# CogSP/CoEvoNet

Hardware: NVIDIA B200
Metric: mpe_env_steps_per_sec (higher is better)
Workload: dtype f32

## Files before the change

### coevonet_b200/_lib.py

```python
from __future__ import annotations

import ctypes
import os
from ctypes import (POINTER, Structure, c_char_p, c_double, c_float, c_int, c_int32,
                    c_int64, c_uint8, c_uint32, c_uint64, c_void_p)

_HERE = os.path.dirname(os.path.abspath(__file__))
LIB_PATH = os.environ.get("COEVONET_LIB") or os.path.join(_HERE, "csrc", "libcoevonet_b200.so")

CEV_OK = 0
STATUS_NONFINITE = 1
SEAT = {"adversary_0": 0, "agent_0": 1, "agent_1": 2}
KIND_ES, KIND_GA, KIND_ENV, KIND_FRAMES, KIND_INIT, KIND_XOVER = 0, 1, 2, 3, 4, 5
INIT_STATE_DIM = 11
ROLLOUT_OUT_DIM = 4
ORDER_STABLE_DESC, ORDER_REFERENCE = 0, 1
GS_GEN, GS_SIGMA, GS_BEST, GS_STALE, GS_STOP, GS_STOP_GEN, GS_LAST_EVAL, GS_HIST = 0, 1, 4, 7, 10, 11, 12, 16


class RolloutCfg(Structure):
    _fields_ = [("n_cycles", c_int32), ("integrate_pos_first", c_int32),
                ("variant", c_int32), ("reserved", c_int32)]


class RolloutRole(Structure):
    _fields_ = [("member_seat", c_int32), ("reserved", c_int32),
                ("members", c_void_p), ("member_pitch", c_int64),
                ("opp_a", c_void_p), ("opp_a_pitch", c_int64),
                ("opp_b", c_void_p), ("opp_b_pitch", c_int64),
                ("init", c_void_p), ("out", c_void_p)]


class CevError(RuntimeError):
    pass


_SIGNATURES = {
    "cev_version": (c_int, []),
    "cev_last_error": (c_char_p, []),
    "cev_create": (c_int, [c_int, POINTER(c_void_p)]),
    "cev_destroy": (c_int, [c_void_p]),
    "cev_device_info": (c_int, [c_void_p, POINTER(c_int), POINTER(c_int)]),
    "cev_fc_dim": (c_int, [c_int]),
    "cev_fc_pitch": (c_int, [c_int]),
    "cev_dqn_dim": (c_int, [c_int, c_int]),
    "cev_dqn_pitch": (c_int, [c_int, c_int]),
    "cev_mpe_rollout_f32": (c_int, [c_void_p, c_int, c_void_p, c_int, c_int64,
                                    c_void_p, c_int64, c_void_p, c_int64, c_int,
                                    c_void_p, c_int, c_int, POINTER(RolloutCfg),
                                    c_void_p, c_void_p, c_void_p]),
    "cev_mpe_rollout_roles_f32": (c_int, [c_void_p, c_int, POINTER(RolloutRole), c_int, c_int, c_int, c_int,
                                          POINTER(RolloutCfg), c_void_p, c_void_p]),
    "cev_mpe_rollout_trace_f32": (c_int, [c_void_p, c_int, c_void_p, c_int, c_int64,
                                          c_void_p, c_int64, c_void_p, c_int64, c_int,
                                          c_void_p, c_int, c_int, POINTER(RolloutCfg),
                                          c_void_p, c_void_p, c_void_p, c_void_p, c_void_p, c_void_p]),
    "cev_mpe_rollout_plan": (c_int, [c_void_p, c_int, c_int, c_int, c_int, c_int, POINTER(c_int), POINTER(c_int)]),
    "cev_kernel_timing_enable": (c_int, [c_void_p, c_int]),
    "cev_kernel_timing_read": (c_int, [c_void_p, c_int, POINTER(c_double), POINTER(c_int)]),
    "cev_mpe_rollout_indexed_f32": (c_int, [c_void_p, c_void_p, c_int64, c_void_p, c_int64,
                                            c_void_p, c_int64, c_void_p, c_void_p, c_int,
                                            POINTER(RolloutCfg), c_void_p, c_void_p, c_void_p]),
    "cev_fc_forward_f32": (c_int, [c_void_p, c_void_p, c_int64, c_int, c_void_p, c_void_p, c_int64,
                                   c_void_p, c_void_p, c_void_p, c_void_p]),
    "cev_ga_repopulate_f32": (c_int, [c_void_p, c_void_p, c_int, c_int, c_int64, c_float, c_void_p, c_float,
                                      c_uint64, c_int, c_uint32, c_int64, c_int64,
                                      c_void_p, c_void_p, c_void_p]),
    "cev_gather_rows_f32": (c_int, [c_void_p, c_void_p, c_int64, c_void_p, c_int, c_int64, c_int64, c_void_p,
                                    c_void_p]),
    "cev_select_topk_f64": (c_int, [c_void_p, c_void_p, c_int64, c_int, c_int, c_void_p, c_void_p]),
    "cev_es_perturb_f32": (c_int, [c_void_p, c_void_p, c_int, c_float, c_void_p, c_uint64, c_int, c_uint32,
                                   c_int64, c_int64, c_int64, c_void_p, c_void_p, c_void_p]),
    "cev_es_perturb_prefix_f32": (c_int, [c_void_p, c_void_p, c_int64, c_int64, c_float, c_void_p, c_uint64, c_int,
                                          c_uint32, c_int64, c_int64, c_int64, c_void_p, c_void_p]),
    "cev_es_update_f32": (c_int, [c_void_p, c_void_p, c_int, c_float, c_void_p, c_float, c_int64,
                                  c_uint64, c_int, c_uint32, c_int64, c_int64, c_void_p, c_void_p]),
    "cev_es_update_members_f32": (c_int, [c_void_p, c_void_p, c_void_p, c_int64, c_void_p, c_int, c_float, c_void_p,
                                          c_float, c_int64, c_int64, c_void_p, c_void_p]),
    "cev_weight_stats_f32": (c_int, [c_void_p, c_void_p, c_int64, c_int64, c_int, c_void_p, c_void_p]),
    "cev_generation_state_doubles": (c_int, [c_int]),
    "cev_generation_end_f64": (c_int, [c_void_p, c_void_p, c_int, c_int, c_int, c_void_p, c_int, c_int, c_double,
                                       c_double, c_int, c_double, c_int, c_void_p]),
    "cev_axpy_f32": (c_int, [c_void_p, c_float, c_void_p, c_void_p, c_int64, c_void_p]),
    "cev_diversity_dist_f32": (c_int, [c_void_p, c_void_p, c_int64, c_int64, c_void_p, c_int,
                                       c_void_p, c_void_p]),
    "cev_deepqn_forward": (c_int, [c_void_p, c_void_p, c_int, c_int64, c_void_p, c_int, c_int,
                                   c_int, c_void_p, c_void_p, c_void_p]),
    "cev_atari_synth_step_u8": (c_int, [c_void_p, c_uint64, c_int64, c_int64, c_int, c_void_p, c_void_p, c_void_p,
                                        c_void_p, c_void_p]),
    "cev_atari_observe_u8": (c_int, [c_void_p, c_void_p, c_int64, c_int, c_int, c_void_p, c_void_p]),
    "cev_fc_init_f32": (c_int, [c_void_p, c_int, c_uint64, c_int, c_int64, c_int64, c_int64, c_void_p, c_void_p]),
    "cev_init_states_f64": (c_int, [c_void_p, c_uint64, c_uint32, c_int64, c_int64, c_void_p, c_void_p]),
    "cev_random_frames_u8": (c_int, [c_void_p, c_uint64, c_int64, c_void_p, c_void_p]),
    "cev_philox_words": (c_int, [c_void_p, c_uint64, c_int, c_int, c_uint32, c_int64, c_int64,
                                 c_int64, c_void_p, c_void_p]),
    "cev_fp32_peak": (c_int, [c_void_p, c_int, POINTER(c_double), c_void_p]),
}

EXPORTED_SYMBOLS = tuple(_SIGNATURES)

_lib = None


def load():
    global _lib
    if _lib is not None:
        return _lib
    if not os.path.isfile(LIB_PATH):
        raise CevError(
            f"{LIB_PATH} is missing: build it with `python -c 'import __graft_entry__ as g; g.build()'` "
            "(or `make -C coevonet_b200/csrc`).  coevonet_b200 has no CPU fallback.")
    lib = ctypes.CDLL(LIB_PATH)
    for name, (res, args) in _SIGNATURES.items():
        fn = getattr(lib, name)
        fn.restype = res
        fn.argtypes = args
    _lib = lib
    return lib


def check(rc, what=""):
    if rc != CEV_OK:
        msg = load().cev_last_error()
        raise CevError(f"{what} failed (rc={rc}): {msg.decode() if msg else ''}")


_handles = {}


def handle(device_index, stream=0):
    key = (int(device_index), int(stream or 0))
    h = _handles.get(key)
    if h is None:
        lib = load()
        hp = c_void_p()
        check(lib.cev_create(int(device_index), ctypes.byref(hp)), "cev_create")
        h = _handles[key] = hp
    return h


def device_info(device_index):
    n_sm, n_cl = c_int(), c_int()
    check(load().cev_device_info(handle(device_index), ctypes.byref(n_sm), ctypes.byref(n_cl)),
          "cev_device_info")
    return n_sm.value, n_cl.value
```

### coevonet_b200/csrc/api.cu

```cuda
#include <stdarg.h>
#include <string.h>

#include "common.cuh"

namespace cev {

static thread_local char g_err[512] = "";

void set_error(const char* fmt, ...) {
    va_list ap;
    va_start(ap, fmt);
    vsnprintf(g_err, sizeof(g_err), fmt, ap);
    va_end(ap);
}

int check_cuda(cudaError_t e, const char* what) {
    if (e == cudaSuccess) return CEV_OK;
    set_error("CUDA error %d (%s) in %s", (int)e, cudaGetErrorString(e), what);
    return CEV_ERR_CUDA;
}

}

using namespace cev;
// ... 83 lines not shown

int cev_dqn_dim(int c_in, int n_actions) {
    return 32 * c_in * 64 + 32 + 64 * 32 * 16 + 64 + 64 * 64 * 9 + 64 + 512 * 3136 + 512 + n_actions * 512 +
           n_actions + 2 * (32 + 64 + 64);
}
int cev_dqn_pitch(int c_in, int n_actions) { return round_up(cev_dqn_dim(c_in, n_actions), 32); }

static int rollout_plan(const cev_handle* h, int P, int K, int E, int variant) {
    if (variant != 0) return variant;
    if ((int64_t)P * K * E >= 2048) return 3;
    return h->n_clusters > 0 ? 2 : 1;
}

static int check_cfg(const cev_rollout_cfg* cfg) {
    CEV_REQUIRE(cfg != nullptr, "rollout: null cfg");
    CEV_REQUIRE(cfg->n_cycles >= 0 && cfg->n_cycles <= MAX_CYCLES, "rollout: n_cycles must be in [0, %d]", MAX_CYCLES);
    CEV_REQUIRE(cfg->variant >= 0 && cfg->variant <= 3, "rollout: variant must be 0..3");
    return CEV_OK;
}

int cev_mpe_rollout_f32(cev_handle* h, int member_seat, const float* members, int P, int64_t member_pitch,
                        const float* opp_a, int64_t opp_a_pitch, const float* opp_b, int64_t opp_b_pitch, int K,
                        const double* init, int init_shared, int E, const cev_rollout_cfg* cfg, double* out,
                        int32_t* status, cev_stream stream) {
    CEV_REQUIRE(h && members && opp_a && opp_b && init && out, "mpe_rollout: null pointer");
    CEV_REQUIRE(member_seat >= 0 && member_seat <= 2, "mpe_rollout: member_seat must be 0..2");
    CEV_REQUIRE(P >= 0 && K >= 1 && E >= 1, "mpe_rollout: need P >= 0, K >= 1, E >= 1");
    int rc = check_cfg(cfg);
    if (rc) return rc;
    const int other[2] = {member_seat == 0 ? 1 : 0, member_seat == 2 ? 1 : 2};
    CEV_REQUIRE(member_pitch >= fc_offsets(seat_in_dim(member_seat)).total && member_pitch % 4 == 0,
                "mpe_rollout: member pitch too small / not a multiple of 4");
    CEV_REQUIRE(opp_a_pitch >= fc_offsets(seat_in_dim(other[0])).total && opp_a_pitch % 4 == 0 &&
                    opp_b_pitch >= fc_offsets(seat_in_dim(other[1])).total && opp_b_pitch % 4 == 0,
                "mpe_rollout: opponent pitch too small / not a multiple of 4");
    CEV_REQUIRE(aligned16(members) && aligned16(opp_a) && aligned16(opp_b), "mpe_rollout: rows must be 16B aligned");
    if (P == 0) return CEV_OK;
    CEV_GUARD(h);
    cudaStream_t st = (cudaStream_t)stream;
    const int variant = rollout_plan(h, P, K, E, cfg->variant);
    if (variant >= 2) {
        ClusterParams p{};
        p.members = members;
        p.member_pitch = member_pitch;
        p.P = P;
        p.opp[0] = opp_a;
        p.opp[1] = opp_b;
        p.opp_pitch[0] = opp_a_pitch;
        p.opp_pitch[1] = opp_b_pitch;
        p.K = K;
        p.member_seat = member_seat;
        p.init = init;
        p.init_shared = init_shared;
        p.E = E;
        p.out = out;
        p.status = status;
        p.n_cycles = cfg->n_cycles;
        p.pos_first = cfg->integrate_pos_first;
        return variant == 3 ? launch_rollout_lockstep(h, p, st) : launch_rollout_cluster(h, p, st);
    }
    GenericParams g{};
    g.w[member_seat] = members;
    g.pitch[member_seat] = member_pitch;
    g.w[other[0]] = opp_a;
    g.pitch[other[0]] = opp_a_pitch;
    g.w[other[1]] = opp_b;
    g.pitch[other[1]] = opp_b_pitch;
    g.idx = nullptr;
    g.member_seat = member_seat;
    g.K = K;
    g.E = E;
    g.init_shared = init_shared;
    g.init = init;
    g.out = out;
    g.status = status;
    g.n_cycles = cfg->n_cycles;
    g.pos_first = cfg->integrate_pos_first;
    g.N = (int64_t)P * K * E;
    return launch_rollout_generic(h, g, st);
}

int cev_mpe_rollout_roles_f32(cev_handle* h, int n_roles, const cev_rollout_role* roles, int P, int K, int init_shared,
                              int E, const cev_rollout_cfg* cfg, int32_t* status, cev_stream stream) {
    CEV_REQUIRE(h && roles, "mpe_rollout_roles: null pointer");
    CEV_REQUIRE(n_roles >= 1 && n_roles <= CEV_MAX_ROLES, "mpe_rollout_roles: n_roles must be 1..%d", CEV_MAX_ROLES);
    CEV_REQUIRE(P >= 0 && K >= 1 && E >= 1, "mpe_rollout_roles: need P >= 0, K >= 1, E >= 1");
    int rc = check_cfg(cfg);
    if (rc) return rc;
    for (int r = 0; r < n_roles; ++r)
        CEV_REQUIRE(roles[r].members && roles[r].opp_a && roles[r].opp_b && roles[r].init && roles[r].out,
                    "mpe_rollout_roles: null pointer in role %d", r);
    if (P == 0) return CEV_OK;
    const int variant = rollout_plan(h, P, K, E, cfg->variant);
    if (variant != 3) {
        for (int r = 0; r < n_roles; ++r) {
            rc = cev_mpe_rollout_f32(h, roles[r].member_seat, roles[r].members, P, roles[r].member_pitch, roles[r].opp_a,
                                     roles[r].opp_a_pitch, roles[r].opp_b, roles[r].opp_b_pitch, K, roles[r].init,
                                     init_shared, E, cfg, roles[r].out, status, stream);
            if (rc) return rc;
        }
        return CEV_OK;
    }
    ClusterParams ps[CEV_MAX_ROLES];
    for (int r = 0; r < n_roles; ++r) {
        const cev_rollout_role& q = roles[r];
        CEV_REQUIRE(q.member_seat >= 0 && q.member_seat <= 2, "mpe_rollout_roles: member_seat must be 0..2");
        const int other[2] = {q.member_seat == 0 ? 1 : 0, q.member_seat == 2 ? 1 : 2};
        CEV_REQUIRE(q.member_pitch >= fc_offsets(seat_in_dim(q.member_seat)).total && q.member_pitch % 4 == 0 &&
                        q.opp_a_pitch >= fc_offsets(seat_in_dim(other[0])).total && q.opp_a_pitch % 4 == 0 &&
                        q.opp_b_pitch >= fc_offsets(seat_in_dim(other[1])).total && q.opp_b_pitch % 4 == 0,
                    "mpe_rollout_roles: pitch too small / not a multiple of 4");
        CEV_REQUIRE(aligned16(q.members) && aligned16(q.opp_a) && aligned16(q.opp_b),
                    "mpe_rollout_roles: rows must be 16B aligned");
        ClusterParams& p = ps[r];
        p = ClusterParams{};
        p.members = q.members;
        p.member_pitch = q.member_pitch;
        p.P = P;
        p.opp[0] = q.opp_a;
        p.opp[1] = q.opp_b;
        p.opp_pitch[0] = q.opp_a_pitch;
        p.opp_pitch[1] = q.opp_b_pitch;
        p.K = K;
        p.member_seat = q.member_seat;
        p.init = q.init;
        p.init_shared = init_shared;
        p.E = E;
        p.out = q.out;
        p.status = status;
        p.n_cycles = cfg->n_cycles;
        p.pos_first = cfg->integrate_pos_first;
    }
    CEV_GUARD(h);
    return launch_rollout_lockstep_roles(h, ps, n_roles, (cudaStream_t)stream);
}

int cev_mpe_rollout_trace_f32(cev_handle* h, int member_seat, const float* members, int P, int64_t member_pitch,
                              const float* opp_a, int64_t opp_a_pitch, const float* opp_b, int64_t opp_b_pitch, int K,
                              const double* init, int init_shared, int E, const cev_rollout_cfg* cfg,
                              const int32_t* forced_actions, float* logits_out, int32_t* actions_out, double* out,
                              int32_t* status, cev_stream stream) {
    CEV_REQUIRE(h && members && opp_a && opp_b && init && out, "mpe_rollout_trace: null pointer");
    CEV_REQUIRE(member_seat >= 0 && member_seat <= 2, "mpe_rollout_trace: member_seat must be 0..2");
    CEV_REQUIRE(P >= 1 && K >= 1 && E >= 1, "mpe_rollout_trace: need P, K, E >= 1");
    int rc = check_cfg(cfg);
    if (rc) return rc;
    const int other[2] = {member_seat == 0 ? 1 : 0, member_seat == 2 ? 1 : 2};
    CEV_REQUIRE(member_pitch >= fc_offsets(seat_in_dim(member_seat)).total && member_pitch % 4 == 0 &&
                    opp_a_pitch >= fc_offsets(seat_in_dim(other[0])).total && opp_a_pitch % 4 == 0 &&
                    opp_b_pitch >= fc_offsets(seat_in_dim(other[1])).total && opp_b_pitch % 4 == 0,
                "mpe_rollout_trace: pitch too small / not a multiple of 4");
    CEV_REQUIRE(aligned16(members) && aligned16(opp_a) && aligned16(opp_b), "mpe_rollout_trace: rows must be 16B aligned");
    CEV_GUARD(h);
    ClusterParams p{};
    p.members = members;
    p.member_pitch = member_pitch;
    p.P = P;
    p.opp[0] = opp_a;
    p.opp[1] = opp_b;
    p.opp_pitch[0] = opp_a_pitch;
    p.opp_pitch[1] = opp_b_pitch;
    p.K = K;
    p.member_seat = member_seat;
    p.init = init;
    p.init_shared = init_shared;
    p.E = E;
    p.out = out;
    p.status = status;
    p.n_cycles = cfg->n_cycles;
    p.pos_first = cfg->integrate_pos_first;
    p.trace_forced = forced_actions;
    p.trace_logits = logits_out;
    p.trace_actions = actions_out;
    return launch_rollout_lockstep(h, p, (cudaStream_t)stream);
}

int cev_mpe_rollout_plan(cev_handle* h, int P, int K, int E, int n_cycles, int variant, int* variant_used,
                         int* n_launches) {
    CEV_REQUIRE(h != nullptr, "mpe_rollout_plan: null handle");
    CEV_REQUIRE(variant >= 0 && variant <= 3, "mpe_rollout_plan: variant must be 0..3");
    const int v = rollout_plan(h, P, K, E, variant);
    if (variant_used) *variant_used = v;
    if (n_launches) *n_launches = v == 3 ? rollout_lockstep_launches(n_cycles) : (v == 2 ? 3 : 1);
    return CEV_OK;
}

int cev_kernel_timing_enable(cev_handle* h, int on) {
    CEV_REQUIRE(h != nullptr, "kernel_timing_enable: null handle");
    CEV_GUARD(h);
    if (on && !h->timing_ev[0]) {
        for (int k = 0; k < 2; ++k) {
            h->timing_ev[k] = new cudaEvent_t[2 * CEV_TIMING_MAX];
            for (int i = 0; i < 2 * CEV_TIMING_MAX; ++i) CEV_CUDA(cudaEventCreate(&h->timing_ev[k][i]));
        }
    }
    h->timing_on = on ? 1 : 0;
    h->timing_n[0] = h->timing_n[1] = 0;
    return CEV_OK;
}

int cev_kernel_timing_read(cev_handle* h, int which, double* total_ms, int* n_launches) {
    CEV_REQUIRE(h != nullptr && (which == 0 || which == 1), "kernel_timing_read: bad arguments");
    CEV_GUARD(h);
    double tot = 0.0;
    const int n = h->timing_n[which];
    for (int i = 0; i < n; ++i) {
        CEV_CUDA(cudaEventSynchronize(h->timing_ev[which][2 * i + 1]));
        float ms = 0.f;
        CEV_CUDA(cudaEventElapsedTime(&ms, h->timing_ev[which][2 * i], h->timing_ev[which][2 * i + 1]));
        tot += ms;
    }
    if (total_ms) *total_ms = tot;
    if (n_launches) *n_launches = n;
    h->timing_n[which] = 0;
// ... 51 lines not shown
```

### coevonet_b200/csrc/common.cuh

```cuda
#pragma once

#include <cuda_runtime.h>
#include <math_constants.h>
#include <stdint.h>
#include <stdio.h>

#include "../../include/coevonet_b200.h"

namespace cev {

constexpr int H1 = 512;
constexpr int H2 = 256;
constexpr int NACT = 5;
constexpr int IN_ADV = 8;
constexpr int IN_GOOD = 10;
constexpr float LN_EPS = 1e-5f;
constexpr int MAX_CYCLES = 25;

struct FcOffsets {
    int fc1w, fc1b, ln1g, ln1b, fc2w, fc2b, ln2g, ln2b, outw, outb, total;
};

__host__ __device__ constexpr FcOffsets fc_offsets(int in_dim) {
    FcOffsets o{};
// ... 189 lines not shown
    return __fmaf_rn(__uint2float_rn(x), 2.3283064365386963e-10f, 1.1641532182693481e-10f);
}

__device__ __forceinline__ float neg2_log_u(float u) {
    const float t = 1.0f - u;
    const float ser = t * fmaf(t, fmaf(t, fmaf(t, fmaf(t, 0.2f, 0.25f), 0.33333334f), 0.5f), 1.0f);
    const float lg = -0.6931471805599453f * __log2f(u);
    return 2.0f * (t < 0.03125f ? ser : lg);
}

__device__ __forceinline__ void box_muller(uint32_t xa, uint32_t xb, float& z0, float& z1) {
    const float u1 = u01(xa), u2 = u01(xb);
    float r;
    asm("sqrt.approx.ftz.f32 %0, %1;\n" : "=f"(r) : "f"(neg2_log_u(u1)));
    float s, c;
    __sincosf(6.283185307179586f * (u2 - 0.5f), &s, &c);
    z0 = -(r * c);
    z1 = -(r * s);
}

__device__ __forceinline__ void normal4(const PhiloxKeys& keys, uint32_t tag, uint32_t gen,
                                        uint32_t member, uint32_t j4, float z[4]) {
    const U4 r = philox4x32_10(U4{j4, member, gen, tag}, keys);
    box_muller(r.x, r.y, z[0], z[1]);
    box_muller(r.z, r.w, z[2], z[3]);
}

__host__ __device__ __forceinline__ uint32_t noise_tag(int kind, int role) {
    return (uint32_t)(role & 0xFF) | ((uint32_t)kind << 8);
}

}

constexpr int CEV_TIMING_MAX = 4096;

#define CEV_MAX_ROLES 3

struct cev_handle {
    int device;
    int n_sm;
    int n_clusters;
    void* workspace;
    size_t workspace_bytes;
    void* opp_workspace;
    size_t opp_workspace_bytes;
    void* ls_workspace;
    size_t ls_workspace_bytes;
    cudaStream_t side_stream;
    cudaEvent_t fork_ev, join_ev;
    cudaStream_t env_stream, opp_stream2[3], mem_stream2[2];
    cudaEvent_t ev_opp[CEV_MAX_ROLES], ev_mem[CEV_MAX_ROLES], ev_env[CEV_MAX_ROLES];
    int timing_on;
    int timing_n[2];
    cudaEvent_t* timing_ev[2];
};

namespace cev {
struct GenericParams {
    const float* w[3];
    int64_t pitch[3];
    const int32_t* idx;
    int member_seat, K, E, init_shared;
    const double* init;
    double* out;
    int32_t* status;
    int n_cycles, pos_first;
    int64_t N;
};
struct ClusterParams {
    const float* members;
    int64_t member_pitch;
    int P;
    const float* opp[2];
    int64_t opp_pitch[2];
    const float4* opp_packed[2];
    int K;
    int member_seat;
    const double* init;
    int init_shared;
    int E;
    double* out;
    int32_t* status;
    int n_cycles, pos_first;
    const int32_t* trace_forced;
    float* trace_logits;
    int32_t* trace_actions;
};
int launch_rollout_generic(cev_handle* h, const GenericParams& p, cudaStream_t stream);
int launch_rollout_cluster(cev_handle* h, const ClusterParams& p, cudaStream_t stream);
int rollout_cluster_max_clusters(int device);
int launch_rollout_lockstep(cev_handle* h, const ClusterParams& p, cudaStream_t stream);
int launch_rollout_lockstep_roles(cev_handle* h, const ClusterParams* ps, int n_roles, cudaStream_t stream);
int rollout_lockstep_launches(int n_cycles);
int launch_deepqn_fc_tc(cev_handle* h, const float* members, int64_t pitch, int P, int B, int n_act, int f1w_off,
                        int f1b_off, int ow_off, int ob_off, const float* act3, float* logits, int32_t* actions,
                        cudaStream_t stream);
int launch_fc_forward(cev_handle* h, const float* W, int64_t pitch, int in_dim, const int32_t* idx,
                      const float* obs, int64_t N, float* logits, int32_t* actions, int32_t* status,
                      cudaStream_t stream);
}
```

### coevonet_b200/csrc/ls_member_tc.cuh

```cuda
#pragma once

namespace cev {

constexpr int MT_THREADS = 480;
constexpr int MT_PROD_WARPS = 8;
constexpr int MT_BK = 32, MT_KT = H1 / MT_BK;
constexpr int MT_NB = LS_BT;
constexpr int MT_R = 5, MT_L = 3;
constexpr uint32_t MT_A_BYTES = H2 * MT_BK * 4;
constexpr uint32_t MT_X_BYTES = MT_NB * MT_BK * 4;
constexpr uint32_t MT_XSLOT = 2 * MT_X_BYTES;
constexpr uint32_t MT_W1C_FLOATS = MT_BK * IN_GOOD + 3 * MT_BK;
constexpr uint32_t MT_W1C_BYTES = MT_W1C_FLOATS * 4;
constexpr uint32_t MT_TAIL_BYTES = LS_TAIL_FLOATS * 4;
constexpr size_t MT_OFF_X = (size_t)MT_R * MT_A_BYTES;
constexpr size_t MT_OFF_W1C = MT_OFF_X + (size_t)MT_L * MT_XSLOT;
constexpr size_t MT_OFF_HS = MT_OFF_W1C + (size_t)MT_R * MT_W1C_BYTES;
constexpr size_t MT_OFF_TAIL = MT_OFF_HS + (size_t)H2 * MT_NB * 4;
constexpr size_t MT_OFF_OBS = MT_OFF_TAIL + MT_TAIL_BYTES;
constexpr size_t MT_OFF_STAT = MT_OFF_OBS + 2 * MT_NB * LS_OBS_PAD * 4;
constexpr size_t MT_OFF_RED = MT_OFF_STAT + 2 * MT_NB * 8;
constexpr size_t MT_OFF_BAR = MT_OFF_RED + (size_t)(2 + NACT) * 4 * MT_NB * 4;
constexpr size_t MT_SMEM = MT_OFF_BAR + 256 + 1024 ;
constexpr int MT_ACC = 2 * MT_NB;
constexpr int MT_TM_OP = 2 * 2 * MT_ACC;
constexpr int MT_TM_SLOT = 2 * 2 * MT_BK;
static_assert(MT_TM_OP + MT_L * MT_TM_SLOT <= 512, "tensor memory budget");
static_assert(MT_OFF_X % 1024 == 0 && MT_XSLOT % 1024 == 0, "operand tiles must keep the 1024-byte alignment of the swizzle atoms");
static_assert(MT_OFF_W1C % 16 == 0 && MT_W1C_BYTES % 16 == 0 && MT_OFF_TAIL % 16 == 0 && MT_OFF_BAR % 8 == 0,
              "bulk-copy alignment");
static_assert(MT_SMEM <= 232448, "member stage exceeds the 227 KB shared-memory limit");
constexpr uint32_t MT_IDESC32 = (1u << 4) | (2u << 7) | (2u << 10) | ((uint32_t)((2 * MT_NB) >> 3) << 17) |
                                ((uint32_t)(128 >> 4) << 24);

__device__ __forceinline__ void mt_issue_ktile(uint32_t d_tmem, uint32_t a_tmem, uint64_t x_hilo, uint32_t accumulate,
                                               uint32_t bar_op) {
    asm volatile(
        "{\n"
        ".reg .pred pe, pa, pt;\n"
        ".reg .b64 b1, b2, b3;\n"
        ".reg .b32 h1, h2, h3, l0, l1, l2, l3;\n"
        "elect.sync _|pe, 0xffffffff;\n"
        "setp.ne.b32 pa, %3, 0;\n"
        "setp.eq.b32 pt, 0, 0;\n"
        "add.s64 b1, %2, 2;\n add.s64 b2, %2, 4;\n add.s64 b3, %2, 6;\n"
        "add.u32 h1, %1, 8;\n add.u32 h2, %1, 16;\n add.u32 h3, %1, 24;\n"
        "add.u32 l0, %1, 32;\n add.u32 l1, %1, 40;\n add.u32 l2, %1, 48;\n add.u32 l3, %1, 56;\n"
        "@pe tcgen05.mma.cta_group::1.kind::tf32 [%0], [l0], %2, %5, pa;\n"
        "@pe tcgen05.mma.cta_group::1.kind::tf32 [%0], [%1], %2, %5, pt;\n"
        "@pe tcgen05.mma.cta_group::1.kind::tf32 [%0], [l1], b1, %5, pt;\n"
        "@pe tcgen05.mma.cta_group::1.kind::tf32 [%0], [h1], b1, %5, pt;\n"
        "@pe tcgen05.mma.cta_group::1.kind::tf32 [%0], [l2], b2, %5, pt;\n"
        "@pe tcgen05.mma.cta_group::1.kind::tf32 [%0], [h2], b2, %5, pt;\n"
        "@pe tcgen05.mma.cta_group::1.kind::tf32 [%0], [l3], b3, %5, pt;\n"
        "@pe tcgen05.mma.cta_group::1.kind::tf32 [%0], [h3], b3, %5, pt;\n"
        "@pe tcgen05.commit.cta_group::1.mbarrier::arrive::one.shared::cluster.b64 [%4];\n"
        "}\n" ::"r"(d_tmem),
        "r"(a_tmem), "l"(x_hilo), "r"(accumulate), "r"(bar_op), "r"(MT_IDESC32)
        : "memory");
}
struct LsMemberTcParams {
    const float* members;
    int64_t pitch;
    int n_chunks, KE, seat, n_jobs;
    int64_t N;
    const float* obs;
    int32_t* act;
    float* gap;
    const double* l1stats;
    int32_t* status;
    float* logits;
};

template <int IN>
__global__ void __launch_bounds__(MT_THREADS, 1)
ls_member_tc_kernel(const __grid_constant__ CUtensorMap map_w, const LsMemberTcParams p) {
    extern __shared__ unsigned char mt_raw[];
    unsigned char* base = mt_raw + ((1024u - (tc_smem_u32(mt_raw) & 1023u)) & 1023u);
    unsigned char* raw_mem = base;
    unsigned char* x_mem = base + MT_OFF_X;
    float* hs = reinterpret_cast<float*>(base + MT_OFF_HS);
    unsigned char* w1c_mem = base + MT_OFF_W1C;
    float* tail = reinterpret_cast<float*>(base + MT_OFF_TAIL);
    float* obsbuf = reinterpret_cast<float*>(base + MT_OFF_OBS);
    float2* statbuf = reinterpret_cast<float2*>(base + MT_OFF_STAT);
    float* redA = reinterpret_cast<float*>(base + MT_OFF_RED);
    float* redB = redA + 4 * MT_NB;
    float* redC = redB + 4 * MT_NB;
    uint64_t* bar_raw_full = reinterpret_cast<uint64_t*>(base + MT_OFF_BAR);
    uint64_t* bar_raw_empty = bar_raw_full + MT_R;
    uint64_t* bar_lo_full = bar_raw_empty + MT_R;
    uint64_t* bar_lo_empty = bar_lo_full + MT_L;
    uint64_t* bar_tfull = bar_lo_empty + MT_L;
    uint64_t* bar_tempty = bar_tfull + 2;
    uint64_t* bar_stat_full = bar_tempty + 2;
    uint64_t* bar_tail_full = bar_stat_full + 2;
    uint64_t* bar_tail_empty = bar_tail_full + 1;
    uint32_t* tmem_slot = reinterpret_cast<uint32_t*>(bar_tail_empty + 1);
    int* flag = reinterpret_cast<int*>(tmem_slot + 1);

    const int warp = threadIdx.x >> 5, lane = threadIdx.x & 31;
    const int job0 = (int)blockIdx.x, job_stride = (int)gridDim.x;
    constexpr uint32_t W1ROWS_BYTES = (uint32_t)(MT_BK * IN) * 4;
    const FcOffsets om = fc_offsets(IN);

    if (threadIdx.x == 0) {
        *flag = 0;
        for (int i = 0; i < MT_R; ++i) {
            tc_mbar_init(bar_raw_full + i, 1);
            tc_mbar_init(bar_raw_empty + i, MT_PROD_WARPS / 2);
        }
        for (int i = 0; i < MT_L; ++i) {
            tc_mbar_init(bar_lo_full + i, MT_PROD_WARPS / 2);
            tc_mbar_init(bar_lo_empty + i, 2);
        }
        for (int i = 0; i < 2; ++i) {
            tc_mbar_init(bar_tfull + i, 2);
            tc_mbar_init(bar_tempty + i, 4);
            tc_mbar_init(bar_stat_full + i, 1);
        }
        tc_mbar_init(bar_tail_full, 1);
        tc_mbar_init(bar_tail_empty, 1);
        asm volatile("fence.mbarrier_init.release.cluster;\n" ::: "memory");
    }
    if (warp == 1) {
        asm volatile("tcgen05.alloc.cta_group::1.sync.aligned.shared::cta.b32 [%0], %1;\n" ::"r"(tc_smem_u32(tmem_slot)),
                     "r"(512u)
                     : "memory");
        asm volatile("tcgen05.relinquish_alloc_permit.cta_group::1.sync.aligned;\n" ::: "memory");
    }
    asm volatile("tcgen05.fence::before_thread_sync;\n" ::: "memory");
    __syncthreads();
    asm volatile("tcgen05.fence::after_thread_sync;\n" ::: "memory");
    const uint32_t tmem_base = *tmem_slot;

    if (warp == 0) {
        if (lane == 0) {
            uint32_t it = 0, js = 0;
            for (int job = job0; job < p.n_jobs; job += job_stride, ++js) {
                const int m = job / p.n_chunks;
                const float* mrow = p.members + (int64_t)m * p.pitch;
                for (int kt = 0; kt < MT_KT; ++kt, ++it) {
                    const uint32_t rs = it % MT_R, use = it / MT_R;
                    if (use > 0) tc_mbar_wait(bar_raw_empty + rs, (use - 1) & 1);
                    tc_mbar_expect_tx(bar_raw_full + rs, MT_A_BYTES + W1ROWS_BYTES + 3 * MT_BK * 4);
                    tma_load_3d(raw_mem + (size_t)rs * MT_A_BYTES, &map_w, bar_raw_full + rs, kt * MT_BK, 0, m);
                    float* c = reinterpret_cast<float*>(w1c_mem + (size_t)rs * MT_W1C_BYTES);
                    bulk_g2s(c, mrow + kt * MT_BK * IN, W1ROWS_BYTES, bar_raw_full + rs);
                    bulk_g2s(c + MT_BK * IN, mrow + om.fc1b + kt * MT_BK, MT_BK * 4, bar_raw_full + rs);
                    bulk_g2s(c + MT_BK * IN + MT_BK, mrow + om.ln1g + kt * MT_BK, MT_BK * 4, bar_raw_full + rs);
                    bulk_g2s(c + MT_BK * IN + 2 * MT_BK, mrow + om.ln1b + kt * MT_BK, MT_BK * 4, bar_raw_full + rs);
                }
                if (js >= 1) tc_mbar_wait(bar_tail_empty, (js - 1) & 1);
                tc_mbar_expect_tx(bar_tail_full, MT_TAIL_BYTES);
                bulk_g2s(tail, mrow + om.fc2b, MT_TAIL_BYTES, bar_tail_full);
            }
        }
    } else if (warp == 1 || warp == 14) {
        const int t = warp == 1 ? 0 : 1;
        const uint32_t x_base = tc_smem_u32(x_mem);
        uint32_t it = 0, js = 0;
        for (int job = job0; job < p.n_jobs; job += job_stride, ++js) {
            const uint32_t as = js & 1, ause = js >> 1;
            if (ause > 0) tc_mbar_wait(bar_tempty + as, (ause - 1) & 1);
            asm volatile("tcgen05.fence::after_thread_sync;\n" ::: "memory");
            const uint32_t d_tmem = tmem_base + as * (2 * MT_ACC) + t * MT_ACC;
            for (int kt = 0; kt < MT_KT; ++kt, ++it) {
                const uint32_t ls = it % MT_L, luse = it / MT_L;
                const uint64_t x_hilo = umma_desc_sw128(x_base + ls * MT_XSLOT);
                const uint32_t a_tmem = tmem_base + MT_TM_OP + ls * MT_TM_SLOT + t * (2 * MT_BK);
                tc_mbar_wait(bar_lo_full + ls, luse & 1);
                asm volatile("tcgen05.fence::after_thread_sync;\n" ::: "memory");
                mt_issue_ktile(d_tmem, a_tmem, x_hilo, kt ? 1u : 0u, tc_smem_u32(bar_lo_empty + ls));
                if (kt == MT_KT - 1) tc_commit_elected(tc_smem_u32(bar_tfull + as));
                __syncwarp();
            }
        }
    } else if (warp < 2 + MT_PROD_WARPS) {
        const int grp = (warp - 2) >> 2;
        const int pt = (threadIdx.x - 64) & 127;
        const int q = warp & 3;
        const int r = q * 32 + lane;
        const int e = pt & 15, g = pt >> 4;
        uint32_t it = 0, js = 0;
        for (int job = job0; job < p.n_jobs; job += job_stride, ++js) {
            const uint32_t b = js & 1, buse = js >> 1;
            tc_mbar_wait(bar_stat_full + b, buse & 1);
            float x[IN];
            {
                const float* ob = obsbuf + ((size_t)b * MT_NB + e) * LS_OBS_PAD;
#pragma unroll
                for (int i = 0; i < IN; i += 2) {
                    const float2 v = *reinterpret_cast<const float2*>(ob + i);
                    x[i] = v.x;
                    x[i + 1] = v.y;
                }
            }
            const float2 st = statbuf[b * MT_NB + e];
            const float mean = st.x, rstd = st.y;
            for (int kt = 0; kt < MT_KT; ++kt, ++it) {
                if ((int)(it & 1) != grp) continue;
                const uint32_t rs = it % MT_R, ruse = it / MT_R, ls = it % MT_L, luse = it / MT_L;
                const unsigned char* slot = raw_mem + (size_t)rs * MT_A_BYTES;
                unsigned char* xs = x_mem + (size_t)ls * MT_XSLOT;
                if (luse > 0) tc_mbar_wait(bar_lo_empty + ls, (luse - 1) & 1);
                tc_mbar_wait(bar_raw_full + rs, ruse & 1);
                asm volatile("tcgen05.fence::after_thread_sync;\n" ::: "memory");
#pragma unroll
                for (int t = 0; t < 2; ++t) {
                    const float4* row = reinterpret_cast<const float4*>(slot + (size_t)(t * 128 + r) * 128);
                    float w[32];
#pragma unroll
                    for (int c = 0; c < 8; ++c) {
                        const float4 v = row[c ^ (r & 7)];
                        w[4 * c] = v.x;
                        w[4 * c + 1] = v.y;
                        w[4 * c + 2] = v.z;
                        w[4 * c + 3] = v.w;
                    }
                    const uint32_t ta = tmem_base + ((uint32_t)(q * 32) << 16) + MT_TM_OP + ls * MT_TM_SLOT + t * (2 * MT_BK);
                    f3_tmem_st32(ta, w);
#pragma unroll
                    for (int i = 0; i < 32; ++i) w[i] = f3_lo(w[i]);
                    f3_tmem_st32(ta + MT_BK, w);
                }
                {
                    const float* w1c = reinterpret_cast<const float*>(w1c_mem + (size_t)rs * MT_W1C_BYTES);
                    const int kl = g * 4;
                    const float4 bb = *reinterpret_cast<const float4*>(w1c + MT_BK * IN + kl);
                    const float4 gg = *reinterpret_cast<const float4*>(w1c + MT_BK * IN + MT_BK + kl);
                    const float4 ee = *reinterpret_cast<const float4*>(w1c + MT_BK * IN + 2 * MT_BK + kl);
                    const float bq[4] = {bb.x, bb.y, bb.z, bb.w}, gq[4] = {gg.x, gg.y, gg.z, gg.w},
                                eq[4] = {ee.x, ee.y, ee.z, ee.w};
                    float hi[4], lo[4];
#pragma unroll
                    for (int qq = 0; qq < 4; ++qq) {
                        const float2* wr = reinterpret_cast<const float2*>(w1c + (kl + qq) * IN);
                        float pre = 0.f;
#pragma unroll
                        for (int i2 = 0; i2 < IN / 2; ++i2) {
                            const float2 v = wr[i2];
                            pre = fmaf(v.x, x[2 * i2], pre);
                            pre = fmaf(v.y, x[2 * i2 + 1], pre);
                        }
                        pre += bq[qq];
                        const float h = fmaxf(fmaf((pre - mean) * rstd, gq[qq], eq[qq]), 0.f);
                        hi[qq] = __uint_as_float(__float_as_uint(h) & 0xffffe000u);
                        lo[qq] = h - hi[qq];
                    }
                    const int off = e * 128 + ((g ^ (e & 7)) << 4);
                    *reinterpret_cast<float4*>(xs + off) = make_float4(hi[0], hi[1], hi[2], hi[3]);
                    *reinterpret_cast<float4*>(xs + MT_X_BYTES + off) = make_float4(lo[0], lo[1], lo[2], lo[3]);
                }
                __syncwarp();
                if (lane == 0) tc_mbar_arrive(bar_raw_empty + rs);
                asm volatile("tcgen05.wait::st.sync.aligned;\n" ::: "memory");
                asm volatile("fence.proxy.async.shared::cta;\n" ::: "memory");
                asm volatile("tcgen05.fence::before_thread_sync;\n" ::: "memory");
                __syncwarp();
                if (lane == 0) tc_mbar_arrive(bar_lo_full + ls);
            }
        }
    } else {
        const int q = warp & 3;
        const int et = (warp - 10) * 32 + lane;
        const int we = warp - 10;
        const int e1 = et & 15, g1 = et >> 4;
        constexpr int RP = H2 / 8;
        const float* b2 = tail;
        const float* g2 = tail + H2;
        const float* be2 = tail + 2 * H2;
        const float* w3 = tail + 3 * H2;
        const float* b3 = tail + 3 * H2 + NACT * H2;
        auto stage_job = [&](int job, uint32_t js) {
            if (job < p.n_jobs && et < MT_NB) {
                const uint32_t b = js & 1;
                const int m = job / p.n_chunks, ch = job % p.n_chunks;
                const int n_env = min(MT_NB, p.KE - ch * MT_NB);
                const int64_t ep = (int64_t)m * p.KE + (int64_t)ch * MT_NB + (et < n_env ? et : 0);
                const float4* src = reinterpret_cast<const float4*>(p.obs + ep * LS_OBS_PAD);
                const float4 v0 = __ldg(src), v1 = __ldg(src + 1), v2 = __ldg(src + 2);
                float4* dst = reinterpret_cast<float4*>(obsbuf + ((size_t)b * MT_NB + et) * LS_OBS_PAD);
                dst[0] = v0;
                dst[1] = v1;
                dst[2] = v2;
                const float xo[12] = {v0.x, v0.y, v0.z, v0.w, v1.x, v1.y, v1.z, v1.w, v2.x, v2.y, v2.z, v2.w};
                const double* S = p.l1stats + (size_t)m * LS_L1S;
                double z[11];
#pragma unroll
                for (int a = 0; a < 11; ++a) z[a] = a < IN ? (double)xo[a] : (a == IN ? 1.0 : 0.0);
                double md = 0.0, vd = 0.0;
#pragma unroll
                for (int a = 0; a < 11; ++a) {
                    md = fma(__ldg(S + a), z[a], md);
                    double ra = 0.0;
#pragma unroll
                    for (int c = 0; c < 11; ++c) ra = fma(__ldg(S + 11 + a * 11 + c), z[c], ra);
                    vd = fma(ra, z[a], vd);
                }
                const float m1 = (float)md, var = (float)vd;
                if (!isfinite(m1) || !isfinite(var)) *flag = 1;
                statbuf[b * MT_NB + et] = make_float2(m1, 1.0f / sqrtf(var + LN_EPS));
            }
            if (job < p.n_jobs && we == 0) {
                __syncwarp();
                if (lane == 0) tc_mbar_arrive(bar_stat_full + (js & 1));
            }
        };
        stage_job(job0, 0);
        stage_job(job0 + job_stride, 1);
        uint32_t js = 0;
        for (int job = job0; job < p.n_jobs; job += job_stride, ++js) {
            const int m = job / p.n_chunks, ch = job % p.n_chunks;
            const int n_env = min(MT_NB, p.KE - ch * MT_NB);
            const int64_t ep0 = (int64_t)m * p.KE + (int64_t)ch * MT_NB;
            const uint32_t as = js & 1, ause = js >> 1;
            tc_mbar_wait(bar_tail_full, js & 1);
            tc_mbar_wait(bar_tfull + as, ause & 1);
            asm volatile("tcgen05.fence::after_thread_sync;\n" ::: "memory");
#pragma unroll
            for (int t = 0; t < 2; ++t) {
                uint32_t xh[16], xl[16];
                const uint32_t ta = tmem_base + ((uint32_t)(q * 32) << 16) + as * (2 * MT_ACC) + t * MT_ACC;
                f3_tmem_ld16(ta, xh);
                f3_tmem_ld16(ta + MT_NB, xl);
                const int row = t * 128 + q * 32 + lane;
                const float bias = b2[row];
                float4* dst = reinterpret_cast<float4*>(hs + row * MT_NB);
                const int sw = (row >> 1) & 3;
                float h[16];
#pragma unroll
                for (int n = 0; n < 16; ++n)
                    h[n] = (__uint_as_float(xl[n]) + __uint_as_float(xh[n])) + bias;
#pragma unroll
                for (int c = 0; c < 4; ++c) dst[c ^ sw] = make_float4(h[4 * c], h[4 * c + 1], h[4 * c + 2], h[4 * c + 3]);
            }
            asm volatile("tcgen05.fence::before_thread_sync;\n" ::: "memory");
            __syncwarp();
            if (lane == 0) tc_mbar_arrive(bar_tempty + as);
            asm volatile("bar.sync 1, 128;\n" ::: "memory");
            float pre2[RP];
            float lsum = 0.f;
#pragma unroll
            for (int j = 0; j < RP; ++j) {
                const int row = g1 + 8 * j;
                pre2[j] = hs[row * MT_NB + ((((e1 >> 2) ^ ((row >> 1) & 3))) << 2) + (e1 & 3)];
                lsum += pre2[j];
            }
            lsum = group_sum<MT_NB>(lsum);
            if (lane < MT_NB) redA[we * MT_NB + e1] = lsum;
            asm volatile("bar.sync 1, 128;\n" ::: "memory");
            float mean = 0.f;
#pragma unroll
            for (int w = 0; w < 4; ++w) mean += redA[w * MT_NB + e1];
            mean *= (1.0f / H2);
            float lsq = 0.f;
#pragma unroll
            for (int j = 0; j < RP; ++j) {
                const float d = pre2[j] - mean;
                lsq = fmaf(d, d, lsq);
            }
            lsq = group_sum<MT_NB>(lsq);
            if (lane < MT_NB) redB[we * MT_NB + e1] = lsq;
            asm volatile("bar.sync 1, 128;\n" ::: "memory");
            float var = 0.f;
#pragma unroll
            for (int w = 0; w < 4; ++w) var += redB[w * MT_NB + e1];
            var *= (1.0f / H2);
            if (!isfinite(mean) || !isfinite(var)) *flag = 1;
            const float rstd = 1.0f / sqrtf(var + LN_EPS);
            float pl[NACT] = {0.f, 0.f, 0.f, 0.f, 0.f};
#pragma unroll
            for (int j = 0; j < RP; ++j) {
                const int row = g1 + 8 * j;
                const float h = fmaxf(fmaf((pre2[j] - mean) * rstd, g2[row], be2[row]), 0.f);
#pragma unroll
                for (int a = 0; a < NACT; ++a) pl[a] = fmaf(w3[a * H2 + row], h, pl[a]);
            }
#pragma unroll
            for (int a = 0; a < NACT; ++a) {
                const float v = group_sum<MT_NB>(pl[a]);
                if (lane < MT_NB) redC[(we * NACT + a) * MT_NB + e1] = v;
            }
            asm volatile("bar.sync 1, 128;\n" ::: "memory");
            if (et < MT_NB) {
                float lg[NACT];
                bool fin = true;
#pragma unroll
                for (int a = 0; a < NACT; ++a) {
                    float v = redC[a * MT_NB + et];
#pragma unroll
                    for (int w = 1; w < 4; ++w) v += redC[(w * NACT + a) * MT_NB + et];
                    lg[a] = v + b3[a];
                    fin = fin && isfinite(lg[a]);
                }
                float gap;
                const int a = argmax_first5(lg, gap);
                if (et < n_env) {
                    if (!fin) *flag = 1;
                    p.act[ep0 + et] = a;
                    p.gap[ep0 + et] = gap;
                    if (p.logits) {
#pragma unroll
                        for (int u = 0; u < NACT; ++u) p.logits[(ep0 + et) * NACT + u] = lg[u];
                    }
                }
            }
            asm volatile("bar.sync 1, 128;\n" ::: "memory");
            if (et == 0) tc_mbar_arrive(bar_tail_empty);
            stage_job(job + 2 * job_stride, js + 2);
        }
    }
    asm volatile("tcgen05.fence::before_thread_sync;\n" ::: "memory");
    __syncthreads();
    if (threadIdx.x == 0 && *flag && p.status) atomicOr(p.status, CEV_STATUS_NONFINITE);
    if (warp == 1)
        asm volatile("tcgen05.dealloc.cta_group::1.sync.aligned.b32 %0, %1;\n" ::"r"(tmem_base), "r"(512u) : "memory");
}

}
```

### coevonet_b200/csrc/population_ops.cu

```cuda
#include "common.cuh"

namespace cev {

constexpr int PT = 256;

__device__ __forceinline__ float pick_sigma(float sigma, const double* __restrict__ sigma_dev) {
    return sigma_dev ? (float)__ldg(sigma_dev) : sigma;
}

__global__ void __launch_bounds__(PT) ga_repopulate_kernel(
    const float* __restrict__ elites, int E, int D, int64_t pitch, float sigma_arg,
    const double* __restrict__ sigma_dev,
    const PhiloxKeys keys, uint32_t tag, uint32_t gen, int64_t row0,
    float xrate, uint32_t xtag,
    float* __restrict__ out, float* __restrict__ noise_out) {
    const float sigma = pick_sigma(sigma_arg, sigma_dev);
    const int64_t r = blockIdx.x;
    const int64_t c = row0 + r;
    const int j4 = blockIdx.y * PT + threadIdx.x;
    __shared__ int64_t mate_s;
    int64_t mate = -1;
    if (xrate > 0.f && E >= 2) {
        if (threadIdx.x == 0) {
            int64_t m = -1;
            if (c != 0) {
                const U4 y = philox4x32_10(U4{0xFFFFFFFFu, (uint32_t)c, gen, xtag}, keys);
                if ((double)y.x < (double)xrate * 4294967296.0)
                    m = ((c - 1) % E + 1 + (int64_t)(y.y % (uint32_t)(E - 1))) % E;
            }
            mate_s = m;
        }
        __syncthreads();
        mate = mate_s;
    }
    if ((int64_t)j4 * 4 >= pitch) return;
    const int64_t parent = (c == 0) ? 0 : (c - 1) % E;
    const float4 pv = *reinterpret_cast<const float4*>(elites + parent * pitch + (int64_t)j4 * 4);
    float p[4] = {pv.x, pv.y, pv.z, pv.w};
    if (mate >= 0) {
        const float4 qv = *reinterpret_cast<const float4*>(elites + mate * pitch + (int64_t)j4 * 4);
        const U4 x = philox4x32_10(U4{(uint32_t)j4, (uint32_t)c, gen, xtag}, keys);
        if (!(x.x & 1u)) p[0] = qv.x;
        if (!(x.y & 1u)) p[1] = qv.y;
        if (!(x.z & 1u)) p[2] = qv.z;
        if (!(x.w & 1u)) p[3] = qv.w;
    }
    float z[4] = {0.f, 0.f, 0.f, 0.f};
    if (c != 0) {
        normal4(keys, tag, gen, (uint32_t)c, (uint32_t)j4, z);
#pragma unroll
        for (int i = 0; i < 4; ++i) {
            const int j = j4 * 4 + i;
            if (j < D) p[i] = __fadd_rn(p[i], __fmul_rn(sigma, z[i]));
            else { p[i] = 0.f; z[i] = 0.f; }
        }
    }
    *reinterpret_cast<float4*>(out + r * pitch + (int64_t)j4 * 4) = make_float4(p[0], p[1], p[2], p[3]);
    if (noise_out)
        *reinterpret_cast<float4*>(noise_out + r * pitch + (int64_t)j4 * 4) = make_float4(z[0], z[1], z[2], z[3]);
}

constexpr int K5T = 128;
__global__ void __launch_bounds__(K5T, 10) es_perturb_kernel(
    const float* __restrict__ theta, int in_dim, int64_t pitch, float sigma_arg,
    const double* __restrict__ sigma_dev,
    const PhiloxKeys keys, uint32_t tag, uint32_t gen, int64_t row0,
    float* __restrict__ out, float* __restrict__ noise_out) {
    const float sigma = pick_sigma(sigma_arg, sigma_dev);
    const FcOffsets o = fc_offsets(in_dim);
    const int64_t r = blockIdx.x;
    const int64_t c = row0 + r;
    const int j4 = blockIdx.y * K5T + threadIdx.x;
    const int j = j4 * 4;
    if ((int64_t)j >= pitch) return;
    const float4 pv = __ldg(reinterpret_cast<const float4*>(theta + j));
    float p[4] = {pv.x, pv.y, pv.z, pv.w};
    float z[4] = {0.f, 0.f, 0.f, 0.f};
    if (j < o.total && fc_is_perturbable(o, j)) {
        normal4(keys, tag, gen, (uint32_t)c, (uint32_t)j4, z);
#pragma unroll
        for (int i = 0; i < 4; ++i) {
            if (j + i < o.total) p[i] = __fadd_rn(p[i], __fmul_rn(sigma, z[i]));
            else { z[i] = 0.f; p[i] = 0.f; }
        }
    } else if (j >= o.total) {
        p[0] = p[1] = p[2] = p[3] = 0.f;
    }
    __stcs(reinterpret_cast<float4*>(out + r * pitch + j), make_float4(p[0], p[1], p[2], p[3]));
    if (noise_out)
        *reinterpret_cast<float4*>(noise_out + r * pitch + j) = make_float4(z[0], z[1], z[2], z[3]);
}

__global__ void __launch_bounds__(PT) es_perturb_prefix_kernel(
    const float* __restrict__ theta, int64_t d_pert, int64_t d_total, int64_t pitch, float sigma_arg,
    const double* __restrict__ sigma_dev,
    const PhiloxKeys keys, uint32_t tag, uint32_t gen, int64_t row0, float* __restrict__ out) {
    const float sigma = pick_sigma(sigma_arg, sigma_dev);
    const int64_t r = blockIdx.x;
    const int64_t j4 = (int64_t)blockIdx.y * PT + threadIdx.x;
    if (j4 * 4 >= pitch) return;
    const float4 pv = *reinterpret_cast<const float4*>(theta + j4 * 4);
    float p[4] = {pv.x, pv.y, pv.z, pv.w};
    if (j4 * 4 < d_pert) {
        float z[4];
        normal4(keys, tag, gen, (uint32_t)(row0 + r), (uint32_t)j4, z);
#pragma unroll
        for (int i = 0; i < 4; ++i)
            if (j4 * 4 + i < d_pert) p[i] = __fadd_rn(p[i], __fmul_rn(sigma, z[i]));
    }
#pragma unroll
    for (int i = 0; i < 4; ++i)
        if (j4 * 4 + i >= d_total) p[i] = 0.f;
    __stcs(reinterpret_cast<float4*>(out + r * pitch + j4 * 4), make_float4(p[0], p[1], p[2], p[3]));
}

__global__ void __launch_bounds__(PT) es_update_partial_kernel(
    const double* __restrict__ fitness, int in_dim, int64_t pitch, float sigma_arg,
    const double* __restrict__ sigma_dev,
    const PhiloxKeys keys, uint32_t tag, uint32_t gen, int64_t row0, int64_t n_rows,
    int n_split, float* __restrict__ partial) {
    const float sigma = pick_sigma(sigma_arg, sigma_dev);
    const FcOffsets o = fc_offsets(in_dim);
    const int j4 = blockIdx.x * PT + threadIdx.x;
    if ((int64_t)j4 * 4 >= pitch) return;
    const int sp = blockIdx.y;
    const int64_t per = (n_rows + n_split - 1) / n_split;
    const int64_t r_lo = sp * per, r_hi = min(n_rows, r_lo + per);
    float acc[4] = {0.f, 0.f, 0.f, 0.f};
    bool pert[4];
#pragma unroll
    for (int i = 0; i < 4; ++i) {
        const int j = j4 * 4 + i;
        pert[i] = j < o.total && fc_is_perturbable(o, j);
    }
    if (pert[0] || pert[1] || pert[2] || pert[3]) {
        for (int64_t r = r_lo; r < r_hi; ++r) {
            const float f = (float)fitness[r];
            float z[4];
            normal4(keys, tag, gen, (uint32_t)(row0 + r), (uint32_t)j4, z);
#pragma unroll
            for (int i = 0; i < 4; ++i) acc[i] = fmaf(__fmul_rn(sigma, z[i]), f, acc[i]);
        }
    }
#pragma unroll
    for (int i = 0; i < 4; ++i)
        if (!pert[i]) acc[i] = 0.f;
    *reinterpret_cast<float4*>(partial + (int64_t)sp * pitch + (int64_t)j4 * 4) =
        make_float4(acc[0], acc[1], acc[2], acc[3]);
}

__global__ void __launch_bounds__(PT) es_update_members_partial_kernel(
    const double* __restrict__ fitness, const float* __restrict__ members, const float* __restrict__ theta,
    int64_t pitch, int64_t n_rows, int n_split, float* __restrict__ partial) {
    const int j4 = blockIdx.x * PT + threadIdx.x;
    if ((int64_t)j4 * 4 >= pitch) return;
    const int sp = blockIdx.y;
    const int64_t per = (n_rows + n_split - 1) / n_split;
    const int64_t r_lo = sp * per, r_hi = min(n_rows, r_lo + per);
    const float4 t4 = *reinterpret_cast<const float4*>(theta + (int64_t)j4 * 4);
    float acc[4] = {0.f, 0.f, 0.f, 0.f};
    const float4* col = reinterpret_cast<const float4*>(members) + j4;
    const int64_t stride4 = pitch / 4;
#pragma unroll 8
    for (int64_t r = r_lo; r < r_hi; ++r) {
        const float f = (float)fitness[r];
        const float4 m = __ldcs(col + r * stride4);
        acc[0] = fmaf(__fsub_rn(m.x, t4.x), f, acc[0]);
        acc[1] = fmaf(__fsub_rn(m.y, t4.y), f, acc[1]);
        acc[2] = fmaf(__fsub_rn(m.z, t4.z), f, acc[2]);
        acc[3] = fmaf(__fsub_rn(m.w, t4.w), f, acc[3]);
    }
    *reinterpret_cast<float4*>(partial + (int64_t)sp * pitch + (int64_t)j4 * 4) =
        make_float4(acc[0], acc[1], acc[2], acc[3]);
}
// ... 330 lines not shown
#pragma unroll
        for (int i = 0; i < 8; ++i) {
            if (MODE == 1) a[i] = __ffma2_rn(a[i], b, c);
            else { a[i].x = fmaf(a[i].x, b.x, c.x); a[i].y = fmaf(a[i].y, b.y, c.y); }
        }
    }
    float s = 0.f;
#pragma unroll
    for (int i = 0; i < 8; ++i) s += a[i].x + a[i].y;
    if (s == 123.456f) out[0] = s;
}

}

using namespace cev;

static inline void split_seed(uint64_t seed, uint32_t& k0, uint32_t& k1) {
    k0 = (uint32_t)(seed & 0xFFFFFFFFull);
    k1 = (uint32_t)(seed >> 32);
}

static int ensure_workspace(cev_handle* h, size_t bytes) {
    if (h->workspace_bytes >= bytes) return CEV_OK;
    if (h->workspace) cudaFree(h->workspace);
    h->workspace = nullptr;
    h->workspace_bytes = 0;
    CEV_CUDA(cudaMalloc(&h->workspace, bytes));
    h->workspace_bytes = bytes;
    return CEV_OK;
}

static bool aligned16(const void* p) { return (reinterpret_cast<uintptr_t>(p) & 15u) == 0; }

extern "C" {

int cev_ga_repopulate_f32(cev_handle* h, const float* elites, int E, int D, int64_t pitch, float sigma,
                          const double* sigma_dev, float crossover_rate, uint64_t seed, int role, uint32_t gen,
                          int64_t row0, int64_t n_rows, float* out, float* noise_out, cev_stream stream) {
    CEV_REQUIRE(h != nullptr, "ga_repopulate: null handle");
    if (n_rows == 0) return CEV_OK;
    CEV_REQUIRE(elites && out, "ga_repopulate: null pointer");
    CEV_REQUIRE(E >= 1 && D >= 1 && pitch >= D && pitch % 4 == 0, "ga_repopulate: bad E/D/pitch");
    CEV_REQUIRE(crossover_rate >= 0.f && crossover_rate <= 1.f, "ga_repopulate: crossover_rate must be in [0, 1]");
    CEV_REQUIRE(aligned16(elites) && aligned16(out) && aligned16(noise_out), "ga_repopulate: 16B alignment");
    CEV_REQUIRE(row0 >= 0 && n_rows >= 0 && row0 + n_rows <= 0xFFFFFFFFll, "ga_repopulate: bad row range");
    CEV_GUARD(h);
    uint32_t k0, k1;
    split_seed(seed, k0, k1);
    dim3 grid((unsigned)n_rows, (unsigned)((pitch / 4 + PT - 1) / PT));
    ga_repopulate_kernel<<<grid, PT, 0, (cudaStream_t)stream>>>(elites, E, D, pitch, sigma, sigma_dev, philox_keys(k0, k1),
                                                               noise_tag(CEV_KIND_GA, role), gen, row0, crossover_rate,
                                                               noise_tag(CEV_KIND_XOVER, role), out, noise_out);
    return check_cuda(cudaGetLastError(), "ga_repopulate_kernel");
}

int cev_gather_rows_f32(cev_handle* h, const float* src, int64_t pitch, const int64_t* idx, int n, int64_t row0,
                        int64_t n_local, float* dst, cev_stream stream) {
    CEV_REQUIRE(h != nullptr, "gather_rows: null handle");
    if (n <= 0) return CEV_OK;
    CEV_REQUIRE((src || n_local == 0) && idx && dst, "gather_rows: null pointer");
    CEV_REQUIRE(pitch % 4 == 0 && aligned16(src) && aligned16(dst), "gather_rows: alignment");
    CEV_GUARD(h);
    dim3 grid((unsigned)n, (unsigned)((pitch / 4 + PT - 1) / PT));
    gather_rows_kernel<<<grid, PT, 0, (cudaStream_t)stream>>>(src, pitch, idx, row0, n_local, dst);
    return check_cuda(cudaGetLastError(), "gather_rows_kernel");
}

int cev_select_topk_f64(cev_handle* h, const double* fitness, int64_t P, int k, int order, int64_t* idx_out,
                        cev_stream stream) {
    CEV_REQUIRE(h && fitness && idx_out, "select_topk: null pointer");
    CEV_REQUIRE(k >= 1 && k <= P, "select_topk: need 1 <= k <= P (elites_number %d, population %lld)", k, (long long)P);
    CEV_REQUIRE(order == 0 || order == 1, "select_topk: order must be 0 (ties -> lower index) or 1 (reference)");
    CEV_GUARD(h);
    int rc = ensure_workspace(h, (size_t)P + 256);
    if (rc) return rc;
    select_topk_kernel<<<1, SEL_T, 0, (cudaStream_t)stream>>>(fitness, P, k, order, static_cast<uint8_t*>(h->workspace),
                                                              idx_out);
    return check_cuda(cudaGetLastError(), "select_topk_kernel");
}

int cev_es_perturb_f32(cev_handle* h, const float* theta, int in_dim, float sigma, const double* sigma_dev,
                       uint64_t seed, int role, uint32_t gen, int64_t row0, int64_t n_rows, int64_t pitch,
                       float* out, float* noise_out, cev_stream stream) {
    CEV_REQUIRE(h != nullptr, "es_perturb: null handle");
    if (n_rows == 0) return CEV_OK;
    CEV_REQUIRE(theta && out, "es_perturb: null pointer");
    CEV_REQUIRE(in_dim == IN_ADV || in_dim == IN_GOOD, "es_perturb: in_dim must be 8 or 10");
    CEV_REQUIRE(pitch >= fc_offsets(in_dim).total && pitch % 4 == 0, "es_perturb: bad pitch");
    CEV_REQUIRE(aligned16(theta) && aligned16(out) && aligned16(noise_out), "es_perturb: 16B alignment");
    CEV_REQUIRE(row0 >= 0 && n_rows >= 0 && row0 + n_rows <= 0xFFFFFFFFll, "es_perturb: bad row range");
    CEV_GUARD(h);
    uint32_t k0, k1;
    split_seed(seed, k0, k1);
    dim3 grid((unsigned)n_rows, (unsigned)((pitch / 4 + K5T - 1) / K5T));
    es_perturb_kernel<<<grid, K5T, 0, (cudaStream_t)stream>>>(theta, in_dim, pitch, sigma, sigma_dev, philox_keys(k0, k1),
                                                            noise_tag(CEV_KIND_ES, role), gen, row0, out,
                                                            noise_out);
    return check_cuda(cudaGetLastError(), "es_perturb_kernel");
}

int cev_es_update_f32(cev_handle* h, const double* fitness, int in_dim, float sigma, const double* sigma_dev,
                      float lr, int64_t n_total, uint64_t seed, int role, uint32_t gen, int64_t row0,
                      int64_t n_rows, float* delta, cev_stream stream) {
    CEV_REQUIRE(h && (fitness || n_rows == 0) && delta, "es_update: null pointer");
    CEV_REQUIRE(in_dim == IN_ADV || in_dim == IN_GOOD, "es_update: in_dim must be 8 or 10");
    CEV_REQUIRE(n_total >= 1 && n_rows >= 0 && (sigma_dev || sigma > 0.f), "es_update: bad n/sigma");
    CEV_REQUIRE(aligned16(delta), "es_update: 16B alignment");
    CEV_GUARD(h);
    const int64_t pitch = fc_pitch(in_dim);
    int n_split = (int)((n_rows + 63) / 64);
    if (n_split > 16) n_split = 16;
    if (n_split < 1) n_split = 1;
    int rc = ensure_workspace(h, (size_t)n_split * pitch * sizeof(float));
    if (rc) return rc;
    uint32_t k0, k1;
    split_seed(seed, k0, k1);
    float* partial = static_cast<float*>(h->workspace);
    dim3 grid((unsigned)((pitch / 4 + PT - 1) / PT), (unsigned)n_split);
    es_update_partial_kernel<<<grid, PT, 0, (cudaStream_t)stream>>>(fitness, in_dim, pitch, sigma, sigma_dev, philox_keys(k0, k1),
                                                                   noise_tag(CEV_KIND_ES, role), gen, row0,
                                                                   n_rows, n_split, partial);
    CEV_CUDA(cudaGetLastError());
    es_update_finish_kernel<<<(unsigned)((pitch + PT - 1) / PT), PT, 0, (cudaStream_t)stream>>>(
        partial, n_split, pitch, (double)lr, (double)n_total, sigma, sigma_dev, delta);
    return check_cuda(cudaGetLastError(), "es_update kernels");
}

int cev_es_perturb_prefix_f32(cev_handle* h, const float* theta, int64_t d_pert, int64_t d_total, float sigma,
                              const double* sigma_dev, uint64_t seed, int role, uint32_t gen, int64_t row0,
                              int64_t n_rows, int64_t pitch, float* out, cev_stream stream) {
    CEV_REQUIRE(h != nullptr, "es_perturb_prefix: null handle");
    if (n_rows == 0) return CEV_OK;
    CEV_REQUIRE(theta && out, "es_perturb_prefix: null pointer");
    CEV_REQUIRE(d_pert >= 0 && d_pert <= d_total && d_total <= pitch && pitch % 4 == 0 && pitch / 4 <= 0xFFFFFFFFll,
                "es_perturb_prefix: need 0 <= d_pert <= d_total <= pitch, pitch a multiple of 4");
    CEV_REQUIRE(aligned16(theta) && aligned16(out), "es_perturb_prefix: 16B alignment");
    CEV_REQUIRE(row0 >= 0 && n_rows >= 0 && row0 + n_rows <= 0xFFFFFFFFll, "es_perturb_prefix: bad row range");
    CEV_GUARD(h);
    uint32_t k0, k1;
    split_seed(seed, k0, k1);
    dim3 grid((unsigned)n_rows, (unsigned)((pitch / 4 + PT - 1) / PT));
    es_perturb_prefix_kernel<<<grid, PT, 0, (cudaStream_t)stream>>>(theta, d_pert, d_total, pitch, sigma, sigma_dev, philox_keys(k0, k1),
                                                                   noise_tag(CEV_KIND_ES, role), gen, row0, out);
    return check_cuda(cudaGetLastError(), "es_perturb_prefix_kernel");
}

int cev_es_update_members_f32(cev_handle* h, const double* fitness, const float* members, int64_t pitch,
                              const float* theta, int in_dim, float sigma, const double* sigma_dev, float lr,
                              int64_t n_total, int64_t n_rows, float* delta, cev_stream stream) {
    CEV_REQUIRE(h && ((fitness && members) || n_rows == 0) && theta && delta, "es_update_members: null pointer");
    CEV_REQUIRE(n_total >= 1 && n_rows >= 0 && (sigma_dev || sigma > 0.f), "es_update_members: bad n/sigma");
    CEV_REQUIRE(in_dim == 0 || in_dim == IN_ADV || in_dim == IN_GOOD, "es_update_members: in_dim must be 0, 8 or 10");
    CEV_REQUIRE(in_dim == 0 ? (pitch > 0 && pitch % 4 == 0) : pitch == fc_pitch(in_dim),
                "es_update_members: rows must use the padded pitch (cev_fc_pitch / cev_dqn_pitch)");
    CEV_REQUIRE(aligned16(delta) && aligned16(members) && aligned16(theta), "es_update_members: 16B alignment");
    CEV_GUARD(h);
    int n_split = (int)((n_rows + 31) / 32);
    if (n_split > 32) n_split = 32;
    if (n_split < 1) n_split = 1;
    int rc = ensure_workspace(h, (size_t)n_split * pitch * sizeof(float));
    if (rc) return rc;
    float* partial = static_cast<float*>(h->workspace);
    dim3 grid((unsigned)((pitch / 4 + PT - 1) / PT), (unsigned)n_split);
    es_update_members_partial_kernel<<<grid, PT, 0, (cudaStream_t)stream>>>(fitness, members, theta, pitch, n_rows,
                                                                           n_split, partial);
    CEV_CUDA(cudaGetLastError());
    es_update_finish_kernel<<<(unsigned)((pitch + PT - 1) / PT), PT, 0, (cudaStream_t)stream>>>(
        partial, n_split, pitch, (double)lr, (double)n_total, sigma, sigma_dev, delta);
    return check_cuda(cudaGetLastError(), "es_update_members kernels");
}

int cev_axpy_f32(cev_handle* h, float a, const float* x, float* y, int64_t n, cev_stream stream) {
    CEV_REQUIRE(h && x && y && n >= 0, "axpy: bad arguments");
    if (n == 0) return CEV_OK;
    CEV_GUARD(h);
    axpy_kernel<<<(unsigned)((n + PT - 1) / PT), PT, 0, (cudaStream_t)stream>>>(a, x, y, n);
    return check_cuda(cudaGetLastError(), "axpy_kernel");
}

int cev_diversity_dist_f32(cev_handle* h, const float* pop, int64_t n_rows, int64_t pitch, const float* ref,
// ... 123 lines not shown
```

### coevonet_b200/csrc/rollout_lockstep.cu

```cuda
#include <stdlib.h>

#include <cuda_fp16.h>

#include "rollout_common.cuh"
#include "tc_common.cuh"

namespace cev {

constexpr int LS_ST_FIELDS = 16;
constexpr int LS_OBS_PAD = 12;
constexpr int LS_L1S = 132;

struct LsBuffers {
    double* st;
    double* acc;
    float* min_gap;
    int32_t* goal;
    float* obs;
    int32_t* act;
    float* gap;
    __half* w2split;
    uint32_t* wmax;
    float* oscale;
    double* l1stats;
    float2* l1ms;
    double* ml1stats;
};

static size_t ls_align(size_t x) { return (x + 255) & ~(size_t)255; }

static size_t ls_carve(void* base, int64_t N, int K, int P, LsBuffers* b) {
    size_t off = 0;
    char* p = static_cast<char*>(base);
    auto take = [&](size_t bytes) {
        void* r = p ? p + off : nullptr;
        off += ls_align(bytes);
        return r;
    };
    LsBuffers t;
    t.w2split = static_cast<__half*>(take((size_t)2 * K * 2 * H2 * H1 * sizeof(__half)));
    t.wmax = static_cast<uint32_t*>(take((size_t)2 * K * sizeof(uint32_t)));
    t.oscale = static_cast<float*>(take((size_t)2 * K * 2 * sizeof(float)));
    t.st = static_cast<double*>(take((size_t)LS_ST_FIELDS * N * sizeof(double)));
    t.acc = static_cast<double*>(take((size_t)3 * N * sizeof(double)));
    t.min_gap = static_cast<float*>(take((size_t)N * sizeof(float)));
    t.goal = static_cast<int32_t*>(take((size_t)N * sizeof(int32_t)));
    t.obs = static_cast<float*>(take((size_t)3 * N * LS_OBS_PAD * sizeof(float)));
    t.act = static_cast<int32_t*>(take((size_t)3 * N * sizeof(int32_t)));
    t.gap = static_cast<float*>(take((size_t)3 * N * sizeof(float)));
    t.l1stats = static_cast<double*>(take((size_t)2 * K * LS_L1S * sizeof(double)));
    t.l1ms = static_cast<float2*>(take((size_t)2 * N * sizeof(float2)));
    t.ml1stats = static_cast<double*>(take((size_t)P * LS_L1S * sizeof(double)));
    if (b) *b = t;
    return off;
}

__device__ __forceinline__ void ls_store_state(const LsBuffers& b, int64_t N, int64_t ep, const EnvState& s) {
#pragma unroll
    for (int i = 0; i < 3; ++i) {
        b.st[(0 + i) * N + ep] = s.px[i];
        b.st[(3 + i) * N + ep] = s.py[i];
        b.st[(6 + i) * N + ep] = s.vx[i];
        b.st[(9 + i) * N + ep] = s.vy[i];
    }
#pragma unroll
    for (int l = 0; l < 2; ++l) {
        b.st[(12 + l) * N + ep] = s.lx[l];
        b.st[(14 + l) * N + ep] = s.ly[l];
    }
}
__device__ __forceinline__ void ls_load_state(const LsBuffers& b, int64_t N, int64_t ep, EnvState& s) {
#pragma unroll
    for (int i = 0; i < 3; ++i) {
        s.px[i] = b.st[(0 + i) * N + ep];
        s.py[i] = b.st[(3 + i) * N + ep];
        s.vx[i] = b.st[(6 + i) * N + ep];
        s.vy[i] = b.st[(9 + i) * N + ep];
    }
#pragma unroll
    for (int l = 0; l < 2; ++l) {
        s.lx[l] = b.st[(12 + l) * N + ep];
        s.ly[l] = b.st[(14 + l) * N + ep];
    }
    s.goal = b.goal[ep];
}
__device__ __forceinline__ float2 ls_row_stats(const double* __restrict__ S, const float* __restrict__ x, int in, bool& finite) {
    double z[11];
#pragma unroll
    for (int a = 0; a < 11; ++a) z[a] = a < in ? (double)x[a] : (a == in ? 1.0 : 0.0);
    double md = 0.0, vd = 0.0;
#pragma unroll
    for (int a = 0; a < 11; ++a) {
        md = fma(__ldg(S + a), z[a], md);
        double ra = 0.0;
#pragma unroll
        for (int b = 0; b < 11; ++b) ra = fma(__ldg(S + 11 + a * 11 + b), z[b], ra);
        vd = fma(ra, z[a], vd);
    }
    const float m1 = (float)md, var = (float)vd;
    finite = isfinite(m1) && isfinite(var);
    return make_float2(m1, 1.0f / sqrtf(var + LN_EPS));
}

__device__ __forceinline__ bool ls_store_obs(const LsBuffers& b, int64_t N, int64_t ep, const EnvState& s, int K, int E,
                                             const int (&opp_seat)[2]) {
    bool ok = true;
#pragma unroll
    for (int seat = 0; seat < 3; ++seat) {
        float o[LS_OBS_PAD];
#pragma unroll
        for (int j = 0; j < LS_OBS_PAD; ++j) o[j] = 0.f;
        env_observe(s, seat, o);
        float4* dst = reinterpret_cast<float4*>(b.obs + ((int64_t)seat * N + ep) * LS_OBS_PAD);
        dst[0] = make_float4(o[0], o[1], o[2], o[3]);
        dst[1] = make_float4(o[4], o[5], o[6], o[7]);
        dst[2] = make_float4(o[8], o[9], o[10], o[11]);
#pragma unroll
        for (int oi = 0; oi < 2; ++oi)
            if (seat == opp_seat[oi]) {
                const int k = (int)((ep / E) % K);
                bool fin;
                b.l1ms[(int64_t)oi * N + ep] = ls_row_stats(b.l1stats + (size_t)(oi * K + k) * LS_L1S, o, seat_in_dim(seat), fin);
                ok = ok && fin;
            }
    }
    return ok;
}

struct LsEnvParams {
    LsBuffers b;
    int64_t N;
    int K, E, init_shared, pos_first, last;
    const double* init;
    double* out;
    const int32_t* forced;
    int32_t* act_out;
    int opp_seat[2];
    int32_t* status;
};

__global__ void __launch_bounds__(256) ls_init_kernel(const LsEnvParams p) {
    const int64_t ep = (int64_t)blockIdx.x * blockDim.x + threadIdx.x;
    if (ep >= p.N) return;
    const int e = (int)(ep % p.E), k = (int)((ep / p.E) % p.K);
    const int64_t rec = p.init_shared ? ((int64_t)k * p.E + e) : ep;
    EnvState s;
    env_load(s, p.init + rec * CEV_INIT_STATE_DIM);
    ls_store_state(p.b, p.N, ep, s);
    p.b.goal[ep] = s.goal;
    p.b.acc[ep] = 0.0;
    p.b.acc[p.N + ep] = 0.0;
    p.b.acc[2 * p.N + ep] = 0.0;
    p.b.min_gap[ep] = CUDART_INF_F;
    if (!ls_store_obs(p.b, p.N, ep, s, p.K, p.E, p.opp_seat) && p.status) atomicOr(p.status, CEV_STATUS_NONFINITE);
    if (p.last) {
        double* o = p.out + ep * CEV_ROLLOUT_OUT_DIM;
        o[0] = 0.0;
        o[1] = 0.0;
        o[2] = 0.0;
        o[3] = (double)CUDART_INF_F;
    }
}

__global__ void __launch_bounds__(256) ls_env_step_kernel(const LsEnvParams p) {
    const int64_t ep = (int64_t)blockIdx.x * blockDim.x + threadIdx.x;
    if (ep >= p.N) return;
    EnvState s;
    ls_load_state(p.b, p.N, ep, s);
    int act[3] = {p.b.act[ep], p.b.act[p.N + ep], p.b.act[2 * p.N + ep]};
    if (p.act_out) {
        p.act_out[ep] = act[0];
        p.act_out[p.N + ep] = act[1];
        p.act_out[2 * p.N + ep] = act[2];
    }
    if (p.forced) {
        act[0] = p.forced[ep];
        act[1] = p.forced[p.N + ep];
        act[2] = p.forced[2 * p.N + ep];
    }
    const float g = fminf(p.b.gap[ep], fminf(p.b.gap[p.N + ep], p.b.gap[2 * p.N + ep]));
    double rg, ra;
    env_step(s, act, p.pos_first != 0, rg, ra);
    const double sum_good = __dadd_rn(p.b.acc[ep], rg);
    const double sum_adv = __dadd_rn(p.b.acc[2 * p.N + ep], ra);
    const float min_gap = fminf(p.b.min_gap[ep], g);
    if (p.last) {
        double* o = p.out + ep * CEV_ROLLOUT_OUT_DIM;
        o[0] = sum_good;
        o[1] = rg;
        o[2] = sum_adv;
        o[3] = (double)min_gap;
        return;
    }
    p.b.acc[ep] = sum_good;
    p.b.acc[p.N + ep] = rg;
    p.b.acc[2 * p.N + ep] = sum_adv;
    p.b.min_gap[ep] = min_gap;
    ls_store_state(p.b, p.N, ep, s);
    if (!ls_store_obs(p.b, p.N, ep, s, p.K, p.E, p.opp_seat) && p.status) atomicOr(p.status, CEV_STATUS_NONFINITE);
}

struct LsPrepParams {
    const float* opp[2];
    int64_t opp_pitch[2];
    int seat[2];
    int K;
    __half* w2split;
    uint32_t* wmax;
    float* oscale;
    double* l1stats;
};

__device__ __forceinline__ int ls_scale_exp(float bound, int target) {
    if (!(bound > 0.f) || !isfinite(bound)) return 0;
    const int s = target - ilogbf(bound);
    return s < -40 ? -40 : (s > 40 ? 40 : s);
}

__global__ void __launch_bounds__(256) ls_wmax_kernel(const LsPrepParams p) {
    const int oi = blockIdx.y / p.K, k = blockIdx.y % p.K;
    const FcOffsets o = fc_offsets(seat_in_dim(p.seat[oi]));
    const float4* src = reinterpret_cast<const float4*>(p.opp[oi] + (int64_t)k * p.opp_pitch[oi] + o.fc2w);
    float m = 0.f;
    for (int f = blockIdx.x * blockDim.x + threadIdx.x; f < H2 * H1 / 4; f += gridDim.x * blockDim.x) {
        const float4 w = src[f];
        m = fmaxf(fmaxf(m, fmaxf(fabsf(w.x), fabsf(w.y))), fmaxf(fabsf(w.z), fabsf(w.w)));
    }
#pragma unroll
    for (int off = 16; off > 0; off >>= 1) m = fmaxf(m, __shfl_xor_sync(0xffffffffu, m, off));
    if ((threadIdx.x & 31) == 0) atomicMax(p.wmax + blockIdx.y, __float_as_uint(m));
}

__global__ void __launch_bounds__(256) ls_split_w2_kernel(const LsPrepParams p) {
    const int oi = blockIdx.y / p.K, k = blockIdx.y % p.K;
    const FcOffsets o = fc_offsets(seat_in_dim(p.seat[oi]));
    const float4* src = reinterpret_cast<const float4*>(p.opp[oi] + (int64_t)k * p.opp_pitch[oi] + o.fc2w);
    const float sw = ldexpf(1.0f, ls_scale_exp(__uint_as_float(p.wmax[blockIdx.y]), 14));
    uint2* hi = reinterpret_cast<uint2*>(p.w2split + (size_t)(blockIdx.y * 2 + 0) * H2 * H1);
    uint2* lo = reinterpret_cast<uint2*>(p.w2split + (size_t)(blockIdx.y * 2 + 1) * H2 * H1);
    for (int f = blockIdx.x * blockDim.x + threadIdx.x; f < H2 * H1 / 4; f += gridDim.x * blockDim.x) {
        const float4 w = src[f];
        const float v[4] = {w.x * sw, w.y * sw, w.z * sw, w.w * sw};
        __half h[4], l[4];
#pragma unroll
        for (int i = 0; i < 4; ++i) {
            h[i] = __float2half_rn(v[i]);
            l[i] = __float2half_rn(v[i] - __half2float(h[i]));
        }
        const __half2 h01 = __halves2half2(h[0], h[1]), h23 = __halves2half2(h[2], h[3]);
        const __half2 l01 = __halves2half2(l[0], l[1]), l23 = __halves2half2(l[2], l[3]);
        hi[f] = make_uint2(*reinterpret_cast<const uint32_t*>(&h01), *reinterpret_cast<const uint32_t*>(&h23));
        lo[f] = make_uint2(*reinterpret_cast<const uint32_t*>(&l01), *reinterpret_cast<const uint32_t*>(&l23));
    }
}

__device__ __forceinline__ void ls_l1stats_row(const float* __restrict__ row, int in, double* __restrict__ out) {
    const int d = in + 1;
    const float* w1 = row;
    const float* b1 = row + H1 * in;
    __shared__ float cols[11][H1 + 1];
    __shared__ double wbar[11];
    const int t = threadIdx.x, lane = t & 31, warp = t >> 5;
    for (int i = t; i < H1 * in; i += 512) cols[i % in][i / in] = w1[i];
    cols[in][t] = b1[t];
    __syncthreads();
    for (int a = warp; a < 11; a += 16) {
        double s = 0.0;
        if (a < d)
            for (int r = lane; r < H1; r += 32) s += (double)cols[a][r];
#pragma unroll
        for (int o = 16; o > 0; o >>= 1) s += __shfl_xor_sync(0xffffffffu, s, o);
        if (lane == 0) wbar[a] = s / H1;
    }
    __syncthreads();
    if (t < 11) out[t] = wbar[t];
    for (int pr = warp; pr < 66; pr += 16) {
        int a = 0, rem = pr;
        while (rem >= 11 - a) {
            rem -= 11 - a;
            ++a;
        }
        const int b = a + rem;
        double s = 0.0;
        if (a < d && b < d) {
            const double ma = wbar[a], mb = wbar[b];
            for (int r = lane; r < H1; r += 32) s += ((double)cols[a][r] - ma) * ((double)cols[b][r] - mb);
        }
#pragma unroll
        for (int o = 16; o > 0; o >>= 1) s += __shfl_xor_sync(0xffffffffu, s, o);
        if (lane == 0) {
            out[11 + a * 11 + b] = s / H1;
            out[11 + b * 11 + a] = s / H1;
        }
    }
}

__global__ void __launch_bounds__(512) ls_l1stats_kernel(const LsPrepParams p) {
    const int oi = blockIdx.x / p.K, k = blockIdx.x % p.K;
    const int in = seat_in_dim(p.seat[oi]);
    const float* row = p.opp[oi] + (int64_t)k * p.opp_pitch[oi];
    ls_l1stats_row(row, in, p.l1stats + (size_t)blockIdx.x * LS_L1S);
    __shared__ float red[2][16];
    const int t = threadIdx.x;
    float g = fabsf(row[H1 * in + H1 + t]), be = fabsf(row[H1 * in + 2 * H1 + t]);
#pragma unroll
    for (int off = 16; off > 0; off >>= 1) {
        g = fmaxf(g, __shfl_xor_sync(0xffffffffu, g, off));
        be = fmaxf(be, __shfl_xor_sync(0xffffffffu, be, off));
    }
    if ((t & 31) == 0) {
        red[0][t >> 5] = g;
        red[1][t >> 5] = be;
    }
    __syncthreads();
    if (t == 0) {
        for (int w = 1; w < 16; ++w) {
            g = fmaxf(g, red[0][w]);
            be = fmaxf(be, red[1][w]);
        }
        const int sx = ls_scale_exp(22.63f * g + be, 13);
        const int sw = ls_scale_exp(__uint_as_float(p.wmax[blockIdx.x]), 14);
        p.oscale[blockIdx.x * 2 + 0] = ldexpf(1.0f, sx);
        p.oscale[blockIdx.x * 2 + 1] = ldexpf(1.0f, -(sx + sw));
    }
}

__global__ void __launch_bounds__(512) ls_member_l1stats_kernel(const float* __restrict__ members, int64_t pitch, int in,
                                                                double* __restrict__ out) {
    ls_l1stats_row(members + (int64_t)blockIdx.x * pitch, in, out + (size_t)blockIdx.x * LS_L1S);
}

#ifndef LS_GRID_OPP_DEFAULT
#define LS_GRID_OPP_DEFAULT 0
#endif
#ifndef LS_GRID_MEM_DEFAULT
#define LS_GRID_MEM_DEFAULT 0
#endif
constexpr int LS_BT = 16;
constexpr int LS_TAIL_FLOATS = 2056;
constexpr int LS_W1A_FLOATS = H1 * IN_GOOD + 3 * H1;

constexpr int OP_THREADS = 448;
constexpr int OP_PROD = 256;
constexpr int OP_BM = 128, OP_BN = 256, OP_BK = 64, OP_KT = H1 / OP_BK;
constexpr uint32_t OP_A_BYTES = OP_BM * OP_BK * 2;
constexpr uint32_t OP_B_BYTES = OP_BN * OP_BK * 2;
constexpr uint32_t OP_STAGE_BYTES = 2 * OP_A_BYTES + 2 * OP_B_BYTES;
constexpr int OP_STAGES = 2;
constexpr size_t OP_OFF_W1A = (size_t)OP_STAGES * OP_STAGE_BYTES;
constexpr size_t OP_OFF_TAIL = OP_OFF_W1A + (size_t)LS_W1A_FLOATS * 4;
constexpr size_t OP_OFF_BAR = OP_OFF_TAIL + (size_t)LS_TAIL_FLOATS * 4;
constexpr size_t OP_SMEM_MAX = 232448;
constexpr size_t OP_SLACK = OP_SMEM_MAX - (OP_OFF_BAR + 128);
constexpr size_t OP_SMEM = OP_SMEM_MAX;
constexpr uint32_t OP_IDESC = (1u << 4) | ((uint32_t)(OP_BN >> 3) << 17) | ((uint32_t)(OP_BM >> 4) << 24);

struct LsOppParams {
    const float* opp[2];
    int64_t opp_pitch[2];
    int seat[2];
    int K, E, n_tiles, n_jobs;
    int64_t PE;
    int64_t N;
    const float* obs;
    int32_t* act;
    float* gap;
    const float2* l1ms;
    const float* oscale;
    int32_t* status;
    float* logits;
};

template <int IN>
__device__ __forceinline__ void op_produce_chunk(const float* __restrict__ w1a, const float (&x)[4][IN_GOOD],
                                                 const float (&mean)[4], const float (&rstd)[4], float sx, int kt, int c,
                                                 int lane, unsigned char* __restrict__ a_hi,
                                                 unsigned char* __restrict__ a_lo) {
    const float* fc1b = w1a + H1 * IN;
    const float* ln1g = fc1b + H1;
    const float* ln1b = ln1g + H1;
    const int k0 = kt * OP_BK + c * 8;
    uint32_t hi[4][4], lo[4][4];
#pragma unroll
    for (int half = 0; half < 2; ++half) {
        const float4 bb = *reinterpret_cast<const float4*>(fc1b + k0 + 4 * half);
        const float4 gg = *reinterpret_cast<const float4*>(ln1g + k0 + 4 * half);
        const float4 ee = *reinterpret_cast<const float4*>(ln1b + k0 + 4 * half);
        const float bq[4] = {bb.x, bb.y, bb.z, bb.w}, gq[4] = {gg.x * sx, gg.y * sx, gg.z * sx, gg.w * sx},
                    eq[4] = {ee.x * sx, ee.y * sx, ee.z * sx, ee.w * sx};
        float hv[4][4];
#pragma unroll
        for (int qq = 0; qq < 4; ++qq) {
            float w[IN];
            const float2* wr = reinterpret_cast<const float2*>(w1a + (k0 + 4 * half + qq) * IN);
#pragma unroll
            for (int i2 = 0; i2 < IN / 2; ++i2) {
                const float2 v = wr[i2];
                w[2 * i2] = v.x;
                w[2 * i2 + 1] = v.y;
            }
#pragma unroll
            for (int j = 0; j < 4; ++j) {
                float pre = 0.f;
#pragma unroll
                for (int i = 0; i < IN; ++i) pre = fmaf(w[i], x[j][i], pre);
                pre += bq[qq];
                hv[j][qq] = fmaxf(fmaf((pre - mean[j]) * rstd[j], gq[qq], eq[qq]), 0.f);
            }
        }
#pragma unroll
        for (int j = 0; j < 4; ++j)
#pragma unroll
// ... 280 lines not shown
                                          tc_smem_u32(bar_empty + st));
                    if (kt == OP_KT - 1) tc_commit_elected(tc_smem_u32(bar_tfull + as));
                }
                __syncwarp();
            }
        }
    }
    asm volatile("tcgen05.fence::before_thread_sync;\n" ::: "memory");
    __syncthreads();
    if (threadIdx.x == 0 && *flag && p.status) atomicOr(p.status, CEV_STATUS_NONFINITE);
    if (warp == 13)
        asm volatile("tcgen05.dealloc.cta_group::1.sync.aligned.b32 %0, %1;\n" ::"r"(tmem_base), "r"(512u) : "memory");
}

}

#include "ls_member_tc.cuh"

namespace cev {

int rollout_lockstep_launches(int n_cycles) { return 5 + 3 * n_cycles; }

static void ls_split_sms(int n_sm, int opp_jobs, int mem_jobs, int* g_opp, int* g_mem) {
    double best = 1e30;
    int bo = n_sm / 2;
    for (int g = 1; g < n_sm; ++g) {
        const int gm = n_sm - g;
        const int mg = mem_jobs < gm ? mem_jobs : gm, og = opp_jobs < g ? opp_jobs : g;
        const double t_job_mem = fmax(8.6, mg * 0.0873);
        const double t_opp = 12.0 + 14.0 * ((opp_jobs + og - 1) / og);
        const double t_mem = 4.0 + t_job_mem * ((mem_jobs + mg - 1) / mg);
        const double t = fmax(t_opp, t_mem);
        if (t < best - 1e-9) {
            best = t;
            bo = g;
        }
    }
    *g_opp = bo;
    *g_mem = n_sm - bo;
}

struct LsRoleCtx {
    LsBuffers b;
    CUtensorMap map_b, map_wtc;
    LsEnvParams ep;
    LsOppParams op;
    LsMemberTcParams tp;
    int env_blocks;
    int64_t member_ctas;
    int ms;
};

static int ls_configure(cev_handle* h) {
    static bool configured[16] = {};
    if (h->device < 16 && !configured[h->device]) {
        CEV_CUDA(cudaFuncSetAttribute(ls_opp_kernel, cudaFuncAttributeMaxDynamicSharedMemorySize, (int)OP_SMEM));
        CEV_CUDA(cudaFuncSetAttribute(ls_member_tc_kernel<IN_ADV>, cudaFuncAttributeMaxDynamicSharedMemorySize, (int)MT_SMEM));
        CEV_CUDA(cudaFuncSetAttribute(ls_member_tc_kernel<IN_GOOD>, cudaFuncAttributeMaxDynamicSharedMemorySize, (int)MT_SMEM));
        configured[h->device] = true;
    }
    return CEV_OK;
}

static int ls_reserve(cev_handle* h, size_t need) {
    if (h->ls_workspace_bytes < need) {
        if (h->ls_workspace) CEV_CUDA(cudaFree(h->ls_workspace));
        h->ls_workspace = nullptr;
        h->ls_workspace_bytes = 0;
        CEV_CUDA(cudaMalloc(&h->ls_workspace, need));
        h->ls_workspace_bytes = need;
    }
    return CEV_OK;
}

static int ls_build_role(cev_handle* h, const ClusterParams& p, void* ws, cudaStream_t stream, cudaStream_t stream_m,
                         LsRoleCtx* c) {
    EncodeTiledFn encode = get_encode_fn();
    if (!encode) {
        set_error("rollout_lockstep: cuTensorMapEncodeTiled is not available from the driver");
        return CEV_ERR_UNSUPPORTED;
    }
    const int64_t N = (int64_t)p.P * p.K * p.E;
    LsBuffers& b = c->b;
    ls_carve(ws, N, p.K, p.P, &b);
    const int ms = p.member_seat;
    c->ms = ms;
    const int seat_of[2] = {ms == 0 ? 1 : 0, ms == 2 ? 1 : 2};

    LsPrepParams pp{};
    for (int oi = 0; oi < 2; ++oi) {
        pp.opp[oi] = p.opp[oi];
        pp.opp_pitch[oi] = p.opp_pitch[oi];
        pp.seat[oi] = seat_of[oi];
    }
    pp.K = p.K;
    pp.w2split = b.w2split;
    pp.wmax = b.wmax;
    pp.oscale = b.oscale;
    pp.l1stats = b.l1stats;
    CEV_CUDA(cudaMemsetAsync(b.wmax, 0, (size_t)2 * p.K * sizeof(uint32_t), stream));
    ls_wmax_kernel<<<dim3(32, 2 * p.K), 256, 0, stream>>>(pp);
    ls_split_w2_kernel<<<dim3(32, 2 * p.K), 256, 0, stream>>>(pp);
    ls_l1stats_kernel<<<2 * p.K, 512, 0, stream>>>(pp);
    ls_member_l1stats_kernel<<<p.P, 512, 0, stream_m>>>(p.members, p.member_pitch, seat_in_dim(ms), b.ml1stats);

    const FcOffsets om = fc_offsets(seat_in_dim(ms));
    {
        cuuint64_t dims[3] = {(cuuint64_t)H1, (cuuint64_t)H2, (cuuint64_t)p.P};
        cuuint64_t strides[2] = {(cuuint64_t)H1 * 4, (cuuint64_t)p.member_pitch * 4};
        cuuint32_t box[3] = {MT_BK, H2, 1};
        cuuint32_t estr[3] = {1, 1, 1};
        CUresult r = encode(&c->map_wtc, CU_TENSOR_MAP_DATA_TYPE_FLOAT32, 3, const_cast<float*>(p.members + om.fc2w), dims,
                            strides, box, estr, CU_TENSOR_MAP_INTERLEAVE_NONE, CU_TENSOR_MAP_SWIZZLE_128B,
                            CU_TENSOR_MAP_L2_PROMOTION_L2_256B, CU_TENSOR_MAP_FLOAT_OOB_FILL_NONE);
        if (r != CUDA_SUCCESS) {
            set_error("rollout_lockstep: cuTensorMapEncodeTiled(member fc2, tensor-core form) failed with %d", (int)r);
            return CEV_ERR_CUDA;
        }
    }
    {
        cuuint64_t dims[2] = {(cuuint64_t)H1, (cuuint64_t)2 * p.K * 2 * H2};
        cuuint64_t strides[1] = {(cuuint64_t)H1 * sizeof(__half)};
        cuuint32_t box[2] = {OP_BK, OP_BN};
        cuuint32_t estr[2] = {1, 1};
        CUresult r = encode(&c->map_b, CU_TENSOR_MAP_DATA_TYPE_FLOAT16, 2, b.w2split, dims, strides, box, estr,
                            CU_TENSOR_MAP_INTERLEAVE_NONE, CU_TENSOR_MAP_SWIZZLE_128B,
                            CU_TENSOR_MAP_L2_PROMOTION_L2_128B, CU_TENSOR_MAP_FLOAT_OOB_FILL_NONE);
        if (r != CUDA_SUCCESS) {
            set_error("rollout_lockstep: cuTensorMapEncodeTiled(opponent fc2) failed with %d", (int)r);
            return CEV_ERR_CUDA;
        }
    }

    LsEnvParams& ep = c->ep;
    ep = LsEnvParams{};
    ep.b = b;
    ep.N = N;
    ep.K = p.K;
    ep.E = p.E;
    ep.init_shared = p.init_shared;
    ep.pos_first = p.pos_first;
    ep.init = p.init;
    ep.out = p.out;
    ep.opp_seat[0] = seat_of[0];
    ep.opp_seat[1] = seat_of[1];
    ep.status = p.status;
    c->env_blocks = (int)((N + 255) / 256);

    const int KE = p.K * p.E;
    const int n_chunks = (KE + LS_BT - 1) / LS_BT;
    c->member_ctas = (int64_t)p.P * n_chunks;
    CEV_REQUIRE(c->member_ctas < (1ll << 31), "rollout_lockstep: too many member tiles");

    LsOppParams& op = c->op;
    op = LsOppParams{};
    for (int oi = 0; oi < 2; ++oi) {
        op.opp[oi] = p.opp[oi];
        op.opp_pitch[oi] = p.opp_pitch[oi];
        op.seat[oi] = seat_of[oi];
    }
    op.K = p.K;
    op.E = p.E;
    op.PE = (int64_t)p.P * p.E;
    op.n_tiles = (int)((op.PE + OP_BM - 1) / OP_BM);
    op.n_jobs = 2 * p.K * op.n_tiles;
    op.N = N;
    op.obs = b.obs;
    op.act = b.act;
    op.gap = b.gap;
    op.l1ms = b.l1ms;
    op.oscale = b.oscale;
    op.status = p.status;

    LsMemberTcParams& tp = c->tp;
    tp = LsMemberTcParams{};
    tp.members = p.members;
    tp.pitch = p.member_pitch;
    tp.KE = KE;
    tp.n_chunks = n_chunks;
    tp.seat = ms;
    tp.n_jobs = (int)c->member_ctas;
    tp.N = N;
    tp.obs = b.obs + (int64_t)ms * N * LS_OBS_PAD;
    tp.act = b.act + (int64_t)ms * N;
    tp.gap = b.gap + (int64_t)ms * N;
    tp.l1stats = b.ml1stats;
    tp.status = p.status;
    return CEV_OK;
}

static void ls_launch_member_tc(const LsRoleCtx& c, int grid, cudaStream_t stream) {
    if (c.ms == 0) ls_member_tc_kernel<IN_ADV><<<grid, MT_THREADS, MT_SMEM, stream>>>(c.map_wtc, c.tp);
    else ls_member_tc_kernel<IN_GOOD><<<grid, MT_THREADS, MT_SMEM, stream>>>(c.map_wtc, c.tp);
}

int launch_rollout_lockstep(cev_handle* h, const ClusterParams& p, cudaStream_t stream) {
    if (p.P <= 0 || p.K <= 0 || p.E <= 0) return CEV_OK;
    const int64_t N = (int64_t)p.P * p.K * p.E;
    int rc = ls_reserve(h, ls_carve(nullptr, N, p.K, p.P, nullptr));
    if (rc) return rc;
    rc = ls_configure(h);
    if (rc) return rc;
    LsRoleCtx ctx;
    rc = ls_build_role(h, p, h->ls_workspace, stream, stream, &ctx);
    if (rc) return rc;
    LsEnvParams& ep = ctx.ep;
    LsOppParams& op = ctx.op;
    LsMemberTcParams& tp = ctx.tp;
    const int ms = ctx.ms;
    const int env_blocks = ctx.env_blocks;
    int opp_grid = op.n_jobs < h->n_sm ? op.n_jobs : h->n_sm;
    int mem_grid = tp.n_jobs < h->n_sm ? tp.n_jobs : h->n_sm;
    static const int want_fork = getenv("CEV_LS_FORK") ? atoi(getenv("CEV_LS_FORK")) : 1;
    const bool fork = want_fork && !h->timing_on;
    if (fork) {
        static const int g_opp_env = getenv("CEV_LS_GRID_OPP") ? atoi(getenv("CEV_LS_GRID_OPP")) : LS_GRID_OPP_DEFAULT;
        static const int g_mem_env = getenv("CEV_LS_GRID_MEM") ? atoi(getenv("CEV_LS_GRID_MEM")) : LS_GRID_MEM_DEFAULT;
        int g_opp = 0, g_mem = 0;
        ls_split_sms(h->n_sm, op.n_jobs, tp.n_jobs, &g_opp, &g_mem);
        if (g_opp_env > 0) g_opp = g_opp_env;
        if (g_mem_env > 0) g_mem = g_mem_env;
        if (g_opp < opp_grid) opp_grid = g_opp;
        if (g_mem < mem_grid) mem_grid = g_mem;
    }

    static const int skip = getenv("CEV_LS_SKIP") ? atoi(getenv("CEV_LS_SKIP")) : 0;
    if (fork && !h->side_stream) {
        CEV_CUDA(cudaStreamCreateWithFlags(&h->side_stream, cudaStreamNonBlocking));
        CEV_CUDA(cudaEventCreateWithFlags(&h->fork_ev, cudaEventDisableTiming));
        CEV_CUDA(cudaEventCreateWithFlags(&h->join_ev, cudaEventDisableTiming));
    }
    ep.last = p.n_cycles == 0;
    ls_init_kernel<<<env_blocks, 256, 0, stream>>>(ep);
    for (int c = 0; c < p.n_cycles; ++c) {
        if (p.trace_logits) {
            op.logits = p.trace_logits + (size_t)c * 3 * N * NACT;
            tp.logits = op.logits + (size_t)ms * N * NACT;
        }
        ep.forced = p.trace_forced ? p.trace_forced + (size_t)c * 3 * N : nullptr;
        ep.act_out = p.trace_actions ? p.trace_actions + (size_t)c * 3 * N : nullptr;
        auto tick = [&](int which, int end) {
            if (h->timing_on && h->timing_n[which] < CEV_TIMING_MAX) {
                cudaEventRecord(h->timing_ev[which][2 * h->timing_n[which] + end], stream);
                if (end) ++h->timing_n[which];
            }
        };
        if (!(skip & 1)) {
            if (fork) {
                CEV_CUDA(cudaEventRecord(h->fork_ev, stream));
                CEV_CUDA(cudaStreamWaitEvent(h->side_stream, h->fork_ev, 0));
                ls_opp_kernel<<<opp_grid, OP_THREADS, OP_SMEM, h->side_stream>>>(ctx.map_b, op);
                CEV_CUDA(cudaEventRecord(h->join_ev, h->side_stream));
            } else {
                tick(1, 0);
                ls_opp_kernel<<<opp_grid, OP_THREADS, OP_SMEM, stream>>>(ctx.map_b, op);
                tick(1, 1);
            }
        }
        if (!(skip & 2)) {
            tick(0, 0);
            ls_launch_member_tc(ctx, mem_grid, stream);
            tick(0, 1);
        }
        if (fork && !(skip & 1)) CEV_CUDA(cudaStreamWaitEvent(stream, h->join_ev, 0));
        ep.last = c == p.n_cycles - 1;
        ls_env_step_kernel<<<env_blocks, 256, 0, stream>>>(ep);
    }
    return check_cuda(cudaGetLastError(), "rollout_lockstep launch");
}

int launch_rollout_lockstep_roles(cev_handle* h, const ClusterParams* ps, int n_roles, cudaStream_t stream) {
    if (n_roles <= 0) return CEV_OK;
    const ClusterParams& p0 = ps[0];
    if (p0.P <= 0 || p0.K <= 0 || p0.E <= 0) return CEV_OK;
    static const int want_roles = getenv("CEV_LS_ROLES") ? atoi(getenv("CEV_LS_ROLES")) : 1;
    if (h->timing_on || !want_roles || n_roles > CEV_MAX_ROLES) {
        for (int r = 0; r < n_roles; ++r) {
            const int rc = launch_rollout_lockstep(h, ps[r], stream);
            if (rc) return rc;
        }
        return CEV_OK;
    }
    const int64_t N = (int64_t)p0.P * p0.K * p0.E;
    const size_t per_role = ls_align(ls_carve(nullptr, N, p0.K, p0.P, nullptr));
    int rc = ls_reserve(h, per_role * n_roles);
    if (rc) return rc;
    rc = ls_configure(h);
    if (rc) return rc;
    if (!h->side_stream) {
        CEV_CUDA(cudaStreamCreateWithFlags(&h->side_stream, cudaStreamNonBlocking));
        CEV_CUDA(cudaEventCreateWithFlags(&h->fork_ev, cudaEventDisableTiming));
        CEV_CUDA(cudaEventCreateWithFlags(&h->join_ev, cudaEventDisableTiming));
    }
    if (!h->env_stream) {
        int lo = 0, hi = 0;
        CEV_CUDA(cudaDeviceGetStreamPriorityRange(&lo, &hi));
        const int mid = hi < lo ? lo - 1 : lo;
        static const int prio = getenv("CEV_LS_PRIO") ? atoi(getenv("CEV_LS_PRIO")) : 0;
        const int p_opp = prio == 1 ? lo : mid, p_mem = prio == 2 ? (hi < lo - 1 ? lo - 2 : lo) : lo;
        CEV_CUDA(cudaStreamCreateWithPriority(&h->env_stream, cudaStreamNonBlocking, hi));
        for (int i = 0; i < 3; ++i) CEV_CUDA(cudaStreamCreateWithPriority(&h->opp_stream2[i], cudaStreamNonBlocking, p_opp));
        for (int i = 0; i < 2; ++i) CEV_CUDA(cudaStreamCreateWithPriority(&h->mem_stream2[i], cudaStreamNonBlocking, p_mem));
        for (int r = 0; r < CEV_MAX_ROLES; ++r) {
            CEV_CUDA(cudaEventCreateWithFlags(&h->ev_opp[r], cudaEventDisableTiming));
            CEV_CUDA(cudaEventCreateWithFlags(&h->ev_mem[r], cudaEventDisableTiming));
            CEV_CUDA(cudaEventCreateWithFlags(&h->ev_env[r], cudaEventDisableTiming));
        }
    }
    static const int alt = getenv("CEV_LS_ALT") ? atoi(getenv("CEV_LS_ALT")) : 1;
    static const int skip = getenv("CEV_LS_SKIP") ? atoi(getenv("CEV_LS_SKIP")) : 0;
    static const int ns_env = getenv("CEV_LS_NSTREAMS") ? atoi(getenv("CEV_LS_NSTREAMS")) : 2;
    const int ns = alt ? (ns_env >= 3 ? 3 : 2) : 1;
    cudaStream_t s_mem[3] = {stream, h->mem_stream2[0], h->mem_stream2[1]};
    cudaStream_t s_opp[3] = {h->opp_stream2[0], h->opp_stream2[1], h->opp_stream2[2]};
    cudaStream_t s_env = h->env_stream;
    CEV_CUDA(cudaEventRecord(h->fork_ev, stream));
    for (int k = 0; k < ns; ++k) {
        CEV_CUDA(cudaStreamWaitEvent(s_opp[k], h->fork_ev, 0));
        if (k > 0) CEV_CUDA(cudaStreamWaitEvent(s_mem[k], h->fork_ev, 0));
    }
    CEV_CUDA(cudaStreamWaitEvent(s_env, h->fork_ev, 0));
    LsRoleCtx ctx[CEV_MAX_ROLES];
    for (int r = 0; r < n_roles; ++r) {
        rc = ls_build_role(h, ps[r], static_cast<char*>(h->ls_workspace) + per_role * r, s_opp[r % ns], s_mem[r % ns], &ctx[r]);
        if (rc) return rc;
        ctx[r].ep.last = ps[r].n_cycles == 0;
        ls_init_kernel<<<ctx[r].env_blocks, 256, 0, s_opp[r % ns]>>>(ctx[r].ep);
        CEV_CUDA(cudaEventRecord(h->ev_env[r], s_opp[r % ns]));
    }
    int opp_grid = 0, mem_grid = 0;
    ls_split_sms(h->n_sm, ctx[0].op.n_jobs, ctx[0].tp.n_jobs, &opp_grid, &mem_grid);
    static const int g_opp_env = getenv("CEV_LS_GRID_OPP") ? atoi(getenv("CEV_LS_GRID_OPP")) : LS_GRID_OPP_DEFAULT;
    static const int g_mem_env = getenv("CEV_LS_GRID_MEM") ? atoi(getenv("CEV_LS_GRID_MEM")) : LS_GRID_MEM_DEFAULT;
    if (g_opp_env > 0) opp_grid = g_opp_env;
    if (g_mem_env > 0) mem_grid = g_mem_env;
    if (ctx[0].op.n_jobs < opp_grid) opp_grid = ctx[0].op.n_jobs;
    if (ctx[0].tp.n_jobs < mem_grid) mem_grid = ctx[0].tp.n_jobs;

    const int n_cycles = p0.n_cycles;
    int i = 0;
    for (int c = 0; c < n_cycles; ++c) {
        for (int r = 0; r < n_roles; ++r, ++i) {
            cudaStream_t so = s_opp[i % ns], sm = s_mem[i % ns];
            CEV_CUDA(cudaStreamWaitEvent(so, h->ev_env[r], 0));
            CEV_CUDA(cudaStreamWaitEvent(sm, h->ev_env[r], 0));
            if (!(skip & 1)) ls_opp_kernel<<<opp_grid, OP_THREADS, OP_SMEM, so>>>(ctx[r].map_b, ctx[r].op);
            CEV_CUDA(cudaEventRecord(h->ev_opp[r], so));
            if (!(skip & 2)) ls_launch_member_tc(ctx[r], mem_grid, sm);
            CEV_CUDA(cudaEventRecord(h->ev_mem[r], sm));
            CEV_CUDA(cudaStreamWaitEvent(s_env, h->ev_opp[r], 0));
            CEV_CUDA(cudaStreamWaitEvent(s_env, h->ev_mem[r], 0));
            ctx[r].ep.last = c == n_cycles - 1;
            ls_env_step_kernel<<<ctx[r].env_blocks, 256, 0, s_env>>>(ctx[r].ep);
            CEV_CUDA(cudaEventRecord(h->ev_env[r], s_env));
        }
    }
    CEV_CUDA(cudaEventRecord(h->join_ev, s_env));
    CEV_CUDA(cudaStreamWaitEvent(stream, h->join_ev, 0));
    for (int k = 0; k < ns; ++k) {
        CEV_CUDA(cudaEventRecord(h->ev_opp[k], s_opp[k]));
        CEV_CUDA(cudaStreamWaitEvent(stream, h->ev_opp[k], 0));
        if (k > 0) {
            CEV_CUDA(cudaEventRecord(h->ev_mem[k], s_mem[k]));
            CEV_CUDA(cudaStreamWaitEvent(stream, h->ev_mem[k], 0));
        }
    }
    return check_cuda(cudaGetLastError(), "rollout_lockstep (roles) launch");
}

}
```

### coevonet_b200/engine.py

```python
from __future__ import annotations

import numpy as np
import torch
import torch.distributed as dist

from . import _lib, layout
from .utils import mpe_spec

ROLES = layout.ROLES
N_EVAL_GAMES = 10
HIST_MIN_CAPACITY = 1024


class Shard:

    def __init__(self, P, rank=0, world=1):
        self.P, self.rank, self.world = int(P), int(rank), int(world)
        base, rem = divmod(self.P, self.world)
        self.counts = [base + (1 if r < rem else 0) for r in range(self.world)]
        self.offsets = [sum(self.counts[:r]) for r in range(self.world)]
        self.row0 = self.offsets[self.rank]
        self.n_local = self.counts[self.rank]

    def owner(self, row):
# ... 15 lines not shown
        return self.all_gather_rows_start(local, shard)()

    def all_gather_rows_start(self, local, shard):
        if not self.enabled:
            return lambda: local
        nmax = max(shard.counts)
        tail = tuple(local.shape[1:])
        if local.shape[0] == nmax:
            pad = local.contiguous()
        else:
            pad = torch.zeros((nmax,) + tail, dtype=local.dtype, device=local.device)
            pad[:local.shape[0]] = local
        out = torch.empty((self.world * nmax,) + tail, dtype=local.dtype, device=local.device)
        work = dist.all_gather_into_tensor(out, pad, group=self.group, async_op=True)

        def finish(out=out, pad=pad):
            work.wait()
            if shard.P == self.world * nmax:
                return out
            o = out.view((self.world, nmax) + tail)
            return torch.cat([o[r, :shard.counts[r]] for r in range(self.world)], dim=0)

        return finish

    def all_reduce_sum(self, t):
        if self.enabled:
            dist.all_reduce(t, op=dist.ReduceOp.SUM, group=self.group)
        return t

    def all_reduce_max(self, t):
        if self.enabled:
            dist.all_reduce(t, op=dist.ReduceOp.MAX, group=self.group)
        return t

    def broadcast0(self, t):
        if self.enabled:
            dist.broadcast(t, src=dist.get_global_rank(self.group, 0) if self.group is not None else 0,
                           group=self.group)
        return t


def sync_torch_rng(comm, device="cpu"):
    if not comm.enabled:
        return
    state = torch.get_rng_state()
    dev = torch.device(device)
    buf = state.to(dev) if dev.type == "cuda" else state.clone()
    comm.broadcast0(buf)
    torch.set_rng_state(buf.cpu())


def default_kernels():
    from . import ops
    return ops


def _limit_cycles(k, limit):
    return k.cycles_for_limit(limit)


class _EngineBase:
    kind = "base"

    def __init__(self, args, device, env=None, kernels=None, comm=None):
        self.args = args
        self.device = torch.device(device)
        self.k = kernels if kernels is not None else default_kernels()
        self.comm = comm if comm is not None else Comm()
        self.env = env if env is not None else mpe_spec.DeviceMPEEnv()
        self.seed = int(getattr(args, "seed", mpe_spec.ENV_SEED))
        self.compat = bool(getattr(args, "reference_compat", True))
        self.E = int(getattr(args, "envs_per_member", 1))
        self.pos_first = bool(getattr(args, "integrate_pos_first", True))
        self.init_mode = getattr(args, "init_states", "reference")
        self.status = torch.zeros(1, dtype=torch.int32, device=self.device)
        self.gen = 0
        self.history = [] if getattr(args, "record_history", False) else None
        self.k1_events = None
        self.overlap_roles = bool(getattr(args, "overlap_roles", True)) and self.device.type == "cuda"
        self._role_streams = None
        self._eval_stream = None
        self.fused_roles = bool(getattr(args, "fused_roles", True)) and self.device.type == "cuda"
        self.update_from_members = bool(getattr(args, "update_from_members", True))
        self.order = _lib.ORDER_REFERENCE if self.compat else _lib.ORDER_STABLE_DESC
        self.adaptive = bool(getattr(args, "adaptive", False))
        self.early_stopping = bool(getattr(args, "early_stopping", False))
        self.hist_cap = max(int(getattr(args, "generations", 1)) + 1, HIST_MIN_CAPACITY)
        self.gstate = self.k.generation_state(
            [args.mutation_power_agent_0, args.mutation_power_agent_1, args.mutation_power_adversary],
            self.hist_cap, self.device)
        self._eval_init_tag = 0x40000000
        self._pending_status = []

    def sigma_dev(self, role):
        i = _lib.GS_SIGMA + ROLES.index(role)
        return self.gstate[i:i + 1]

    def sigma(self, role):
        return float(self.gstate[_lib.GS_SIGMA + ROLES.index(role)].item())

    def rollout_variant(self, P_global, K):
        plan = getattr(self.k, "rollout_plan", None)
        if plan is None or self.device.type != "cuda":
            return 0
        used, _ = plan(self.device.index, int(P_global), int(K), self.E, 25)
        return used

    def _initial_states(self, P, K, shard, stream_tag):
        E = self.E
        if self.init_mode == "reference":
            block = self.env.draw_initial_states(P * K * E).reshape(P, K, E, mpe_spec.INIT_STATE_DIM)
            mine = block[shard.row0:shard.row0 + shard.n_local]
            return torch.from_numpy(np.ascontiguousarray(mine)).to(self.device)
        rec0 = shard.row0 * K * E
        out = self.k.init_states(self.seed, stream_tag, shard.n_local * K * E, self.device, rec0=rec0)
        return out.reshape(shard.n_local, K, E, mpe_spec.INIT_STATE_DIM)

    def _post_status(self):
        if self.device.type != "cuda":
            self._pending_status.append((self.status.clone(), None))
            return
        host = torch.empty(1, dtype=torch.int32).pin_memory()
        host.copy_(self.status, non_blocking=True)
        ev = torch.cuda.Event()
        ev.record()
        self._pending_status.append((host, ev))

    def _raise_pending_status(self, keep=1):
        if self.device.type != "cuda":
            keep = 0
        while len(self._pending_status) > keep:
            host, ev = self._pending_status.pop(0)
            if ev is not None:
                ev.synchronize()
            self.k.raise_on_status(host)

    def check_status(self):
        self._raise_pending_status(keep=0)
        self.k.raise_on_status(self.status)

    def _role_slot(self, out, role, limit):
        s0, s1, sadv = self.k.reward_slots(out, agent_step_limit=limit, reference_compat=self.compat)
        return {"agent_0": s0, "agent_1": s1, "adversary_0": sadv}[role]

    def _finish_generation(self, row_a0, row_a1, row_adv):
        a = self.args
        limit = a.max_evaluation_steps
        if self.init_mode == "reference":
            init = torch.from_numpy(self.env.draw_initial_states(N_EVAL_GAMES)).to(self.device)
        else:
            init = self.k.init_states(self.seed, self._eval_init_tag + self.gen, N_EVAL_GAMES, self.device)
        init = init.reshape(1, 1, N_EVAL_GAMES, mpe_spec.INIT_STATE_DIM)

        def body():
            out = self.k.mpe_rollout("agent_0", row_a0.reshape(1, -1), row_adv.reshape(1, -1),
                                     row_a1.reshape(1, -1), init, n_cycles=_limit_cycles(self.k, limit),
                                     pos_first=self.pos_first, status=self.status)
            self.k.generation_end(out, self.gstate, self.hist_cap, agent_step_limit=limit,
                                  reference_compat=self.compat, adaptive=self.adaptive,
                                  sigma_max=a.max_mutation_power, sigma_min=a.min_mutation_power,
                                  early_stopping=self.early_stopping, min_delta=a.min_delta, patience=a.patience)
            self._post_status()

        if self.device.type == "cuda":
            if self._eval_stream is None:
                self._eval_stream = torch.cuda.Stream(device=self.device, priority=-1)
            main = torch.cuda.current_stream(self.device)
            self._eval_stream.wait_stream(main)
            with torch.cuda.stream(self._eval_stream):
                init.record_stream(self._eval_stream)
                body()
        else:
            body()

    def _join_eval(self):
        if self._eval_stream is not None:
            torch.cuda.current_stream(self.device).wait_stream(self._eval_stream)

    def last_eval(self):
        self._join_eval()
        v = self.gstate[_lib.GS_LAST_EVAL:_lib.GS_LAST_EVAL + 3].cpu().tolist()
        return tuple(float(x) for x in v)

    def host_state(self):
        self._join_eval()
        gs = self.gstate.cpu().numpy()
        n = int(gs[_lib.GS_GEN])
        h = gs[_lib.GS_HIST:_lib.GS_HIST + 3 * self.hist_cap].reshape(self.hist_cap, 3)
        sh = gs[_lib.GS_HIST + 3 * self.hist_cap:].reshape(self.hist_cap + 1, 3)
        stop = int(gs[_lib.GS_STOP])
        return {"generations": n, "sigma": {r: float(gs[_lib.GS_SIGMA + i]) for i, r in enumerate(ROLES)},
                "rewards": {r: h[:min(n, self.hist_cap), i].copy() for i, r in enumerate(ROLES)},
                "sigma_history": {r: sh[:min(n, self.hist_cap) + 1, i].copy() for i, r in enumerate(ROLES)},
                "best": {r: float(gs[_lib.GS_BEST + i]) for i, r in enumerate(ROLES)},
                "stale": {r: int(gs[_lib.GS_STALE + i]) for i, r in enumerate(ROLES)},
                "stop_role": ROLES[stop - 1] if stop else None, "stop_generation": int(gs[_lib.GS_STOP_GEN])}

    def write_back_args(self):
        s = self.host_state()["sigma"]
        self.args.mutation_power_agent_0 = s["agent_0"]
        self.args.mutation_power_agent_1 = s["agent_1"]
        self.args.mutation_power_adversary = s["adversary_0"]

    def should_stop(self):
        self._join_eval()
        flag = self.gstate[_lib.GS_STOP:_lib.GS_STOP + 1].clone()
        self.comm.all_reduce_max(flag)
        return int(flag.item())

    def _run_roles(self, fn):
        if self.overlap_roles and self.k1_events is None:
            if self._role_streams is None:
                self._role_streams = [torch.cuda.Stream(device=self.device) for _ in ROLES]
            main = torch.cuda.current_stream(self.device)
            for role, st in zip(ROLES, self._role_streams):
                st.wait_stream(main)
                with torch.cuda.stream(st):
                    fn(role)
            for st in self._role_streams:
                main.wait_stream(st)
        else:
            for role in ROLES:
                fn(role)

    def _rollouts(self, specs, limit):
        n_cycles = _limit_cycles(self.k, limit)
        if self.fused_roles and self.k1_events is None and hasattr(self.k, "mpe_rollout_roles") and len(specs) > 1:
            outs = self.k.mpe_rollout_roles(specs, n_cycles=n_cycles, pos_first=self.pos_first, status=self.status,
                                            variant=self.variant)
            return {spec[0]: out for spec, out in zip(specs, outs)}
        res = {}

        def one(role):
            spec = next(sp for sp in specs if sp[0] == role)
            if self.k1_events is not None:
                e0 = torch.cuda.Event(enable_timing=True)
                e1 = torch.cuda.Event(enable_timing=True)
                e0.record()
            res[role] = self.k.mpe_rollout(role, spec[1], spec[2], spec[3], spec[4], n_cycles=n_cycles,
                                           pos_first=self.pos_first, status=self.status, variant=self.variant)
            if self.k1_events is not None:
                e1.record()
                self.k1_events.append((e0, e1))

        self._run_roles(one)
        return res

    def _base_state(self):
        self._join_eval()
        return {"kind": self.kind, "gen": self.gen, "seed": self.seed, "P": self.P, "world": self.comm.world,
                "row0": self.shard.row0, "n_local": self.shard.n_local, "hist_cap": self.hist_cap,
                "gstate": self.gstate.cpu(), "env": self.env.state_dict() if hasattr(self.env, "state_dict") else None}

    def _load_base_state(self, sd):
        if sd["kind"] != self.kind:
            raise ValueError(f"checkpoint holds a {sd['kind']} engine, this is {self.kind}")
        if int(sd["P"]) != self.P:
            raise ValueError(f"checkpoint population {sd['P']} != {self.P}")
        if int(sd["seed"]) != self.seed:
            raise ValueError("checkpoint was written with another seed")
        self.gen = int(sd["gen"])
        gs = sd["gstate"].to(torch.float64)
        if int(sd["hist_cap"]) != self.hist_cap:
            old = int(sd["hist_cap"])
            new = self.k.generation_state([0, 0, 0], self.hist_cap, "cpu")
            new[:_lib.GS_HIST] = gs[:_lib.GS_HIST]
            n = min(old, self.hist_cap)
            new[_lib.GS_HIST:_lib.GS_HIST + 3 * n] = gs[_lib.GS_HIST:_lib.GS_HIST + 3 * n]
            so, sn = _lib.GS_HIST + 3 * old, _lib.GS_HIST + 3 * self.hist_cap
            new[sn:sn + 3 * (n + 1)] = gs[so:so + 3 * (n + 1)]
            gs = new
        self.gstate.copy_(gs.to(self.device))
        if sd.get("env") is not None and hasattr(self.env, "load_state_dict"):
            self.env.load_state_dict(sd["env"])
        self._pending_status = []


class GAEngine(_EngineBase):

    kind = "GA"

    def __init__(self, args, device, pop_rows, hof_rows, founder_rows, env=None, kernels=None, comm=None):
        super().__init__(args, device, env, kernels, comm)
        self.P = int(args.population)
        self.shard = Shard(self.P, self.comm.rank, self.comm.world)
        self.pop = {r: pop_rows[r].to(self.device).contiguous() for r in ROLES}
        self.hof = {r: hof_rows[r].to(self.device).contiguous() for r in ROLES}
        self.founder = {r: founder_rows[r].to(self.device).contiguous() for r in ROLES}
        for r in ROLES:
            self.comm.broadcast0(self.hof[r])
            self.comm.broadcast0(self.founder[r])
        self.elites = {r: None for r in ROLES}
        self.elite_ids = {r: None for r in ROLES}
        self.fitness = {r: None for r in ROLES}
        self.diversity = {r: None for r in ROLES}
        for r in ROLES:
            assert self.pop[r].shape[0] == self.shard.n_local, "population shard has the wrong row count"
        if int(args.elites_number) > self.P or int(args.elites_number) < 1:
            raise ValueError(f"elites_number must be in [1, population]: {args.elites_number} vs {self.P}")
        K_eff = 1 if (self.compat and not getattr(args, "play_discarded_hof_games", False)) else int(args.hof_size)
        self.variant = self.rollout_variant(self.P, K_eff)

    def _opponents(self, role):
        newest_first = {r: torch.flip(self.hof[r], dims=[0]).contiguous() for r in ROLES}
        if role == "agent_0":
            return newest_first["adversary_0"], newest_first["agent_1"]
        if role == "agent_1":
            return newest_first["adversary_0"], newest_first["agent_0"]
        second = newest_first["agent_0"] if self.compat else newest_first["agent_1"]
        return newest_first["agent_0"], second

    def _rollout_spec(self, role, init):
# ... 61 lines not shown
        E = int(a.elites_number)
        pitches = [layout.fc_pitch(layout.OBS_DIM[r]) for r in ROLES]
        cat = torch.empty(E * sum(pitches), dtype=torch.float32, device=self.device)
        views, off = {}, 0
        for r, pitch in zip(ROLES, pitches):
            views[r] = cat[off:off + E * pitch].view(E, pitch)
            off += E * pitch
        for role in ROLES:
            ids = self.k.select_topk(self.fitness[role], E, order=self.order)
            self.elite_ids[role] = ids
            self.k.gather_rows(self.pop[role], ids, row0=self.shard.row0, n_local=self.shard.n_local,
                               out=views[role])
        self.comm.all_reduce_sum(cat)
        for role in ROLES:
            in_dim = layout.OBS_DIM[role]
            elites = views[role]
            self.elites[role] = elites
            self.hof[role] = torch.cat([self.hof[role][1:], elites[0:1]], dim=0).contiguous()
            self.k.ga_repopulate(elites, layout.fc_dim(in_dim), self.sigma_dev(role), self.seed, role, self.gen,
                                 self.shard.row0, self.shard.n_local, out=self.pop[role],
                                 crossover_rate=float(getattr(a, "crossover_rate", 0.0)))

    def step(self, sync=True):
        self._raise_pending_status()
        if self.adaptive:
            self._join_eval()
        self.evaluate()
        self.select_and_repopulate()
        best = {r: self.elites[r][0] for r in ROLES}
        self._finish_generation(best["agent_0"], best["agent_1"], best["adversary_0"])
        if self.history is not None:
            hs = self.host_state()
            self.check_status()
            self.history.append(dict(
                fitness={r: self.fitness[r].cpu().numpy().copy() for r in ROLES},
                elite_ids={r: self.elite_ids[r].cpu().numpy().copy() for r in ROLES},
                diversity={r: float(self.diversity[r]) for r in ROLES}, evals=self.last_eval(),
                sigma={r: float(hs["sigma_history"][r][self.gen]) for r in ROLES}))
        self.gen += 1
        return self.last_eval() if sync else None

    def state_dict(self):
        sd = self._base_state()
        sd.update(pop={r: self.pop[r].cpu() for r in ROLES}, hof={r: self.hof[r].cpu() for r in ROLES},
                  founder={r: self.founder[r].cpu() for r in ROLES})
        return sd

    def load_state_dict(self, sd):
        self._load_base_state(sd)
        if int(sd["row0"]) != self.shard.row0 or int(sd["n_local"]) != self.shard.n_local:
            raise ValueError("checkpoint shard does not match this rank's row block (same world size needed)")
        for r in ROLES:
            self.pop[r].copy_(sd["pop"][r])
            self.hof[r] = sd["hof"][r].to(self.device).contiguous()
            self.founder[r].copy_(sd["founder"][r])


class ESEngine(_EngineBase):

    kind = "ES"

    def __init__(self, args, device, theta_rows, env=None, kernels=None, comm=None):
        super().__init__(args, device, env, kernels, comm)
        self.P = int(args.population)
        self.shard = Shard(self.P, self.comm.rank, self.comm.world)
        pitches = [layout.fc_pitch(layout.OBS_DIM[r]) for r in ROLES]
        self.theta_cat = torch.empty(sum(pitches), dtype=torch.float32, device=self.device)
        self.delta_cat = torch.zeros(sum(pitches), dtype=torch.float32, device=self.device)
        self.theta, self.last_delta, off = {}, {}, 0
        for r, pitch in zip(ROLES, pitches):
            self.theta[r] = self.theta_cat[off:off + pitch]
            self.last_delta[r] = self.delta_cat[off:off + pitch]
            self.theta[r].copy_(theta_rows[r].reshape(-1)[:pitch])
            off += pitch
        self.comm.broadcast0(self.theta_cat)
        self.members = {r: torch.empty((self.shard.n_local, layout.fc_pitch(layout.OBS_DIM[r])),
                                       dtype=torch.float32, device=self.device) for r in ROLES}
        self.fitness = {r: None for r in ROLES}
        self.rewards = {r: None for r in ROLES}
        self.diversity = {r: None for r in ROLES}
        self.weight_stats = {r: None for r in ROLES}
        self.member_stats = bool(getattr(args, "log_member_weight_stats", False))
        self.variant = self.rollout_variant(self.P, 1)

    def _base_opponents(self, role):
        t = self.theta
        if role == "agent_0":
            return t["adversary_0"].reshape(1, -1), t["agent_1"].reshape(1, -1)
        if role == "agent_1":
            return t["adversary_0"].reshape(1, -1), t["agent_0"].reshape(1, -1)
        return t["agent_0"].reshape(1, -1), t["agent_1"].reshape(1, -1)

    def _reference_initial_states(self):
        E = self.E
        block = self.env.draw_initial_states(self.P * 3 * E).reshape(self.P, 3, E, mpe_spec.INIT_STATE_DIM)
        sl = slice(self.shard.row0, self.shard.row0 + self.shard.n_local)
        return {r: torch.from_numpy(np.ascontiguousarray(block[sl, i][:, None])).to(self.device)
                for i, r in enumerate(ROLES)}

    def evaluate(self, init_by_role=None):
        limit = self.args.max_timesteps_per_episode
        ref_init = init_by_role
        if ref_init is None and self.init_mode == "reference":
            ref_init = self._reference_initial_states()

        specs = {}

        def prepare(role):
            in_dim = layout.OBS_DIM[role]
            self.k.es_perturb(self.theta[role], in_dim, self.sigma_dev(role), self.seed, role, self.gen,
                              self.shard.row0, self.shard.n_local, out=self.members[role])
            if self.member_stats:
                self.weight_stats[role] = self.k.weight_stats(self.members[role], in_dim)
            if ref_init is not None:
                init = ref_init[role]
            else:
                init = self._initial_states(self.P, 1, self.shard, ROLES.index(role) + 4 * self.gen)
            opp_a, opp_b = self._base_opponents(role)
            specs[role] = (role, self.members[role], opp_a, opp_b, init)

        self._run_roles(prepare)
        outs = self._rollouts([specs[r] for r in ROLES], limit)
        for role in ROLES:
            slot = self._role_slot(outs[role], role, limit)
            self.rewards[role] = slot.mean(dim=(1, 2)).contiguous()

    def update(self):
        a = self.args
        fit_local = {r: self.rewards[r].to(torch.float32).to(torch.float64) for r in ROLES}
        cols = [fit_local[r] for r in ROLES]
        if a.fitness_sharing:
            cols += [self.k.diversity_dist(self.members[r], self.theta[r], layout.OBS_DIM[r]).to(torch.float64)
                     for r in ROLES]
        packed = torch.stack(cols, dim=1).contiguous()
        start = getattr(self.comm, "all_gather_rows_start", None)
        if start is not None:
            gathered = start(packed, self.shard)
        else:
            _all = self.comm.all_gather_rows(packed, self.shard)
            gathered = lambda: _all

        def finish_fitness():
            allp = gathered()
            for i, role in enumerate(ROLES):
                if a.fitness_sharing:
                    div = self.k.diversity_from_dist(allp[:, 3 + i].to(torch.float32))
                    self.diversity[role] = div
                    fit_local[role] = (fit_local[role].to(torch.float32) / (1 + div)).to(torch.float64)
                    self.fitness[role] = (allp[:, i].to(torch.float32) / (1 + div)).to(torch.float64)
                else:
                    self.fitness[role] = allp[:, i].contiguous()

        if a.fitness_sharing:
            finish_fitness()
        for role in ROLES:
            in_dim = layout.OBS_DIM[role]
            if self.update_from_members and hasattr(self.k, "es_update_members"):
                self.k.es_update_members(fit_local[role].contiguous(), self.members[role], self.theta[role],
                                         in_dim, self.sigma_dev(role), a.learning_rate, self.P,
                                         out=self.last_delta[role])
            else:
                self.k.es_update(fit_local[role].contiguous(), in_dim, self.sigma_dev(role), a.learning_rate,
                                 self.P, self.seed, role, self.gen, self.shard.row0, out=self.last_delta[role])
        if not a.fitness_sharing:
            finish_fitness()
        self.comm.all_reduce_sum(self.delta_cat)
        self._join_eval()
        self.k.axpy(1.0, self.delta_cat, self.theta_cat)

    def step(self, init_by_role=None, sync=True):
        self._raise_pending_status()
        if self.adaptive:
            self._join_eval()
        self.evaluate(init_by_role)
        self.update()
        self._finish_generation(self.theta["agent_0"], self.theta["agent_1"], self.theta["adversary_0"])
        if self.history is not None:
            hs = self.host_state()
            self.check_status()
            rewards_all = {r: self.comm.all_gather_rows(self.rewards[r], self.shard).cpu().numpy().copy()
                           for r in ROLES}
            self.history.append(dict(
                rewards=rewards_all,
                diversity={r: (float(self.diversity[r]) if self.diversity[r] is not None else None) for r in ROLES},
                evals=self.last_eval(),
                delta={r: self.last_delta[r].cpu().numpy().copy() for r in ROLES},
                sigma={r: float(hs["sigma_history"][r][self.gen]) for r in ROLES}))
        self.gen += 1
        return self.last_eval() if sync else None

    def state_dict(self):
        sd = self._base_state()
        sd.update(theta={r: self.theta[r].cpu().clone() for r in ROLES})
        return sd
# ... 23 lines not shown
```

### coevonet_b200/ops.py

```python
from __future__ import annotations

import ctypes

import torch

from . import _lib, layout
from ._lib import RolloutCfg, check, handle, load

MAX_CYCLES = 25

_KERNELS_PER_CALL = {"cev_es_update_f32": 2, "cev_es_update_members_f32": 2, "cev_fp32_peak": 4}
launch_count = 0


def _call(name, *args, launches=None):
    global launch_count
    launch_count += _KERNELS_PER_CALL.get(name, 1) if launches is None else launches
    return getattr(load(), name)(*args)


def rollout_plan(device_index, P, K, E, n_cycles=25, variant=0):
    used, n = ctypes.c_int(), ctypes.c_int()
    check(load().cev_mpe_rollout_plan(handle(device_index), int(P), int(K), int(E), int(n_cycles),
                                      int(variant), ctypes.byref(used), ctypes.byref(n)),
# ... 18 lines not shown
    for t in tensors:
        if t is None:
            continue
        if not t.is_cuda:
            raise _lib.CevError("coevonet_b200 ops need CUDA tensors (no CPU fallback)")
        if not t.is_contiguous():
            raise _lib.CevError("coevonet_b200 ops need contiguous tensors")
        dev = t.device if dev is None else dev
        if t.device != dev:
            raise _lib.CevError("all tensors of one op must live on the same device")
    return dev


def cycles_for_limit(agent_step_limit):
    if agent_step_limit is None:
        return MAX_CYCLES
    return int(min(MAX_CYCLES, max(0, int(agent_step_limit)) // 3))


def reward_slots(out, agent_step_limit=None, reference_compat=True):
    sg, lg, sa = out[..., 0], out[..., 1], out[..., 2]
    if not reference_compat:
        return sg, sg, sa
    L = 75 if agent_step_limit is None else int(min(75, max(0, int(agent_step_limit))))
    nc = L // 3
    if nc == 0:
        z = torch.zeros_like(sg)
        return z, sa, z
    n_adv = -(-L // 3)
    n_a0 = -(-(L - 1) // 3)
    slot_adv = sg if n_adv - 1 >= nc else sg - lg
    slot_a0 = sg if n_a0 - 1 >= nc else sg - lg
    return slot_a0, sa, slot_adv


def raise_on_status(status):
    code = int(status.item())
    if code & _lib.STATUS_NONFINITE:
        raise ValueError("\n\t Warning: output contains inf or NaN")


def kernel_timing_enable(device_index, on=True):
    check(load().cev_kernel_timing_enable(handle(device_index), int(bool(on))), "cev_kernel_timing_enable")


def kernel_timing_read(device_index, which):
    ms, n = ctypes.c_double(), ctypes.c_int()
    check(load().cev_kernel_timing_read(handle(device_index), int(which), ctypes.byref(ms), ctypes.byref(n)),
          "cev_kernel_timing_read")
    return ms.value, n.value


def mpe_rollout(member_role, members, opp_a, opp_b, init, *, n_cycles=MAX_CYCLES,
                pos_first=True, init_shared=False, variant=0, out=None, status=None):
    dev = _need_cuda(members, opp_a, opp_b, init, out, status)
    seat = layout.SEAT_OF[member_role] if isinstance(member_role, str) else int(member_role)
    P, K = members.shape[0], opp_a.shape[0]
    if opp_b.shape[0] != K:
        raise _lib.CevError("opp_a and opp_b must hold the same number of rows")
    if init_shared:
        if init.dim() != 3 or init.shape[0] != K or init.shape[2] != _lib.INIT_STATE_DIM:
            raise _lib.CevError("shared init must be fp64 [K, E, 11]")
        E = init.shape[1]
    else:
        if init.dim() != 4 or init.shape[:2] != (P, K) or init.shape[3] != _lib.INIT_STATE_DIM:
            raise _lib.CevError("init must be fp64 [P, K, E, 11]")
        E = init.shape[2]
    if members.dtype != torch.float32 or init.dtype != torch.float64:
        raise _lib.CevError("members must be float32 and init float64")
    if out is None:
        out = torch.empty((P, K, E, _lib.ROLLOUT_OUT_DIM), dtype=torch.float64, device=dev)
    if P == 0:
        return out
    cfg = RolloutCfg(int(n_cycles), int(bool(pos_first)), int(variant), 0)
    _, n_launch = rollout_plan(dev.index, P, K, E, n_cycles, variant)
    check(_call("cev_mpe_rollout_f32",
        _h(dev), seat, _ptr(members), P, members.stride(0),
        _ptr(opp_a), opp_a.stride(0), _ptr(opp_b), opp_b.stride(0), K,
        _ptr(init), int(bool(init_shared)), E, ctypes.byref(cfg), _ptr(out), _ptr(status),
        _stream(dev), launches=n_launch), "cev_mpe_rollout_f32")
    return out


def mpe_rollout_roles(roles, *, n_cycles=MAX_CYCLES, pos_first=True, init_shared=False, variant=0, status=None):
    outs, recs, keep = [], (_lib.RolloutRole * len(roles))(), []
    P = K = E = None
    dev = None
    for i, (member_role, members, opp_a, opp_b, init) in enumerate(roles):
        dev = _need_cuda(members, opp_a, opp_b, init, status)
        seat = layout.SEAT_OF[member_role] if isinstance(member_role, str) else int(member_role)
        p_, k_ = members.shape[0], opp_a.shape[0]
        e_ = init.shape[1] if init_shared else init.shape[2]
        if opp_b.shape[0] != k_:
            raise _lib.CevError("opp_a and opp_b must hold the same number of rows")
        if (init_shared and (init.dim() != 3 or init.shape[0] != k_)) or \
                (not init_shared and (init.dim() != 4 or tuple(init.shape[:2]) != (p_, k_))) or \
                init.shape[-1] != _lib.INIT_STATE_DIM:
            raise _lib.CevError("init must be fp64 [P, K, E, 11] (or [K, E, 11] with init_shared)")
        if members.dtype != torch.float32 or init.dtype != torch.float64:
            raise _lib.CevError("members must be float32 and init float64")
        if P is None:
            P, K, E = p_, k_, e_
        elif (P, K, E) != (p_, k_, e_):
            raise _lib.CevError("every role must have the same P, K, E")
        out = torch.empty((p_, k_, e_, _lib.ROLLOUT_OUT_DIM), dtype=torch.float64, device=dev)
        outs.append(out)
        keep.append((members, opp_a, opp_b, init))
        r = recs[i]
        r.member_seat, r.reserved = seat, 0
        r.members, r.member_pitch = members.data_ptr(), members.stride(0)
        r.opp_a, r.opp_a_pitch = opp_a.data_ptr(), opp_a.stride(0)
        r.opp_b, r.opp_b_pitch = opp_b.data_ptr(), opp_b.stride(0)
        r.init, r.out = init.data_ptr(), out.data_ptr()
    if not roles or P == 0:
        return outs
    cfg = RolloutCfg(int(n_cycles), int(bool(pos_first)), int(variant), 0)
    _, n_launch = rollout_plan(dev.index, P, K, E, n_cycles, variant)
    check(_call("cev_mpe_rollout_roles_f32", _h(dev), len(roles), recs, P, K, int(bool(init_shared)), E,
                ctypes.byref(cfg), _ptr(status), _stream(dev), launches=n_launch * len(roles)),
          "cev_mpe_rollout_roles_f32")
    return outs


def mpe_rollout_trace(member_role, members, opp_a, opp_b, init, *, n_cycles=MAX_CYCLES, pos_first=True,
                      forced_actions=None, status=None):
    dev = _need_cuda(members, opp_a, opp_b, init, forced_actions, status)
    seat = layout.SEAT_OF[member_role] if isinstance(member_role, str) else int(member_role)
    P, K = members.shape[0], opp_a.shape[0]
    if init.dim() != 4 or init.shape[:2] != (P, K) or init.shape[3] != _lib.INIT_STATE_DIM:
        raise _lib.CevError("init must be fp64 [P, K, E, 11]")
    E = init.shape[2]
    N = P * K * E
    if forced_actions is not None and (forced_actions.dtype != torch.int32 or
                                       tuple(forced_actions.shape) != (n_cycles, 3, N)):
        raise _lib.CevError("forced_actions must be int32 [n_cycles, 3, N]")
    out = torch.empty((P, K, E, _lib.ROLLOUT_OUT_DIM), dtype=torch.float64, device=dev)
    logits = torch.zeros((n_cycles, 3, N, layout.NACT), dtype=torch.float32, device=dev)
    actions = torch.zeros((n_cycles, 3, N), dtype=torch.int32, device=dev)
    cfg = RolloutCfg(int(n_cycles), int(bool(pos_first)), 3, 0)
    check(_call("cev_mpe_rollout_trace_f32", _h(dev), seat, _ptr(members), P, members.stride(0),
                _ptr(opp_a), opp_a.stride(0), _ptr(opp_b), opp_b.stride(0), K, _ptr(init), 0, E,
                ctypes.byref(cfg), _ptr(forced_actions), _ptr(logits), _ptr(actions), _ptr(out), _ptr(status),
                _stream(dev), launches=3 + 3 * int(n_cycles)), "cev_mpe_rollout_trace_f32")
    return out, logits, actions


def mpe_rollout_indexed(w_adv, w_a0, w_a1, idx, init, *, n_cycles=MAX_CYCLES, pos_first=True,
                        out=None, status=None):
    dev = _need_cuda(w_adv, w_a0, w_a1, idx, init, out, status)
    N = idx.shape[0]
    if idx.dtype != torch.int32 or init.dtype != torch.float64 or init.shape != (N, _lib.INIT_STATE_DIM):
        raise _lib.CevError("idx must be int32 [N,3] and init fp64 [N,11]")
    if out is None:
        out = torch.empty((N, _lib.ROLLOUT_OUT_DIM), dtype=torch.float64, device=dev)
    cfg = RolloutCfg(int(n_cycles), int(bool(pos_first)), 1, 0)
    check(_call("cev_mpe_rollout_indexed_f32", 
        _h(dev), _ptr(w_adv), w_adv.stride(0), _ptr(w_a0), w_a0.stride(0),
        _ptr(w_a1), w_a1.stride(0), _ptr(idx), _ptr(init), N, ctypes.byref(cfg), _ptr(out),
        _ptr(status), _stream(dev)), "cev_mpe_rollout_indexed_f32")
    return out


def fc_forward(rows, in_dim, obs, idx=None, *, status=None):
    dev = _need_cuda(rows, obs, idx, status)
    N = obs.shape[0]
    if obs.dtype != torch.float32 or obs.shape[1] != in_dim:
        raise _lib.CevError("fc_forward: obs must be float32 [N, in_dim]")
    if idx is not None and idx.dtype != torch.int32:
        raise _lib.CevError("fc_forward: idx must be int32")
    logits = torch.empty((N, layout.NACT), dtype=torch.float32, device=dev)
    actions = torch.empty(N, dtype=torch.int32, device=dev)
    check(_call("cev_fc_forward_f32", _h(dev), _ptr(rows), rows.stride(0), int(in_dim), _ptr(idx),
                                    _ptr(obs), N, _ptr(logits), _ptr(actions), _ptr(status), _stream(dev)),
          "cev_fc_forward_f32")
    return logits, actions


def _sigma_args(sigma):
    if torch.is_tensor(sigma):
        if sigma.dtype != torch.float64 or sigma.numel() != 1 or not sigma.is_cuda:
            raise _lib.CevError("a device sigma must be a one-element float64 CUDA tensor")
        return 0.0, _ptr(sigma)
    return float(sigma), ctypes.c_void_p(0)


def ga_repopulate(elites, dim, sigma, seed, role, gen, row0, n_rows, *, out=None, noise_out=None,
                  crossover_rate=0.0):
    dev = _need_cuda(elites, out, noise_out)
    sig, sig_dev = _sigma_args(sigma)
    pitch = elites.stride(0)
    if out is None:
        out = torch.empty((n_rows, pitch), dtype=torch.float32, device=dev)
    role_id = layout.ROLE_ID[role] if isinstance(role, str) else int(role)
    check(_call("cev_ga_repopulate_f32", 
        _h(dev), _ptr(elites), elites.shape[0], int(dim), pitch, sig, sig_dev, float(crossover_rate),
        int(seed), role_id, int(gen), int(row0), int(n_rows), _ptr(out), _ptr(noise_out),
        _stream(dev)), "cev_ga_repopulate_f32")
    return out


def gather_rows(src, idx, *, row0=0, n_local=None, out=None):
    dev = _need_cuda(idx, out, src if src.numel() else None)
    if idx.dtype != torch.int64:
        raise _lib.CevError("gather_rows: idx must be int64")
    pitch = src.stride(0) if src.dim() == 2 and src.shape[0] > 0 else src.shape[-1]
    if out is None:
        out = torch.empty((idx.shape[0], pitch), dtype=torch.float32, device=dev)
    check(_call("cev_gather_rows_f32", _h(dev), _ptr(src) if src.numel() else ctypes.c_void_p(0), pitch, _ptr(idx),
                idx.shape[0], int(row0), -1 if n_local is None else int(n_local), _ptr(out), _stream(dev)),
          "cev_gather_rows_f32")
    return out


def select_topk(fitness, k, order=_lib.ORDER_STABLE_DESC):
    dev = _need_cuda(fitness)
    if fitness.dtype != torch.float64 or fitness.dim() != 1:
        raise _lib.CevError("select_topk: fitness must be float64 [P]")
    idx = torch.empty(k, dtype=torch.int64, device=dev)
    check(_call("cev_select_topk_f64", _h(dev), _ptr(fitness), fitness.shape[0], int(k), int(order),
                                     _ptr(idx), _stream(dev)), "cev_select_topk_f64")
    return idx


def es_perturb(theta, in_dim, sigma, seed, role, gen, row0, n_rows, *, out=None, noise_out=None):
    dev = _need_cuda(theta, out, noise_out)
    pitch = layout.fc_pitch(in_dim)
    if theta.numel() < pitch:
        raise _lib.CevError("es_perturb: theta must be a padded flat row")
    if out is None:
        out = torch.empty((n_rows, pitch), dtype=torch.float32, device=dev)
    role_id = layout.ROLE_ID[role] if isinstance(role, str) else int(role)
    sig, sig_dev = _sigma_args(sigma)
    check(_call("cev_es_perturb_f32", 
        _h(dev), _ptr(theta), int(in_dim), sig, sig_dev, int(seed), role_id, int(gen),
        int(row0), int(n_rows), pitch, _ptr(out), _ptr(noise_out), _stream(dev)), "cev_es_perturb_f32")
    return out


def es_perturb_dqn(theta, c_in, n_actions, sigma, seed, role, gen, row0, n_rows, *, out=None):
    dev = _need_cuda(theta, out)
    pitch, total = layout.dqn_pitch(c_in, n_actions), layout.dqn_dim(c_in, n_actions)
    d_pert = total - 2 * (32 + 64 + 64)
    if theta.numel() < pitch:
        raise _lib.CevError("es_perturb_dqn: theta must be a padded flat row")
    if out is None:
        out = torch.empty((n_rows, pitch), dtype=torch.float32, device=dev)
    role_id = layout.ROLE_ID[role] if isinstance(role, str) else int(role)
    sig, sig_dev = _sigma_args(sigma)
    check(_call("cev_es_perturb_prefix_f32", _h(dev), _ptr(theta), d_pert, total, sig, sig_dev, int(seed), role_id,
                int(gen), int(row0), int(n_rows), pitch, _ptr(out), _stream(dev)), "cev_es_perturb_prefix_f32")
    return out


def es_update(fitness, in_dim, sigma, lr, n_total, seed, role, gen, row0, *, out=None):
    dev = _need_cuda(fitness, out)
    if fitness.dtype != torch.float64:
        raise _lib.CevError("es_update: fitness must be float64")
    pitch = layout.fc_pitch(in_dim)
    if out is None:
        out = torch.empty(pitch, dtype=torch.float32, device=dev)
    role_id = layout.ROLE_ID[role] if isinstance(role, str) else int(role)
    sig, sig_dev = _sigma_args(sigma)
    check(_call("cev_es_update_f32", 
        _h(dev), _ptr(fitness), int(in_dim), sig, sig_dev, float(lr), int(n_total),
        int(seed), role_id, int(gen), int(row0), fitness.shape[0], _ptr(out), _stream(dev)),
        "cev_es_update_f32")
    return out


def es_update_members(fitness, members, theta, in_dim, sigma, lr, n_total, *, out=None):
    dev = _need_cuda(theta, out, fitness if fitness.numel() else None, members if members.numel() else None)
    if fitness.dtype != torch.float64 or fitness.shape[0] != members.shape[0]:
        raise _lib.CevError("es_update_members: fitness must be float64 [n_rows]")
    pitch = layout.fc_pitch(in_dim) if in_dim else members.stride(0)
    if (members.shape[0] > 0 and members.stride(0) != pitch) or theta.numel() < pitch:
        raise _lib.CevError("es_update_members: members / theta must use the padded row pitch")
    if out is None:
        out = torch.empty(pitch, dtype=torch.float32, device=dev)
    sig, sig_dev = _sigma_args(sigma)
    empty = members.shape[0] == 0
    check(_call("cev_es_update_members_f32", _h(dev), ctypes.c_void_p(0) if empty else _ptr(fitness),
                ctypes.c_void_p(0) if empty else _ptr(members), pitch, _ptr(theta),
                int(in_dim), sig, sig_dev, float(lr), int(n_total), members.shape[0], _ptr(out), _stream(dev)),
          "cev_es_update_members_f32")
    return out


def weight_stats(rows, in_dim, *, out=None):
    n = rows.shape[0]
    if out is None:
        out = torch.empty((n, 4), dtype=torch.float32, device=rows.device)
    if n == 0:
        return out
    dev = _need_cuda(rows, out)
    check(_call("cev_weight_stats_f32", _h(dev), _ptr(rows), n, rows.stride(0), int(in_dim), _ptr(out),
                _stream(dev)), "cev_weight_stats_f32")
    return out


def generation_state(sigmas, hist_capacity, device):
    n = int(load().cev_generation_state_doubles(int(hist_capacity)))
    gs = torch.zeros(n, dtype=torch.float64)
    gs[_lib.GS_SIGMA:_lib.GS_SIGMA + 3] = torch.tensor([float(x) for x in sigmas], dtype=torch.float64)
    gs[_lib.GS_BEST:_lib.GS_BEST + 3] = float("-inf")
    sh = _lib.GS_HIST + 3 * int(hist_capacity)
    gs[sh:sh + 3] = gs[_lib.GS_SIGMA:_lib.GS_SIGMA + 3]
    return gs.to(device)


def generation_end(eval_out, gstate, hist_capacity, *, agent_step_limit=None, reference_compat=True,
                   adaptive=False, sigma_max=0.5, sigma_min=0.001, early_stopping=False, min_delta=0.1,
                   patience=300):
    dev = _need_cuda(eval_out, gstate)
    if eval_out.dtype != torch.float64 or gstate.dtype != torch.float64:
        raise _lib.CevError("generation_end: eval_out and gstate must be float64")
    n_games = eval_out.numel() // _lib.ROLLOUT_OUT_DIM
    check(_call("cev_generation_end_f64", _h(dev), _ptr(eval_out), n_games,
                -1 if agent_step_limit is None else int(agent_step_limit), int(bool(reference_compat)),
# ... 113 lines not shown
```

### include/coevonet_b200.h

```cpp
#ifndef COEVONET_B200_H
#define COEVONET_B200_H

#include <stdint.h>

#ifdef __cplusplus
extern "C" {
#endif

typedef struct cev_handle cev_handle;
typedef void* cev_stream;

#define CEV_OK 0
#define CEV_ERR_ARG (-1)
#define CEV_ERR_CUDA (-2)
#define CEV_ERR_UNSUPPORTED (-3)

#define CEV_STATUS_NONFINITE 1

#define CEV_SEAT_ADVERSARY 0
#define CEV_SEAT_AGENT_0 1
#define CEV_SEAT_AGENT_1 2

#define CEV_INIT_STATE_DIM 11
#define CEV_ROLLOUT_OUT_DIM 4

#define CEV_KIND_ES 0
#define CEV_KIND_GA 1
#define CEV_KIND_ENV 2
#define CEV_KIND_FRAMES 3
#define CEV_KIND_INIT 4
#define CEV_KIND_XOVER 5

int cev_version(void);
const char* cev_last_error(void);
int cev_create(int device, cev_handle** out);
int cev_destroy(cev_handle* h);
int cev_device_info(cev_handle* h, int* n_sm, int* n_clusters);

int cev_fc_dim(int in_dim);
int cev_fc_pitch(int in_dim);
int cev_dqn_dim(int c_in, int n_actions);
int cev_dqn_pitch(int c_in, int n_actions);

typedef struct {
    int32_t n_cycles;
    int32_t integrate_pos_first;
    int32_t variant;
    int32_t reserved;
} cev_rollout_cfg;

int cev_mpe_rollout_f32(cev_handle* h, int member_seat,
                        const float* members, int P, int64_t member_pitch,
                        const float* opp_a, int64_t opp_a_pitch,
                        const float* opp_b, int64_t opp_b_pitch, int K,
                        const double* init, int init_shared, int E,
                        const cev_rollout_cfg* cfg,
                        double* out, int32_t* status, cev_stream stream);

typedef struct {
    int32_t member_seat;
    int32_t reserved;
    const float* members;
    int64_t member_pitch;
    const float* opp_a;
    int64_t opp_a_pitch;
    const float* opp_b;
    int64_t opp_b_pitch;
    const double* init;
    double* out;
} cev_rollout_role;

int cev_mpe_rollout_roles_f32(cev_handle* h, int n_roles, const cev_rollout_role* roles,
                              int P, int K, int init_shared, int E,
                              const cev_rollout_cfg* cfg, int32_t* status, cev_stream stream);

int cev_mpe_rollout_trace_f32(cev_handle* h, int member_seat,
                              const float* members, int P, int64_t member_pitch,
                              const float* opp_a, int64_t opp_a_pitch,
                              const float* opp_b, int64_t opp_b_pitch, int K,
                              const double* init, int init_shared, int E,
                              const cev_rollout_cfg* cfg,
                              const int32_t* forced_actions, float* logits_out, int32_t* actions_out,
                              double* out, int32_t* status, cev_stream stream);

int cev_mpe_rollout_plan(cev_handle* h, int P, int K, int E, int n_cycles, int variant,
                         int* variant_used, int* n_launches);

int cev_kernel_timing_enable(cev_handle* h, int on);
int cev_kernel_timing_read(cev_handle* h, int which, double* total_ms, int* n_launches);

int cev_mpe_rollout_indexed_f32(cev_handle* h,
                                const float* w_adv, int64_t adv_pitch,
                                const float* w_a0, int64_t a0_pitch,
                                const float* w_a1, int64_t a1_pitch,
                                const int32_t* idx, const double* init, int N,
                                const cev_rollout_cfg* cfg,
                                double* out, int32_t* status, cev_stream stream);

int cev_fc_forward_f32(cev_handle* h, const float* rows, int64_t pitch, int in_dim,
                       const int32_t* idx, const float* obs, int64_t N,
                       float* logits, int32_t* actions, int32_t* status, cev_stream stream);

int cev_ga_repopulate_f32(cev_handle* h, const float* elites, int E,
                          int D, int64_t pitch, float sigma, const double* sigma_dev,
                          float crossover_rate,
                          uint64_t seed, int role, uint32_t gen,
                          int64_t row0, int64_t n_rows,
                          float* out, float* noise_out, cev_stream stream);

int cev_gather_rows_f32(cev_handle* h, const float* src, int64_t pitch,
                        const int64_t* idx, int n, int64_t row0, int64_t n_local,
                        float* dst, cev_stream stream);

#define CEV_ORDER_STABLE_DESC 0
#define CEV_ORDER_REFERENCE 1
int cev_select_topk_f64(cev_handle* h, const double* fitness, int64_t P, int k, int order,
                        int64_t* idx_out, cev_stream stream);

int cev_es_perturb_f32(cev_handle* h, const float* theta, int in_dim,
                       float sigma, const double* sigma_dev, uint64_t seed, int role, uint32_t gen,
                       int64_t row0, int64_t n_rows, int64_t pitch,
                       float* out, float* noise_out, cev_stream stream);

int cev_es_perturb_prefix_f32(cev_handle* h, const float* theta, int64_t d_pert, int64_t d_total, float sigma,
                              const double* sigma_dev, uint64_t seed, int role, uint32_t gen, int64_t row0,
                              int64_t n_rows, int64_t pitch, float* out, cev_stream stream);

int cev_es_update_f32(cev_handle* h, const double* fitness, int in_dim,
                      float sigma, const double* sigma_dev, float lr, int64_t n_total,
                      uint64_t seed, int role, uint32_t gen,
                      int64_t row0, int64_t n_rows,
                      float* delta, cev_stream stream);

int cev_es_update_members_f32(cev_handle* h, const double* fitness, const float* members, int64_t pitch,
                              const float* theta, int in_dim, float sigma, const double* sigma_dev, float lr,
                              int64_t n_total, int64_t n_rows, float* delta, cev_stream stream);

int cev_axpy_f32(cev_handle* h, float a, const float* x, float* y, int64_t n, cev_stream stream);

int cev_diversity_dist_f32(cev_handle* h, const float* pop, int64_t n_rows,
                           int64_t pitch, const float* ref, int in_dim,
                           float* dist, cev_stream stream);

int cev_weight_stats_f32(cev_handle* h, const float* rows, int64_t n_rows, int64_t pitch, int in_dim,
                         float* out, cev_stream stream);

#define CEV_GS_GEN 0
#define CEV_GS_SIGMA 1
#define CEV_GS_BEST 4
#define CEV_GS_STALE 7
#define CEV_GS_STOP 10
#define CEV_GS_STOP_GEN 11
#define CEV_GS_LAST_EVAL 12
#define CEV_GS_HIST 16
int cev_generation_state_doubles(int hist_capacity);
int cev_generation_end_f64(cev_handle* h, const double* eval_out, int n_games, int agent_step_limit,
                           int reference_compat, double* gstate, int hist_capacity, int adaptive,
                           double sigma_max, double sigma_min, int early_stopping, double min_delta,
                           int patience, cev_stream stream);

int cev_deepqn_forward(cev_handle* h, const float* members, int P, int64_t pitch,
                       const uint8_t* frames, int B, int c_in, int n_actions,
                       float* logits, int32_t* actions, cev_stream stream);

int cev_atari_synth_step_u8(cev_handle* h, uint64_t seed, int64_t ep0, int64_t n, int t,
                            const int32_t* a_first, const int32_t* a_second, uint8_t* ring,
                            float* r_first, cev_stream stream);
int cev_atari_observe_u8(cev_handle* h, const uint8_t* ring, int64_t n, int t, int seat,
                         uint8_t* obs, cev_stream stream);

int cev_fc_init_f32(cev_handle* h, int in_dim, uint64_t seed, int role, int64_t row0, int64_t n_rows,
                    int64_t pitch, float* out, cev_stream stream);

int cev_init_states_f64(cev_handle* h, uint64_t seed, uint32_t stream_id,
                        int64_t rec0, int64_t n, double* out, cev_stream stream);
int cev_random_frames_u8(cev_handle* h, uint64_t seed, int64_t n_bytes,
                         uint8_t* out, cev_stream stream);
int cev_philox_words(cev_handle* h, uint64_t seed, int kind, int role, uint32_t gen,
                     int64_t member0, int64_t n_members, int64_t n4,
                     uint32_t* out, cev_stream stream);

int cev_fp32_peak(cev_handle* h, int mode, double* tflops, cev_stream stream);

#ifdef __cplusplus
}
#endif
#endif
```

Before: 131.7 million.

## Feed member-stage tensor-core MMA with pre-split fp16 weights instead of tf32

The ES perturb step can now also write a pre-split half-precision copy of each member's fc2 weights (two fp16 parts plus a per-row exponent). The rollout member kernel then loads these parts straight into the shared-memory ring by TMA and runs kind::f16 tcgen05 MMAs, replacing tf32 MMAs over a split that was previously staged through tensor memory by producer warps. This removes the in-kernel split work and cuts operand bytes and tensor-memory use, at the cost of an extra split buffer per role, a second kernel path, and a numerical scheme that depends on the two-part fp16 split keeping enough precision.

```diff
diff --git a/coevonet_b200/_lib.py b/coevonet_b200/_lib.py
--- a/coevonet_b200/_lib.py
+++ b/coevonet_b200/_lib.py
@@ -51,6 +51,8 @@
                                     c_void_p, c_void_p, c_void_p]),
     "cev_mpe_rollout_roles_f32": (c_int, [c_void_p, c_int, POINTER(RolloutRole), c_int, c_int, c_int, c_int,
                                           POINTER(RolloutCfg), c_void_p, c_void_p]),
+    "cev_mpe_rollout_roles_split_f32": (c_int, [c_void_p, c_int, POINTER(RolloutRole), POINTER(c_void_p), c_int, c_int,
+                                                c_int, c_int, POINTER(RolloutCfg), c_void_p, c_void_p]),
     "cev_mpe_rollout_trace_f32": (c_int, [c_void_p, c_int, c_void_p, c_int, c_int64,
                                           c_void_p, c_int64, c_void_p, c_int64, c_int,
                                           c_void_p, c_int, c_int, POINTER(RolloutCfg),
@@ -71,6 +73,10 @@
     "cev_select_topk_f64": (c_int, [c_void_p, c_void_p, c_int64, c_int, c_int, c_void_p, c_void_p]),
     "cev_es_perturb_f32": (c_int, [c_void_p, c_void_p, c_int, c_float, c_void_p, c_uint64, c_int, c_uint32,
                                    c_int64, c_int64, c_int64, c_void_p, c_void_p, c_void_p]),
+    "cev_es_perturb_split_f32": (c_int, [c_void_p, c_void_p, c_int, c_float, c_void_p, c_uint64, c_int, c_uint32,
+                                         c_int64, c_int64, c_int64, c_void_p, c_void_p, c_void_p, c_void_p]),
+    "cev_member_split_bytes": (c_int64, [c_int64]),
+    "cev_member_split_f32": (c_int, [c_void_p, c_int, c_void_p, c_int64, c_int64, c_void_p, c_void_p]),
     "cev_es_perturb_prefix_f32": (c_int, [c_void_p, c_void_p, c_int64, c_int64, c_float, c_void_p, c_uint64, c_int,
                                           c_uint32, c_int64, c_int64, c_int64, c_void_p, c_void_p]),
     "cev_es_update_f32": (c_int, [c_void_p, c_void_p, c_int, c_float, c_void_p, c_float, c_int64,
diff --git a/coevonet_b200/csrc/api.cu b/coevonet_b200/csrc/api.cu
--- a/coevonet_b200/csrc/api.cu
+++ b/coevonet_b200/csrc/api.cu
@@ -189,6 +189,27 @@
 
 int cev_mpe_rollout_roles_f32(cev_handle* h, int n_roles, const cev_rollout_role* roles, int P, int K, int init_shared,
                               int E, const cev_rollout_cfg* cfg, int32_t* status, cev_stream stream) {
+    return cev_mpe_rollout_roles_split_f32(h, n_roles, roles, nullptr, P, K, init_shared, E, cfg, status, stream);
+}
+
+int64_t cev_member_split_bytes(int64_t P) { return P < 0 ? 0 : member_split_bytes_api(P); }
+
+int cev_member_split_f32(cev_handle* h, int member_seat, const float* members, int64_t P, int64_t pitch,
+                         void* member_split, cev_stream stream) {
+    CEV_REQUIRE(h != nullptr, "member_split: null handle");
+    if (P == 0) return CEV_OK;
+    CEV_REQUIRE(members && member_split, "member_split: null pointer");
+    CEV_REQUIRE(member_seat >= 0 && member_seat <= 2, "member_split: member_seat must be 0..2");
+    CEV_REQUIRE(P > 0 && P < (1ll << 31), "member_split: need 0 <= P < 2^31");
+    CEV_REQUIRE(pitch >= fc_offsets(seat_in_dim(member_seat)).total && pitch % 4 == 0, "member_split: bad pitch");
+    CEV_REQUIRE(aligned16(members) && aligned16(member_split), "member_split: 16B alignment");
+    CEV_GUARD(h);
+    return launch_member_split(member_seat, members, P, pitch, member_split, (cudaStream_t)stream);
+}
+
+int cev_mpe_rollout_roles_split_f32(cev_handle* h, int n_roles, const cev_rollout_role* roles,
+                                    const void* const* member_split, int P, int K, int init_shared, int E,
+                                    const cev_rollout_cfg* cfg, int32_t* status, cev_stream stream) {
     CEV_REQUIRE(h && roles, "mpe_rollout_roles: null pointer");
     CEV_REQUIRE(n_roles >= 1 && n_roles <= CEV_MAX_ROLES, "mpe_rollout_roles: n_roles must be 1..%d", CEV_MAX_ROLES);
     CEV_REQUIRE(P >= 0 && K >= 1 && E >= 1, "mpe_rollout_roles: need P >= 0, K >= 1, E >= 1");
@@ -237,6 +258,8 @@
         p.status = status;
         p.n_cycles = cfg->n_cycles;
         p.pos_first = cfg->integrate_pos_first;
+        p.member_split = member_split ? member_split[r] : nullptr;
+        CEV_REQUIRE(aligned16(p.member_split), "mpe_rollout_roles: member_split must be 16B aligned");
     }
     CEV_GUARD(h);
     return launch_rollout_lockstep_roles(h, ps, n_roles, (cudaStream_t)stream);
diff --git a/coevonet_b200/csrc/common.cuh b/coevonet_b200/csrc/common.cuh
--- a/coevonet_b200/csrc/common.cuh
+++ b/coevonet_b200/csrc/common.cuh
@@ -295,6 +295,7 @@
     double* out;
     int32_t* status;
     int n_cycles, pos_first;
+    const void* member_split;
     const int32_t* trace_forced;
     float* trace_logits;
     int32_t* trace_actions;
@@ -304,6 +305,9 @@
 int rollout_cluster_max_clusters(int device);
 int launch_rollout_lockstep(cev_handle* h, const ClusterParams& p, cudaStream_t stream);
 int launch_rollout_lockstep_roles(cev_handle* h, const ClusterParams* ps, int n_roles, cudaStream_t stream);
+int64_t member_split_bytes_api(int64_t P);
+int launch_member_split(int member_seat, const float* members, int64_t P, int64_t pitch, void* split,
+                        cudaStream_t stream);
 int rollout_lockstep_launches(int n_cycles);
 int launch_deepqn_fc_tc(cev_handle* h, const float* members, int64_t pitch, int P, int B, int n_act, int f1w_off,
                         int f1b_off, int ow_off, int ob_off, const float* act3, float* logits, int32_t* actions,
diff --git a/coevonet_b200/csrc/ls_member_tc.cuh b/coevonet_b200/csrc/ls_member_tc.cuh
--- a/coevonet_b200/csrc/ls_member_tc.cuh
+++ b/coevonet_b200/csrc/ls_member_tc.cuh
@@ -6,57 +6,57 @@
 constexpr int MT_PROD_WARPS = 8;
 constexpr int MT_BK = 32, MT_KT = H1 / MT_BK;
 constexpr int MT_NB = LS_BT;
-constexpr int MT_R = 5, MT_L = 3;
-constexpr uint32_t MT_A_BYTES = H2 * MT_BK * 4;
-constexpr uint32_t MT_X_BYTES = MT_NB * MT_BK * 4;
-constexpr uint32_t MT_XSLOT = 2 * MT_X_BYTES;
+constexpr int MT_R = 5;
+constexpr uint32_t MT_PART_BYTES = H2 * MT_BK * 2;
+constexpr uint32_t MT_SLOT_BYTES = 2 * MT_PART_BYTES;
+constexpr uint32_t MT_ROW_BYTES = MT_BK * 2;
+constexpr uint32_t MT_XSLOT = 2 * MT_NB * MT_ROW_BYTES;
 constexpr uint32_t MT_W1C_FLOATS = MT_BK * IN_GOOD + 3 * MT_BK;
 constexpr uint32_t MT_W1C_BYTES = MT_W1C_FLOATS * 4;
 constexpr uint32_t MT_TAIL_BYTES = LS_TAIL_FLOATS * 4;
-constexpr size_t MT_OFF_X = (size_t)MT_R * MT_A_BYTES;
-constexpr size_t MT_OFF_W1C = MT_OFF_X + (size_t)MT_L * MT_XSLOT;
+constexpr size_t MT_OFF_X = (size_t)MT_R * MT_SLOT_BYTES;
+constexpr size_t MT_OFF_W1C = MT_OFF_X + (size_t)MT_R * MT_XSLOT;
 constexpr size_t MT_OFF_HS = MT_OFF_W1C + (size_t)MT_R * MT_W1C_BYTES;
 constexpr size_t MT_OFF_TAIL = MT_OFF_HS + (size_t)H2 * MT_NB * 4;
-constexpr size_t MT_OFF_OBS = MT_OFF_TAIL + MT_TAIL_BYTES;
+constexpr size_t MT_OFF_EXP = MT_OFF_TAIL + MT_TAIL_BYTES;
+constexpr size_t MT_OFF_OBS = MT_OFF_EXP + H2;
 constexpr size_t MT_OFF_STAT = MT_OFF_OBS + 2 * MT_NB * LS_OBS_PAD * 4;
 constexpr size_t MT_OFF_RED = MT_OFF_STAT + 2 * MT_NB * 8;
 constexpr size_t MT_OFF_BAR = MT_OFF_RED + (size_t)(2 + NACT) * 4 * MT_NB * 4;
 constexpr size_t MT_SMEM = MT_OFF_BAR + 256 + 1024 ;
 constexpr int MT_ACC = 2 * MT_NB;
-constexpr int MT_TM_OP = 2 * 2 * MT_ACC;
-constexpr int MT_TM_SLOT = 2 * 2 * MT_BK;
-static_assert(MT_TM_OP + MT_L * MT_TM_SLOT <= 512, "tensor memory budget");
-static_assert(MT_OFF_X % 1024 == 0 && MT_XSLOT % 1024 == 0, "operand tiles must keep the 1024-byte alignment of the swizzle atoms");
-static_assert(MT_OFF_W1C % 16 == 0 && MT_W1C_BYTES % 16 == 0 && MT_OFF_TAIL % 16 == 0 && MT_OFF_BAR % 8 == 0,
+constexpr uint32_t MT_TMEM_COLS = 2 * 2 * MT_ACC;
+static_assert(MT_OFF_X % 1024 == 0 && MT_XSLOT % 512 == 0 && MT_PART_BYTES % 1024 == 0,
+              "operand tiles must keep the alignment of the swizzle atoms");
+static_assert(MT_OFF_W1C % 16 == 0 && MT_W1C_BYTES % 16 == 0 && MT_OFF_TAIL % 16 == 0 && MT_OFF_EXP % 16 == 0 &&
+                  MT_OFF_BAR % 8 == 0,
               "bulk-copy alignment");
 static_assert(MT_SMEM <= 232448, "member stage exceeds the 227 KB shared-memory limit");
-constexpr uint32_t MT_IDESC32 = (1u << 4) | (2u << 7) | (2u << 10) | ((uint32_t)((2 * MT_NB) >> 3) << 17) |
-                                ((uint32_t)(128 >> 4) << 24);
-
-__device__ __forceinline__ void mt_issue_ktile(uint32_t d_tmem, uint32_t a_tmem, uint64_t x_hilo, uint32_t accumulate,
-                                               uint32_t bar_op) {
+constexpr uint32_t MT_IDESC_X12 = (1u << 4) | ((uint32_t)(2 * MT_NB >> 3) << 17) | ((uint32_t)(128 >> 4) << 24);
+constexpr uint32_t MT_IDESC_X1 = (1u << 4) | ((uint32_t)(MT_NB >> 3) << 17) | ((uint32_t)(128 >> 4) << 24);
+
+__device__ __forceinline__ uint64_t umma_desc_sw64(uint32_t smem_addr) {
+    return (uint64_t)((smem_addr >> 4) & 0x3FFFu) | ((uint64_t)1 << 16) | ((uint64_t)(512 >> 4) << 32) |
+           ((uint64_t)1 << 46) | ((uint64_t)4 << 61);
+}
+
+__device__ __forceinline__ void mt_issue_ktile(uint32_t d_tmem, uint64_t a_w1, uint64_t a_w2, uint64_t b_x,
+                                               uint32_t accumulate, uint32_t bar_empty) {
     asm volatile(
         "{\n"
         ".reg .pred pe, pa, pt;\n"
-        ".reg .b64 b1, b2, b3;\n"
-        ".reg .b32 h1, h2, h3, l0, l1, l2, l3;\n"
+        ".reg .b64 a1, a2, b1;\n"
         "elect.sync _|pe, 0xffffffff;\n"
-        "setp.ne.b32 pa, %3, 0;\n"
+        "setp.ne.b32 pa, %4, 0;\n"
         "setp.eq.b32 pt, 0, 0;\n"
-        "add.s64 b1, %2, 2;\n add.s64 b2, %2, 4;\n add.s64 b3, %2, 6;\n"
-        "add.u32 h1, %1, 8;\n add.u32 h2, %1, 16;\n add.u32 h3, %1, 24;\n"
-        "add.u32 l0, %1, 32;\n add.u32 l1, %1, 40;\n add.u32 l2, %1, 48;\n add.u32 l3, %1, 56;\n"
-        "@pe tcgen05.mma.cta_group::1.kind::tf32 [%0], [l0], %2, %5, pa;\n"
-        "@pe tcgen05.mma.cta_group::1.kind::tf32 [%0], [%1], %2, %5, pt;\n"
-        "@pe tcgen05.mma.cta_group::1.kind::tf32 [%0], [l1], b1, %5, pt;\n"
-        "@pe tcgen05.mma.cta_group::1.kind::tf32 [%0], [h1], b1, %5, pt;\n"
-        "@pe tcgen05.mma.cta_group::1.kind::tf32 [%0], [l2], b2, %5, pt;\n"
-        "@pe tcgen05.mma.cta_group::1.kind::tf32 [%0], [h2], b2, %5, pt;\n"
-        "@pe tcgen05.mma.cta_group::1.kind::tf32 [%0], [l3], b3, %5, pt;\n"
-        "@pe tcgen05.mma.cta_group::1.kind::tf32 [%0], [h3], b3, %5, pt;\n"
-        "@pe tcgen05.commit.cta_group::1.mbarrier::arrive::one.shared::cluster.b64 [%4];\n"
+        "add.s64 a1, %1, 2;\n add.s64 a2, %2, 2;\n add.s64 b1, %3, 2;\n"
+        "@pe tcgen05.mma.cta_group::1.kind::f16 [%0], %1, %3, %6, pa;\n"
+        "@pe tcgen05.mma.cta_group::1.kind::f16 [%0], %2, %3, %7, pt;\n"
+        "@pe tcgen05.mma.cta_group::1.kind::f16 [%0], a1, b1, %6, pt;\n"
+        "@pe tcgen05.mma.cta_group::1.kind::f16 [%0], a2, b1, %7, pt;\n"
+        "@pe tcgen05.commit.cta_group::1.mbarrier::arrive::one.shared::cluster.b64 [%5];\n"
         "}\n" ::"r"(d_tmem),
-        "r"(a_tmem), "l"(x_hilo), "r"(accumulate), "r"(bar_op), "r"(MT_IDESC32)
+        "l"(a_w1), "l"(a_w2), "l"(b_x), "r"(accumulate), "r"(bar_empty), "r"(MT_IDESC_X12), "r"(MT_IDESC_X1)
         : "memory");
 }
 struct LsMemberTcParams {
@@ -68,6 +68,8 @@
     int32_t* act;
     float* gap;
     const double* l1stats;
+    const int32_t* sx;
+    const int8_t* wexp;
     int32_t* status;
     float* logits;
 };
@@ -77,21 +79,21 @@
 ls_member_tc_kernel(const __grid_constant__ CUtensorMap map_w, const LsMemberTcParams p) {
     extern __shared__ unsigned char mt_raw[];
     unsigned char* base = mt_raw + ((1024u - (tc_smem_u32(mt_raw) & 1023u)) & 1023u);
-    unsigned char* raw_mem = base;
+    unsigned char* ring = base;
     unsigned char* x_mem = base + MT_OFF_X;
     float* hs = reinterpret_cast<float*>(base + MT_OFF_HS);
     unsigned char* w1c_mem = base + MT_OFF_W1C;
     float* tail = reinterpret_cast<float*>(base + MT_OFF_TAIL);
+    const int8_t* wexp = reinterpret_cast<const int8_t*>(base + MT_OFF_EXP);
     float* obsbuf = reinterpret_cast<float*>(base + MT_OFF_OBS);
     float2* statbuf = reinterpret_cast<float2*>(base + MT_OFF_STAT);
     float* redA = reinterpret_cast<float*>(base + MT_OFF_RED);
     float* redB = redA + 4 * MT_NB;
     float* redC = redB + 4 * MT_NB;
-    uint64_t* bar_raw_full = reinterpret_cast<uint64_t*>(base + MT_OFF_BAR);
-    uint64_t* bar_raw_empty = bar_raw_full + MT_R;
-    uint64_t* bar_lo_full = bar_raw_empty + MT_R;
-    uint64_t* bar_lo_empty = bar_lo_full + MT_L;
-    uint64_t* bar_tfull = bar_lo_empty + MT_L;
+    uint64_t* bar_in = reinterpret_cast<uint64_t*>(base + MT_OFF_BAR);
+    uint64_t* bar_full = bar_in + MT_R;
+    uint64_t* bar_empty = bar_full + MT_R;
+    uint64_t* bar_tfull = bar_empty + MT_R;
     uint64_t* bar_tempty = bar_tfull + 2;
     uint64_t* bar_stat_full = bar_tempty + 2;
     uint64_t* bar_tail_full = bar_stat_full + 2;
@@ -107,12 +109,9 @@
     if (threadIdx.x == 0) {
         *flag = 0;
         for (int i = 0; i < MT_R; ++i) {
-            tc_mbar_init(bar_raw_full + i, 1);
-            tc_mbar_init(bar_raw_empty + i, MT_PROD_WARPS / 2);
-        }
-        for (int i = 0; i < MT_L; ++i) {
-            tc_mbar_init(bar_lo_full + i, MT_PROD_WARPS / 2);
-            tc_mbar_init(bar_lo_empty + i, 2);
+            tc_mbar_init(bar_in + i, 1);
+            tc_mbar_init(bar_full + i, 1 + MT_PROD_WARPS / 2);
+            tc_mbar_init(bar_empty + i, 2);
         }
         for (int i = 0; i < 2; ++i) {
             tc_mbar_init(bar_tfull + i, 2);
@@ -125,7 +124,7 @@
     }
     if (warp == 1) {
         asm volatile("tcgen05.alloc.cta_group::1.sync.aligned.shared::cta.b32 [%0], %1;\n" ::"r"(tc_smem_u32(tmem_slot)),
-                     "r"(512u)
+                     "r"(MT_TMEM_COLS)
                      : "memory");
         asm volatile("tcgen05.relinquish_alloc_permit.cta_group::1.sync.aligned;\n" ::: "memory");
     }
@@ -142,22 +141,27 @@
                 const float* mrow = p.members + (int64_t)m * p.pitch;
                 for (int kt = 0; kt < MT_KT; ++kt, ++it) {
                     const uint32_t rs = it % MT_R, use = it / MT_R;
-                    if (use > 0) tc_mbar_wait(bar_raw_empty + rs, (use - 1) & 1);
-                    tc_mbar_expect_tx(bar_raw_full + rs, MT_A_BYTES + W1ROWS_BYTES + 3 * MT_BK * 4);
-                    tma_load_3d(raw_mem + (size_t)rs * MT_A_BYTES, &map_w, bar_raw_full + rs, kt * MT_BK, 0, m);
+                    if (use > 0) tc_mbar_wait(bar_empty + rs, (use - 1) & 1);
+                    tc_mbar_expect_tx(bar_in + rs, W1ROWS_BYTES + 3 * MT_BK * 4);
                     float* c = reinterpret_cast<float*>(w1c_mem + (size_t)rs * MT_W1C_BYTES);
-                    bulk_g2s(c, mrow + kt * MT_BK * IN, W1ROWS_BYTES, bar_raw_full + rs);
-                    bulk_g2s(c + MT_BK * IN, mrow + om.fc1b + kt * MT_BK, MT_BK * 4, bar_raw_full + rs);
-                    bulk_g2s(c + MT_BK * IN + MT_BK, mrow + om.ln1g + kt * MT_BK, MT_BK * 4, bar_raw_full + rs);
-                    bulk_g2s(c + MT_BK * IN + 2 * MT_BK, mrow + om.ln1b + kt * MT_BK, MT_BK * 4, bar_raw_full + rs);
+                    bulk_g2s(c, mrow + kt * MT_BK * IN, W1ROWS_BYTES, bar_in + rs);
+                    bulk_g2s(c + MT_BK * IN, mrow + om.fc1b + kt * MT_BK, MT_BK * 4, bar_in + rs);
+                    bulk_g2s(c + MT_BK * IN + MT_BK, mrow + om.ln1g + kt * MT_BK, MT_BK * 4, bar_in + rs);
+                    bulk_g2s(c + MT_BK * IN + 2 * MT_BK, mrow + om.ln1b + kt * MT_BK, MT_BK * 4, bar_in + rs);
+                    unsigned char* slot = ring + (size_t)rs * MT_SLOT_BYTES;
+                    tc_mbar_expect_tx(bar_full + rs, MT_SLOT_BYTES);
+                    tma_load_3d(slot, &map_w, bar_full + rs, kt * MT_BK, 0, m);
+                    tma_load_3d(slot + MT_PART_BYTES, &map_w, bar_full + rs, kt * MT_BK, H2, m);
                 }
                 if (js >= 1) tc_mbar_wait(bar_tail_empty, (js - 1) & 1);
-                tc_mbar_expect_tx(bar_tail_full, MT_TAIL_BYTES);
+                tc_mbar_expect_tx(bar_tail_full, MT_TAIL_BYTES + H2);
                 bulk_g2s(tail, mrow + om.fc2b, MT_TAIL_BYTES, bar_tail_full);
+                bulk_g2s(base + MT_OFF_EXP, p.wexp + (int64_t)m * H2, H2, bar_tail_full);
             }
         }
     } else if (warp == 1 || warp == 14) {
         const int t = warp == 1 ? 0 : 1;
+        const uint32_t ring_base = tc_smem_u32(ring) + t * (128 * MT_ROW_BYTES);
         const uint32_t x_base = tc_smem_u32(x_mem);
         uint32_t it = 0, js = 0;
         for (int job = job0; job < p.n_jobs; job += job_stride, ++js) {
@@ -166,12 +170,12 @@
             asm volatile("tcgen05.fence::after_thread_sync;\n" ::: "memory");
             const uint32_t d_tmem = tmem_base + as * (2 * MT_ACC) + t * MT_ACC;
             for (int kt = 0; kt < MT_KT; ++kt, ++it) {
-                const uint32_t ls = it % MT_L, luse = it / MT_L;
-                const uint64_t x_hilo = umma_desc_sw128(x_base + ls * MT_XSLOT);
-                const uint32_t a_tmem = tmem_base + MT_TM_OP + ls * MT_TM_SLOT + t * (2 * MT_BK);
-                tc_mbar_wait(bar_lo_full + ls, luse & 1);
+                const uint32_t rs = it % MT_R, use = it / MT_R;
+                const uint32_t a_w1 = ring_base + rs * MT_SLOT_BYTES;
+                tc_mbar_wait(bar_full + rs, use & 1);
                 asm volatile("tcgen05.fence::after_thread_sync;\n" ::: "memory");
-                mt_issue_ktile(d_tmem, a_tmem, x_hilo, kt ? 1u : 0u, tc_smem_u32(bar_lo_empty + ls));
+                mt_issue_ktile(d_tmem, umma_desc_sw64(a_w1), umma_desc_sw64(a_w1 + MT_PART_BYTES),
+                               umma_desc_sw64(x_base + rs * MT_XSLOT), kt ? 1u : 0u, tc_smem_u32(bar_empty + rs));
                 if (kt == MT_KT - 1) tc_commit_elected(tc_smem_u32(bar_tfull + as));
                 __syncwarp();
             }
@@ -179,9 +183,8 @@
     } else if (warp < 2 + MT_PROD_WARPS) {
         const int grp = (warp - 2) >> 2;
         const int pt = (threadIdx.x - 64) & 127;
-        const int q = warp & 3;
-        const int r = q * 32 + lane;
         const int e = pt & 15, g = pt >> 4;
+        const int xoff = e * MT_ROW_BYTES + ((((g >> 1) ^ ((e >> 1) & 3))) << 4) + (g & 1) * 8;
         uint32_t it = 0, js = 0;
         for (int job = job0; job < p.n_jobs; job += job_stride, ++js) {
             const uint32_t b = js & 1, buse = js >> 1;
@@ -198,67 +201,48 @@
             }
             const float2 st = statbuf[b * MT_NB + e];
             const float mean = st.x, rstd = st.y;
+            const float sx = ldexpf(1.0f, __ldg(p.sx + job / p.n_chunks));
             for (int kt = 0; kt < MT_KT; ++kt, ++it) {
                 if ((int)(it & 1) != grp) continue;
-                const uint32_t rs = it % MT_R, ruse = it / MT_R, ls = it % MT_L, luse = it / MT_L;
-                const unsigned char* slot = raw_mem + (size_t)rs * MT_A_BYTES;
-                unsigned char* xs = x_mem + (size_t)ls * MT_XSLOT;
-                if (luse > 0) tc_mbar_wait(bar_lo_empty + ls, (luse - 1) & 1);
-                tc_mbar_wait(bar_raw_full + rs, ruse & 1);
-                asm volatile("tcgen05.fence::after_thread_sync;\n" ::: "memory");
-#pragma unroll
-                for (int t = 0; t < 2; ++t) {
-                    const float4* row = reinterpret_cast<const float4*>(slot + (size_t)(t * 128 + r) * 128);
-                    float w[32];
-#pragma unroll
-                    for (int c = 0; c < 8; ++c) {
-                        const float4 v = row[c ^ (r & 7)];
-                        w[4 * c] = v.x;
-                        w[4 * c + 1] = v.y;
-                        w[4 * c + 2] = v.z;
-                        w[4 * c + 3] = v.w;
+                const uint32_t rs = it % MT_R, use = it / MT_R;
+                unsigned char* xs = x_mem + (size_t)rs * MT_XSLOT;
+                if (use > 0) tc_mbar_wait(bar_empty + rs, (use - 1) & 1);
+                tc_mbar_wait(bar_in + rs, use & 1);
+                const float* w1c = reinterpret_cast<const float*>(w1c_mem + (size_t)rs * MT_W1C_BYTES);
+                const int kl = g * 4;
+                const float4 bb = *reinterpret_cast<const float4*>(w1c + MT_BK * IN + kl);
+                const float4 gg = *reinterpret_cast<const float4*>(w1c + MT_BK * IN + MT_BK + kl);
+                const float4 ee = *reinterpret_cast<const float4*>(w1c + MT_BK * IN + 2 * MT_BK + kl);
+                const float bq[4] = {bb.x, bb.y, bb.z, bb.w}, gq[4] = {gg.x * sx, gg.y * sx, gg.z * sx, gg.w * sx},
+                            eq[4] = {ee.x * sx, ee.y * sx, ee.z * sx, ee.w * sx};
+                float h[4];
+#pragma unroll
+                for (int qq = 0; qq < 4; ++qq) {
+                    const float2* wr = reinterpret_cast<const float2*>(w1c + (kl + qq) * IN);
+                    float pre = 0.f;
+#pragma unroll
+                    for (int i2 = 0; i2 < IN / 2; ++i2) {
+                        const float2 v = wr[i2];
+                        pre = fmaf(v.x, x[2 * i2], pre);
+                        pre = fmaf(v.y, x[2 * i2 + 1], pre);
                     }
-                    const uint32_t ta = tmem_base + ((uint32_t)(q * 32) << 16) + MT_TM_OP + ls * MT_TM_SLOT + t * (2 * MT_BK);
-                    f3_tmem_st32(ta, w);
-#pragma unroll
-                    for (int i = 0; i < 32; ++i) w[i] = f3_lo(w[i]);
-                    f3_tmem_st32(ta + MT_BK, w);
-                }
-                {
-                    const float* w1c = reinterpret_cast<const float*>(w1c_mem + (size_t)rs * MT_W1C_BYTES);
-                    const int kl = g * 4;
-                    const float4 bb = *reinterpret_cast<const float4*>(w1c + MT_BK * IN + kl);
-                    const float4 gg = *reinterpret_cast<const float4*>(w1c + MT_BK * IN + MT_BK + kl);
-                    const float4 ee = *reinterpret_cast<const float4*>(w1c + MT_BK * IN + 2 * MT_BK + kl);
-                    const float bq[4] = {bb.x, bb.y, bb.z, bb.w}, gq[4] = {gg.x, gg.y, gg.z, gg.w},
-                                eq[4] = {ee.x, ee.y, ee.z, ee.w};
-                    float hi[4], lo[4];
-#pragma unroll
-                    for (int qq = 0; qq < 4; ++qq) {
-                        const float2* wr = reinterpret_cast<const float2*>(w1c + (kl + qq) * IN);
-                        float pre = 0.f;
-#pragma unroll
-                        for (int i2 = 0; i2 < IN / 2; ++i2) {
-                            const float2 v = wr[i2];
-                            pre = fmaf(v.x, x[2 * i2], pre);
-                            pre = fmaf(v.y, x[2 * i2 + 1], pre);
-                        }
-                        pre += bq[qq];
-                        const float h = fmaxf(fmaf((pre - mean) * rstd, gq[qq], eq[qq]), 0.f);
-                        hi[qq] = __uint_as_float(__float_as_uint(h) & 0xffffe000u);
-                        lo[qq] = h - hi[qq];
-                    }
-                    const int off = e * 128 + ((g ^ (e & 7)) << 4);
-                    *reinterpret_cast<float4*>(xs + off) = make_float4(hi[0], hi[1], hi[2], hi[3]);
-                    *reinterpret_cast<float4*>(xs + MT_X_BYTES + off) = make_float4(lo[0], lo[1], lo[2], lo[3]);
-                }
+                    pre += bq[qq];
+                    h[qq] = fmaxf(fmaf((pre - mean) * rstd, gq[qq], eq[qq]), 0.f);
+                }
+                uint32_t hi[2], lo[2];
+#pragma unroll
+                for (int pr = 0; pr < 2; ++pr) {
+                    const __half2 h2 = __floats2half2_rn(h[2 * pr], h[2 * pr + 1]);
+                    const float2 hf = __half22float2(h2);
+                    const __half2 l2 = __floats2half2_rn(h[2 * pr] - hf.x, h[2 * pr + 1] - hf.y);
+                    hi[pr] = *reinterpret_cast<const uint32_t*>(&h2);
+                    lo[pr] = *reinterpret_cast<const uint32_t*>(&l2);
+                }
+                *reinterpret_cast<uint2*>(xs + xoff) = make_uint2(hi[0], hi[1]);
+                *reinterpret_cast<uint2*>(xs + MT_NB * MT_ROW_BYTES + xoff) = make_uint2(lo[0], lo[1]);
+                asm volatile("fence.proxy.async.shared::cta;\n" ::: "memory");
                 __syncwarp();
-                if (lane == 0) tc_mbar_arrive(bar_raw_empty + rs);
-                asm volatile("tcgen05.wait::st.sync.aligned;\n" ::: "memory");
-                asm volatile("fence.proxy.async.shared::cta;\n" ::: "memory");
-                asm volatile("tcgen05.fence::before_thread_sync;\n" ::: "memory");
-                __syncwarp();
-                if (lane == 0) tc_mbar_arrive(bar_lo_full + ls);
+                if (lane == 0) tc_mbar_arrive(bar_full + rs);
             }
         }
     } else {
@@ -315,23 +299,25 @@
             const int n_env = min(MT_NB, p.KE - ch * MT_NB);
             const int64_t ep0 = (int64_t)m * p.KE + (int64_t)ch * MT_NB;
             const uint32_t as = js & 1, ause = js >> 1;
+            const int sxm = __ldg(p.sx + m);
             tc_mbar_wait(bar_tail_full, js & 1);
             tc_mbar_wait(bar_tfull + as, ause & 1);
             asm volatile("tcgen05.fence::after_thread_sync;\n" ::: "memory");
 #pragma unroll
             for (int t = 0; t < 2; ++t) {
-                uint32_t xh[16], xl[16];
+                uint32_t x1[16], x2[16];
                 const uint32_t ta = tmem_base + ((uint32_t)(q * 32) << 16) + as * (2 * MT_ACC) + t * MT_ACC;
-                f3_tmem_ld16(ta, xh);
-                f3_tmem_ld16(ta + MT_NB, xl);
+                f3_tmem_ld16(ta, x1);
+                f3_tmem_ld16(ta + MT_NB, x2);
                 const int row = t * 128 + q * 32 + lane;
                 const float bias = b2[row];
+                const float unscale = ldexpf(1.0f, -(wexp[row] + sxm));
                 float4* dst = reinterpret_cast<float4*>(hs + row * MT_NB);
                 const int sw = (row >> 1) & 3;
                 float h[16];
 #pragma unroll
                 for (int n = 0; n < 16; ++n)
-                    h[n] = (__uint_as_float(xl[n]) + __uint_as_float(xh[n])) + bias;
+                    h[n] = fmaf(__uint_as_float(x2[n]) + __uint_as_float(x1[n]), unscale, bias);
 #pragma unroll
                 for (int c = 0; c < 4; ++c) dst[c ^ sw] = make_float4(h[4 * c], h[4 * c + 1], h[4 * c + 2], h[4 * c + 3]);
             }
@@ -415,7 +401,7 @@
     __syncthreads();
     if (threadIdx.x == 0 && *flag && p.status) atomicOr(p.status, CEV_STATUS_NONFINITE);
     if (warp == 1)
-        asm volatile("tcgen05.dealloc.cta_group::1.sync.aligned.b32 %0, %1;\n" ::"r"(tmem_base), "r"(512u) : "memory");
+        asm volatile("tcgen05.dealloc.cta_group::1.sync.aligned.b32 %0, %1;\n" ::"r"(tmem_base), "r"(MT_TMEM_COLS) : "memory");
 }
 
 }
diff --git a/coevonet_b200/csrc/member_split.cuh b/coevonet_b200/csrc/member_split.cuh
--- /dev/null
+++ b/coevonet_b200/csrc/member_split.cuh
@@ -0,0 +1,53 @@
+#pragma once
+
+#include <cuda_fp16.h>
+
+#include "common.cuh"
+
+namespace cev {
+
+constexpr int MS_THREADS = 128;
+static_assert(MS_THREADS * 4 == H1, "one thread per float4 of an fc2 row");
+constexpr size_t MS_MATRIX_HALVES = (size_t)2 * H2 * H1;
+constexpr size_t MS_MEMBER_BYTES = MS_MATRIX_HALVES * sizeof(__half);
+
+__host__ __device__ constexpr size_t member_split_bytes(int64_t P) { return (size_t)P * (MS_MEMBER_BYTES + H2); }
+
+__device__ __forceinline__ int ls_scale_exp(float bound, int target) {
+    if (!(bound > 0.f) || !isfinite(bound)) return 0;
+    const int s = target - ilogbf(bound);
+    return s < -40 ? -40 : (s > 40 ? 40 : s);
+}
+
+__device__ __forceinline__ void member_split_row(const float (&w)[4], __half* __restrict__ split, int64_t P, int64_t m,
+                                                 int row) {
+    __shared__ uint32_t red[MS_THREADS / 32];
+    const int t = threadIdx.x;
+    uint32_t mx = max(max(__float_as_uint(w[0]) & 0x7fffffffu, __float_as_uint(w[1]) & 0x7fffffffu),
+                      max(__float_as_uint(w[2]) & 0x7fffffffu, __float_as_uint(w[3]) & 0x7fffffffu));
+    mx = __reduce_max_sync(0xffffffffu, mx);
+    if ((t & 31) == 0) red[t >> 5] = mx;
+    __syncthreads();
+    mx = max(max(red[0], red[1]), max(red[2], red[3]));
+    int e = 14 - ((int)(mx >> 23) - 127);
+    e = e < -40 ? -40 : (e > 40 ? 40 : e);
+    if (mx == 0u || mx >= 0x7f800000u) e = 0;
+    const float s = __uint_as_float((uint32_t)(127 + e) << 23);
+    uint32_t h[2], l[2];
+#pragma unroll
+    for (int i = 0; i < 2; ++i) {
+        const float v0 = w[2 * i] * s, v1 = w[2 * i + 1] * s;
+        const __half2 hh = __floats2half2_rn(v0, v1);
+        const float2 hf = __half22float2(hh);
+        const __half2 ll = __floats2half2_rn(v0 - hf.x, v1 - hf.y);
+        h[i] = *reinterpret_cast<const uint32_t*>(&hh);
+        l[i] = *reinterpret_cast<const uint32_t*>(&ll);
+    }
+    __half* hi = split + (size_t)m * MS_MATRIX_HALVES + (size_t)row * H1;
+    __half* lo = hi + (size_t)H2 * H1;
+    reinterpret_cast<uint2*>(hi)[t] = make_uint2(h[0], h[1]);
+    reinterpret_cast<uint2*>(lo)[t] = make_uint2(l[0], l[1]);
+    if (t == 0) reinterpret_cast<int8_t*>(split + (size_t)P * MS_MATRIX_HALVES)[m * H2 + row] = (int8_t)e;
+}
+
+}
diff --git a/coevonet_b200/csrc/population_ops.cu b/coevonet_b200/csrc/population_ops.cu
--- a/coevonet_b200/csrc/population_ops.cu
+++ b/coevonet_b200/csrc/population_ops.cu
@@ -1,4 +1,4 @@
-#include "common.cuh"
+#include "member_split.cuh"
 
 namespace cev {
 
@@ -65,7 +65,7 @@
     const float* __restrict__ theta, int in_dim, int64_t pitch, float sigma_arg,
     const double* __restrict__ sigma_dev,
     const PhiloxKeys keys, uint32_t tag, uint32_t gen, int64_t row0,
-    float* __restrict__ out, float* __restrict__ noise_out) {
+    float* __restrict__ out, float* __restrict__ noise_out, __half* __restrict__ split) {
     const float sigma = pick_sigma(sigma_arg, sigma_dev);
     const FcOffsets o = fc_offsets(in_dim);
     const int64_t r = blockIdx.x;
@@ -89,7 +89,11 @@
     __stcs(reinterpret_cast<float4*>(out + r * pitch + j), make_float4(p[0], p[1], p[2], p[3]));
     if (noise_out)
         *reinterpret_cast<float4*>(noise_out + r * pitch + j) = make_float4(z[0], z[1], z[2], z[3]);
-}
+    const int fc2_row = (int)blockIdx.y - o.fc2w / (K5T * 4);
+    if (split && fc2_row >= 0 && fc2_row < H2) member_split_row(p, split, gridDim.x, r, fc2_row);
+}
+static_assert(fc_offsets(IN_ADV).fc2w % (K5T * 4) == 0 && fc_offsets(IN_GOOD).fc2w % (K5T * 4) == 0 && K5T == MS_THREADS,
+              "K5 CTAs must cover whole fc2 rows");
 
 __global__ void __launch_bounds__(PT) es_perturb_prefix_kernel(
     const float* __restrict__ theta, int64_t d_pert, int64_t d_total, int64_t pitch, float sigma_arg,
@@ -586,12 +590,20 @@
 int cev_es_perturb_f32(cev_handle* h, const float* theta, int in_dim, float sigma, const double* sigma_dev,
                        uint64_t seed, int role, uint32_t gen, int64_t row0, int64_t n_rows, int64_t pitch,
                        float* out, float* noise_out, cev_stream stream) {
+    return cev_es_perturb_split_f32(h, theta, in_dim, sigma, sigma_dev, seed, role, gen, row0, n_rows, pitch, out,
+                                    noise_out, nullptr, stream);
+}
+
+int cev_es_perturb_split_f32(cev_handle* h, const float* theta, int in_dim, float sigma, const double* sigma_dev,
+                             uint64_t seed, int role, uint32_t gen, int64_t row0, int64_t n_rows, int64_t pitch,
+                             float* out, float* noise_out, void* member_split, cev_stream stream) {
     CEV_REQUIRE(h != nullptr, "es_perturb: null handle");
     if (n_rows == 0) return CEV_OK;
     CEV_REQUIRE(theta && out, "es_perturb: null pointer");
     CEV_REQUIRE(in_dim == IN_ADV || in_dim == IN_GOOD, "es_perturb: in_dim must be 8 or 10");
     CEV_REQUIRE(pitch >= fc_offsets(in_dim).total && pitch % 4 == 0, "es_perturb: bad pitch");
-    CEV_REQUIRE(aligned16(theta) && aligned16(out) && aligned16(noise_out), "es_perturb: 16B alignment");
+    CEV_REQUIRE(aligned16(theta) && aligned16(out) && aligned16(noise_out) && aligned16(member_split),
+                "es_perturb: 16B alignment");
     CEV_REQUIRE(row0 >= 0 && n_rows >= 0 && row0 + n_rows <= 0xFFFFFFFFll, "es_perturb: bad row range");
     CEV_GUARD(h);
     uint32_t k0, k1;
@@ -599,7 +611,7 @@
     dim3 grid((unsigned)n_rows, (unsigned)((pitch / 4 + K5T - 1) / K5T));
     es_perturb_kernel<<<grid, K5T, 0, (cudaStream_t)stream>>>(theta, in_dim, pitch, sigma, sigma_dev, philox_keys(k0, k1),
                                                             noise_tag(CEV_KIND_ES, role), gen, row0, out,
-                                                            noise_out);
+                                                            noise_out, static_cast<__half*>(member_split));
     return check_cuda(cudaGetLastError(), "es_perturb_kernel");
 }
 
diff --git a/coevonet_b200/csrc/rollout_lockstep.cu b/coevonet_b200/csrc/rollout_lockstep.cu
--- a/coevonet_b200/csrc/rollout_lockstep.cu
+++ b/coevonet_b200/csrc/rollout_lockstep.cu
@@ -2,6 +2,7 @@
 
 #include <cuda_fp16.h>
 
+#include "member_split.cuh"
 #include "rollout_common.cuh"
 #include "tc_common.cuh"
 
@@ -25,11 +26,13 @@
     double* l1stats;
     float2* l1ms;
     double* ml1stats;
+    int32_t* msx;
+    __half* msplit;
 };
 
 static size_t ls_align(size_t x) { return (x + 255) & ~(size_t)255; }
 
-static size_t ls_carve(void* base, int64_t N, int K, int P, LsBuffers* b) {
+static size_t ls_carve(void* base, int64_t N, int K, int P, bool own_split, LsBuffers* b) {
     size_t off = 0;
     char* p = static_cast<char*>(base);
     auto take = [&](size_t bytes) {
@@ -51,6 +54,8 @@
     t.l1stats = static_cast<double*>(take((size_t)2 * K * LS_L1S * sizeof(double)));
     t.l1ms = static_cast<float2*>(take((size_t)2 * N * sizeof(float2)));
     t.ml1stats = static_cast<double*>(take((size_t)P * LS_L1S * sizeof(double)));
+    t.msx = static_cast<int32_t*>(take((size_t)P * sizeof(int32_t)));
+    t.msplit = own_split ? static_cast<__half*>(take(member_split_bytes(P))) : nullptr;
     if (b) *b = t;
     return off;
 }
@@ -211,12 +216,6 @@
     double* l1stats;
 };
 
-__device__ __forceinline__ int ls_scale_exp(float bound, int target) {
-    if (!(bound > 0.f) || !isfinite(bound)) return 0;
-    const int s = target - ilogbf(bound);
-    return s < -40 ? -40 : (s > 40 ? 40 : s);
-}
-
 __global__ void __launch_bounds__(256) ls_wmax_kernel(const LsPrepParams p) {
     const int oi = blockIdx.y / p.K, k = blockIdx.y % p.K;
     const FcOffsets o = fc_offsets(seat_in_dim(p.seat[oi]));
@@ -295,30 +294,35 @@
     }
 }
 
+__device__ __forceinline__ int ls_act_scale_exp(const float* __restrict__ row, int in) {
+    __shared__ float red[2][16];
+    const int t = threadIdx.x;
+    float g = fabsf(row[H1 * in + H1 + t]), be = fabsf(row[H1 * in + 2 * H1 + t]);
+#pragma unroll
+    for (int off = 16; off > 0; off >>= 1) {
+        g = fmaxf(g, __shfl_xor_sync(0xffffffffu, g, off));
+        be = fmaxf(be, __shfl_xor_sync(0xffffffffu, be, off));
+    }
+    if ((t & 31) == 0) {
+        red[0][t >> 5] = g;
+        red[1][t >> 5] = be;
+    }
+    __syncthreads();
+    if (t != 0) return 0;
+    for (int w = 1; w < 16; ++w) {
+        g = fmaxf(g, red[0][w]);
+        be = fmaxf(be, red[1][w]);
+    }
+    return ls_scale_exp(22.63f * g + be, 13);
+}
+
 __global__ void __launch_bounds__(512) ls_l1stats_kernel(const LsPrepParams p) {
     const int oi = blockIdx.x / p.K, k = blockIdx.x % p.K;
     const int in = seat_in_dim(p.seat[oi]);
     const float* row = p.opp[oi] + (int64_t)k * p.opp_pitch[oi];
     ls_l1stats_row(row, in, p.l1stats + (size_t)blockIdx.x * LS_L1S);
-    __shared__ float red[2][16];
-    const int t = threadIdx.x;
-    float g = fabsf(row[H1 * in + H1 + t]), be = fabsf(row[H1 * in + 2 * H1 + t]);
-#pragma unroll
-    for (int off = 16; off > 0; off >>= 1) {
-        g = fmaxf(g, __shfl_xor_sync(0xffffffffu, g, off));
-        be = fmaxf(be, __shfl_xor_sync(0xffffffffu, be, off));
-    }
-    if ((t & 31) == 0) {
-        red[0][t >> 5] = g;
-        red[1][t >> 5] = be;
-    }
-    __syncthreads();
-    if (t == 0) {
-        for (int w = 1; w < 16; ++w) {
-            g = fmaxf(g, red[0][w]);
-            be = fmaxf(be, red[1][w]);
-        }
-        const int sx = ls_scale_exp(22.63f * g + be, 13);
+    const int sx = ls_act_scale_exp(row, in);
+    if (threadIdx.x == 0) {
         const int sw = ls_scale_exp(__uint_as_float(p.wmax[blockIdx.x]), 14);
         p.oscale[blockIdx.x * 2 + 0] = ldexpf(1.0f, sx);
         p.oscale[blockIdx.x * 2 + 1] = ldexpf(1.0f, -(sx + sw));
@@ -326,8 +330,20 @@
 }
 
 __global__ void __launch_bounds__(512) ls_member_l1stats_kernel(const float* __restrict__ members, int64_t pitch, int in,
-                                                                double* __restrict__ out) {
-    ls_l1stats_row(members + (int64_t)blockIdx.x * pitch, in, out + (size_t)blockIdx.x * LS_L1S);
+                                                                double* __restrict__ out, int32_t* __restrict__ sx_out) {
+    const float* row = members + (int64_t)blockIdx.x * pitch;
+    ls_l1stats_row(row, in, out + (size_t)blockIdx.x * LS_L1S);
+    const int sx = ls_act_scale_exp(row, in);
+    if (threadIdx.x == 0) sx_out[blockIdx.x] = sx;
+}
+
+__global__ void __launch_bounds__(MS_THREADS) ls_member_split_kernel(const float* __restrict__ members, int64_t pitch,
+                                                                     int in, __half* __restrict__ split) {
+    const int64_t m = blockIdx.x;
+    const float4 v = __ldg(reinterpret_cast<const float4*>(members + m * pitch + fc_offsets(in).fc2w +
+                                                           (int64_t)blockIdx.y * H1) + threadIdx.x);
+    const float w[4] = {v.x, v.y, v.z, v.w};
+    member_split_row(w, split, gridDim.x, m, blockIdx.y);
 }
 
 #ifndef LS_GRID_OPP_DEFAULT
@@ -774,7 +790,7 @@
     }
     const int64_t N = (int64_t)p.P * p.K * p.E;
     LsBuffers& b = c->b;
-    ls_carve(ws, N, p.K, p.P, &b);
+    ls_carve(ws, N, p.K, p.P, p.member_split == nullptr, &b);
     const int ms = p.member_seat;
     c->ms = ms;
     const int seat_of[2] = {ms == 0 ? 1 : 0, ms == 2 ? 1 : 2};
@@ -794,16 +810,22 @@
     ls_wmax_kernel<<<dim3(32, 2 * p.K), 256, 0, stream>>>(pp);
     ls_split_w2_kernel<<<dim3(32, 2 * p.K), 256, 0, stream>>>(pp);
     ls_l1stats_kernel<<<2 * p.K, 512, 0, stream>>>(pp);
-    ls_member_l1stats_kernel<<<p.P, 512, 0, stream_m>>>(p.members, p.member_pitch, seat_in_dim(ms), b.ml1stats);
+    ls_member_l1stats_kernel<<<p.P, 512, 0, stream_m>>>(p.members, p.member_pitch, seat_in_dim(ms), b.ml1stats, b.msx);
+    const __half* msplit = static_cast<const __half*>(p.member_split);
+    if (!msplit) {
+        ls_member_split_kernel<<<dim3(p.P, H2), MS_THREADS, 0, stream_m>>>(p.members, p.member_pitch, seat_in_dim(ms),
+                                                                             b.msplit);
+        msplit = b.msplit;
+    }
 
     const FcOffsets om = fc_offsets(seat_in_dim(ms));
     {
-        cuuint64_t dims[3] = {(cuuint64_t)H1, (cuuint64_t)H2, (cuuint64_t)p.P};
-        cuuint64_t strides[2] = {(cuuint64_t)H1 * 4, (cuuint64_t)p.member_pitch * 4};
+        cuuint64_t dims[3] = {(cuuint64_t)H1, (cuuint64_t)2 * H2, (cuuint64_t)p.P};
+        cuuint64_t strides[2] = {(cuuint64_t)H1 * sizeof(__half), (cuuint64_t)MS_MEMBER_BYTES};
         cuuint32_t box[3] = {MT_BK, H2, 1};
         cuuint32_t estr[3] = {1, 1, 1};
-        CUresult r = encode(&c->map_wtc, CU_TENSOR_MAP_DATA_TYPE_FLOAT32, 3, const_cast<float*>(p.members + om.fc2w), dims,
-                            strides, box, estr, CU_TENSOR_MAP_INTERLEAVE_NONE, CU_TENSOR_MAP_SWIZZLE_128B,
+        CUresult r = encode(&c->map_wtc, CU_TENSOR_MAP_DATA_TYPE_FLOAT16, 3, const_cast<__half*>(msplit), dims, strides,
+                            box, estr, CU_TENSOR_MAP_INTERLEAVE_NONE, CU_TENSOR_MAP_SWIZZLE_64B,
                             CU_TENSOR_MAP_L2_PROMOTION_L2_256B, CU_TENSOR_MAP_FLOAT_OOB_FILL_NONE);
         if (r != CUDA_SUCCESS) {
             set_error("rollout_lockstep: cuTensorMapEncodeTiled(member fc2, tensor-core form) failed with %d", (int)r);
@@ -877,6 +899,8 @@
     tp.act = b.act + (int64_t)ms * N;
     tp.gap = b.gap + (int64_t)ms * N;
     tp.l1stats = b.ml1stats;
+    tp.sx = b.msx;
+    tp.wexp = reinterpret_cast<const int8_t*>(msplit + (size_t)p.P * MS_MATRIX_HALVES);
     tp.status = p.status;
     return CEV_OK;
 }
@@ -889,7 +913,7 @@
 int launch_rollout_lockstep(cev_handle* h, const ClusterParams& p, cudaStream_t stream) {
     if (p.P <= 0 || p.K <= 0 || p.E <= 0) return CEV_OK;
     const int64_t N = (int64_t)p.P * p.K * p.E;
-    int rc = ls_reserve(h, ls_carve(nullptr, N, p.K, p.P, nullptr));
+    int rc = ls_reserve(h, ls_carve(nullptr, N, p.K, p.P, p.member_split == nullptr, nullptr));
     if (rc) return rc;
     rc = ls_configure(h);
     if (rc) return rc;
@@ -974,7 +998,9 @@
         return CEV_OK;
     }
     const int64_t N = (int64_t)p0.P * p0.K * p0.E;
-    const size_t per_role = ls_align(ls_carve(nullptr, N, p0.K, p0.P, nullptr));
+    bool own_split = false;
+    for (int r = 0; r < n_roles; ++r) own_split = own_split || ps[r].member_split == nullptr;
+    const size_t per_role = ls_align(ls_carve(nullptr, N, p0.K, p0.P, own_split, nullptr));
     int rc = ls_reserve(h, per_role * n_roles);
     if (rc) return rc;
     rc = ls_configure(h);
@@ -1060,4 +1086,13 @@
     return check_cuda(cudaGetLastError(), "rollout_lockstep (roles) launch");
 }
 
-}
+int64_t member_split_bytes_api(int64_t P) { return (int64_t)member_split_bytes(P); }
+
+int launch_member_split(int member_seat, const float* members, int64_t P, int64_t pitch, void* split,
+                        cudaStream_t stream) {
+    ls_member_split_kernel<<<dim3((unsigned)P, H2), MS_THREADS, 0, stream>>>(members, pitch, seat_in_dim(member_seat),
+                                                                           static_cast<__half*>(split));
+    return check_cuda(cudaGetLastError(), "ls_member_split_kernel");
+}
+
+}
diff --git a/coevonet_b200/engine.py b/coevonet_b200/engine.py
--- a/coevonet_b200/engine.py
+++ b/coevonet_b200/engine.py
@@ -121,6 +121,7 @@
         self._eval_stream = None
         self.fused_roles = bool(getattr(args, "fused_roles", True)) and self.device.type == "cuda"
         self.update_from_members = bool(getattr(args, "update_from_members", True))
+        self.member_split = None
         self.order = _lib.ORDER_REFERENCE if self.compat else _lib.ORDER_STABLE_DESC
         self.adaptive = bool(getattr(args, "adaptive", False))
         self.early_stopping = bool(getattr(args, "early_stopping", False))
@@ -265,8 +266,11 @@
     def _rollouts(self, specs, limit):
         n_cycles = _limit_cycles(self.k, limit)
         if self.fused_roles and self.k1_events is None and hasattr(self.k, "mpe_rollout_roles") and len(specs) > 1:
+            kw = {}
+            if self.member_split is not None:
+                kw["member_splits"] = [self.member_split[spec[0]] for spec in specs]
             outs = self.k.mpe_rollout_roles(specs, n_cycles=n_cycles, pos_first=self.pos_first, status=self.status,
-                                            variant=self.variant)
+                                            variant=self.variant, **kw)
             return {spec[0]: out for spec, out in zip(specs, outs)}
         res = {}
 
@@ -494,6 +498,9 @@
         self.weight_stats = {r: None for r in ROLES}
         self.member_stats = bool(getattr(args, "log_member_weight_stats", False))
         self.variant = self.rollout_variant(self.P, 1)
+        if self.variant == 3 and self.fused_roles and hasattr(self.k, "member_split_bytes"):
+            n_bytes = self.k.member_split_bytes(self.shard.n_local)
+            self.member_split = {r: torch.empty(n_bytes, dtype=torch.uint8, device=self.device) for r in ROLES}
 
     def _base_opponents(self, role):
         t = self.theta
@@ -520,8 +527,9 @@
 
         def prepare(role):
             in_dim = layout.OBS_DIM[role]
+            kw = {"split": self.member_split[role]} if self.member_split is not None else {}
             self.k.es_perturb(self.theta[role], in_dim, self.sigma_dev(role), self.seed, role, self.gen,
-                              self.shard.row0, self.shard.n_local, out=self.members[role])
+                              self.shard.row0, self.shard.n_local, out=self.members[role], **kw)
             if self.member_stats:
                 self.weight_stats[role] = self.k.weight_stats(self.members[role], in_dim)
             if ref_init is not None:
diff --git a/coevonet_b200/ops.py b/coevonet_b200/ops.py
--- a/coevonet_b200/ops.py
+++ b/coevonet_b200/ops.py
@@ -124,7 +124,8 @@
     return out
 
 
-def mpe_rollout_roles(roles, *, n_cycles=MAX_CYCLES, pos_first=True, init_shared=False, variant=0, status=None):
+def mpe_rollout_roles(roles, *, n_cycles=MAX_CYCLES, pos_first=True, init_shared=False, variant=0, status=None,
+                      member_splits=None):
     outs, recs, keep = [], (_lib.RolloutRole * len(roles))(), []
     P = K = E = None
     dev = None
@@ -156,12 +157,46 @@
         r.init, r.out = init.data_ptr(), out.data_ptr()
     if not roles or P == 0:
         return outs
+    splits = (ctypes.c_void_p * len(roles))()
+    if member_splits is not None:
+        if len(member_splits) != len(roles):
+            raise _lib.CevError("member_splits needs one entry (or None) per role")
+        for i, sp in enumerate(member_splits):
+            if sp is not None:
+                _check_split(sp, P, dev)
+                splits[i] = sp.data_ptr()
+        keep.append(member_splits)
     cfg = RolloutCfg(int(n_cycles), int(bool(pos_first)), int(variant), 0)
     _, n_launch = rollout_plan(dev.index, P, K, E, n_cycles, variant)
-    check(_call("cev_mpe_rollout_roles_f32", _h(dev), len(roles), recs, P, K, int(bool(init_shared)), E,
-                ctypes.byref(cfg), _ptr(status), _stream(dev), launches=n_launch * len(roles)),
-          "cev_mpe_rollout_roles_f32")
+    check(_call("cev_mpe_rollout_roles_split_f32", _h(dev), len(roles), recs, splits, P, K, int(bool(init_shared)),
+                E, ctypes.byref(cfg), _ptr(status), _stream(dev), launches=n_launch * len(roles)),
+          "cev_mpe_rollout_roles_split_f32")
     return outs
+
+
+def member_split_bytes(P):
+    return int(_lib.load().cev_member_split_bytes(int(P)))
+
+
+def _check_split(split, P, dev):
+    if split.dtype != torch.uint8 or not split.is_contiguous() or split.numel() < member_split_bytes(P) or \
+            split.device != dev:
+        raise _lib.CevError("member split: need a contiguous uint8 buffer of member_split_bytes(P) bytes on the "
+                            "members' device")
+
+
+def member_split(member_role, members, *, out=None):
+    dev = _need_cuda(members, out)
+    seat = layout.SEAT_OF[member_role] if isinstance(member_role, str) else int(member_role)
+    P = members.shape[0]
+    if members.dtype != torch.float32:
+        raise _lib.CevError("members must be float32")
+    if out is None:
+        out = torch.empty(member_split_bytes(P), dtype=torch.uint8, device=dev)
+    _check_split(out, P, dev)
+    check(_call("cev_member_split_f32", _h(dev), seat, _ptr(members), P, members.stride(0), _ptr(out), _stream(dev)),
+          "cev_member_split_f32")
+    return out
 
 
 def mpe_rollout_trace(member_role, members, opp_a, opp_b, init, *, n_cycles=MAX_CYCLES, pos_first=True,
@@ -264,8 +299,8 @@
     return idx
 
 
-def es_perturb(theta, in_dim, sigma, seed, role, gen, row0, n_rows, *, out=None, noise_out=None):
-    dev = _need_cuda(theta, out, noise_out)
+def es_perturb(theta, in_dim, sigma, seed, role, gen, row0, n_rows, *, out=None, noise_out=None, split=None):
+    dev = _need_cuda(theta, out, noise_out, split)
     pitch = layout.fc_pitch(in_dim)
     if theta.numel() < pitch:
         raise _lib.CevError("es_perturb: theta must be a padded flat row")
@@ -273,9 +308,12 @@
         out = torch.empty((n_rows, pitch), dtype=torch.float32, device=dev)
     role_id = layout.ROLE_ID[role] if isinstance(role, str) else int(role)
     sig, sig_dev = _sigma_args(sigma)
-    check(_call("cev_es_perturb_f32", 
+    if split is not None:
+        _check_split(split, n_rows, dev)
+    check(_call("cev_es_perturb_split_f32",
         _h(dev), _ptr(theta), int(in_dim), sig, sig_dev, int(seed), role_id, int(gen),
-        int(row0), int(n_rows), pitch, _ptr(out), _ptr(noise_out), _stream(dev)), "cev_es_perturb_f32")
+        int(row0), int(n_rows), pitch, _ptr(out), _ptr(noise_out), _ptr(split), _stream(dev)),
+        "cev_es_perturb_split_f32")
     return out
 
 
diff --git a/include/coevonet_b200.h b/include/coevonet_b200.h
--- a/include/coevonet_b200.h
+++ b/include/coevonet_b200.h
@@ -74,6 +74,10 @@
                               int P, int K, int init_shared, int E,
                               const cev_rollout_cfg* cfg, int32_t* status, cev_stream stream);
 
+int cev_mpe_rollout_roles_split_f32(cev_handle* h, int n_roles, const cev_rollout_role* roles,
+                                    const void* const* member_split, int P, int K, int init_shared, int E,
+                                    const cev_rollout_cfg* cfg, int32_t* status, cev_stream stream);
+
 int cev_mpe_rollout_trace_f32(cev_handle* h, int member_seat,
                               const float* members, int P, int64_t member_pitch,
                               const float* opp_a, int64_t opp_a_pitch,
@@ -121,6 +125,16 @@
                        float sigma, const double* sigma_dev, uint64_t seed, int role, uint32_t gen,
                        int64_t row0, int64_t n_rows, int64_t pitch,
                        float* out, float* noise_out, cev_stream stream);
+
+int64_t cev_member_split_bytes(int64_t P);
+
+int cev_es_perturb_split_f32(cev_handle* h, const float* theta, int in_dim,
+                             float sigma, const double* sigma_dev, uint64_t seed, int role, uint32_t gen,
+                             int64_t row0, int64_t n_rows, int64_t pitch,
+                             float* out, float* noise_out, void* member_split, cev_stream stream);
+
+int cev_member_split_f32(cev_handle* h, int member_seat, const float* members, int64_t P, int64_t pitch,
+                         void* member_split, cev_stream stream);
 
 int cev_es_perturb_prefix_f32(cev_handle* h, const float* theta, int64_t d_pert, int64_t d_total, float sigma,
                               const double* sigma_dev, uint64_t seed, int role, uint32_t gen, int64_t row0,
```

New measurement: 134.9 million, median of 6. +2.4%, better.
